# ChenDavidTimothy/mujoco-template

Hardware: AMD Instinct MI355X
Metric: env-steps/sec (whole node), humanoid batch=4096 random-ctrl rollout (higher is better)
Workload: dtype f32

## Files before the change

### mujoco_template_amd/csrc/mjb_api.hip

```cpp
#include <hip/hip_runtime.h>

#include <dlfcn.h>

#include <cmath>
#include <cstdio>
#include <cstdlib>
#include <chrono>
#include <cstring>
#include <map>
#include <string>
#include <vector>

#include "../../include/mjbatch.h"
#include "mjb_buffer.hpp"
#include "mjb_host.hpp"
#include "mjb_kernels.hpp"
#include "mjb_lqr.hpp"
#include "mjb_dare.hpp"
#include "mjb_eig.hpp"
#include "mjb_dlyap.hpp"
#include "mjb_traj.hpp"

using namespace mjb;

namespace {
thread_local std::string g_err;
int fail(int code, const std::string& msg) { g_err = msg; return code; }
#define HIPCHK(expr)                                                                                           \
  do {                                                                                                         \
    hipError_t e_ = (expr);                                                                                    \
    if (e_ != hipSuccess) return fail(MJB_ERR_DEVICE, std::string(#expr) + ": " + hipGetErrorString(e_));      \
  } while (0)

struct DevAlloc {
  Arena& arena;
  template <typename X> const X* put(const std::vector<X>& v) {
    X* p = arena.alloc<X>(v.size());
    if (p && v.size() && hipMemcpy(p, v.data(), v.size() * sizeof(X), hipMemcpyHostToDevice) != hipSuccess) arena.ok = false;
    return p;
  }
  const float* putf(const std::vector<float>& v) { return put(v); }
  const double* putf(const std::vector<double>& v) { return put(v); }
  const int* puti(const std::vector<int>& v) { return put(v); }
  const unsigned long long* putu(const std::vector<unsigned long long>& v) { return put(v); }
};
template <typename... B> void reset_all(B&... b) { (b.reset(), ...); }
template <typename X> hipError_t reserve_zeroed(Buffer<X>& b, size_t n) {
  if (n <= b.count()) return hipSuccess;
  hipError_t e = b.reserve(n);
  if (e == hipSuccess && b.kind() != Mem::Device) std::memset(b.get(), 0, n * sizeof(X));
  else if (e == hipSuccess && (e = hipMemset(b.get(), 0, n * sizeof(X))) != hipSuccess) b.reset();
  return e;
}

struct ArrayInfo { void* ptr; long per_env; int kind; };
}

struct mjbModel {
  HostModel h;
  int disableactuator;
  int iterations;
  double tolerance;
  std::vector<char> blob;
  struct Field { std::string name; int dtype; long count; size_t off; };
  std::vector<Field> fields;
  std::map<int, std::vector<std::string>> names;
};

struct mjbObsSpec {
  ObsSpecDev dev;
  Arena arena;
};

struct Config {
  int G, G_fd, ncon_max, nefc_max;
  Lay Lf, Ld;
  Lay Lf2;
};

struct mjbData {
  mjbModel* model;
  int batch, dtype, device, env0;
  Config cfg;
  hipStream_t stream;
  Arena arena;
  DevModel<float> mf;
  DevModel<double> md;
// ... 170 lines not shown
  HIPCHK(hipMemcpy(d->md_dev, &d->md, sizeof(d->md), hipMemcpyHostToDevice));
  d->up_disable = mm->disableactuator; d->up_iter = mm->iterations; d->up_tol = mm->tolerance;
  return MJB_OK;
}


void choose_caps(const HostModel& h, int dtype, int lanes, int nconmax, int nefcmax, int& nc_out, int& ne_out) {
  int ne, nc;
  if (nconmax > 0 || nefcmax > 0) {
    nc = nconmax > 0 ? nconmax : (h.ncon_alloc < 32 ? h.ncon_alloc : 32);
    ne = nefcmax > 0 ? nefcmax : (h.nefc_alloc < 96 ? h.nefc_alloc : 96);
  } else {
    const size_t budget = (size_t)160 * 1024 / (dtype == MJB_F32 ? 8 : 4);
    ne = h.nefc_alloc < 96 ? h.nefc_alloc : 96; nc = 0;
    if (h.nefc_alloc <= 96 && h.ncon_alloc <= 32) {
      ne = h.nefc_alloc; nc = h.ncon_alloc;
    } else for (;; ne -= 8) {
      int hi = ne * 3 / 8; if (hi < 8) hi = 8; if (hi > h.ncon_alloc) hi = h.ncon_alloc;
      int lo = ne / 3; if (lo < 8) lo = 8; if (lo > hi) lo = hi;
      bool fits = false;
      for (nc = hi; nc >= lo; nc--) {
        Lay t = make_layout(h, nc > 0 ? nc : 1, ne > 0 ? ne : 1, dtype == MJB_F32 ? sizeof(float) : sizeof(double));
        if ((size_t)(64 / lanes) * (size_t)t.bytes <= budget) { fits = true; break; }
      }
      if (fits) break;
      if (ne <= 32) { nc = hi; break; }
    }
  }
  if (nc < 1) nc = 1;
  if (ne < 1) ne = 1;
  nc_out = nc; ne_out = ne;
}
int auto_lanes(const HostModel& h, int lanes) { return lanes == 0 ? (h.nv <= 4 ? 8 : (h.nv <= 16 ? 16 : 64)) : lanes; }

bool derive_config(const HostModel& h, int dtype, int lanes, int nconmax, int nefcmax, Config& c, std::string& err) {
  c.G = auto_lanes(h, lanes);
  if (c.G != 8 && c.G != 16 && c.G != 64) { err = "lanes must be 8, 16 or 64"; return false; }
  choose_caps(h, dtype, c.G, nconmax, nefcmax, c.ncon_max, c.nefc_max);
  c.Lf = make_layout(h, c.ncon_max, c.nefc_max, sizeof(float));
  c.Ld = make_layout(h, c.ncon_max, c.nefc_max, sizeof(double));
  c.G_fd = c.G;
  while (c.G_fd < 64 && (size_t)(64 / c.G_fd) * (size_t)c.Ld.bytes > 160 * 1024) c.G_fd = c.G_fd == 8 ? 16 : 64;
  const size_t lds = (size_t)(64 / c.G) * (size_t)(dtype == MJB_F32 ? c.Lf.bytes : c.Ld.bytes);
  if (lds > 160 * 1024 || (size_t)(64 / c.G_fd) * (size_t)c.Ld.bytes > 160 * 1024) {
    char buf[256];
    std::snprintf(buf, sizeof buf, "per-workgroup LDS %zu B exceeds 160 KiB (lower nconmax/nefcmax or use more lanes)", lds);
    err = buf;
    return false;
  }
  std::memset(&c.Lf2, 0, sizeof(Lay));
  if (dtype == MJB_F32 && c.G == 64 && h.nv <= 32 && h.integrator != INT_RK4) {
    c.Lf2 = make_layout(h, c.ncon_max, c.nefc_max, sizeof(float), true);
    if ((size_t)c.Lf2.bytes > 64 * 1024) std::memset(&c.Lf2, 0, sizeof(Lay));
  }
  return true;
}

struct KernelKind { const char* symbol; const char* banner; const char* not_applicable; };
const KernelKind kKinds[4] = {
    {nullptr, nullptr, nullptr},
    {"mjb_k_step_spec", "// generated by mjb_model_spec_source(): size- and layout-specialised k_step<float, float, G> of ONE compiled model\n",
     "only the float32 step kernel is specialised"},
    {"mjb_k_fd_spec", "// generated by mjb_fd_spec_source(): size- and layout-specialised k_fd<double, TS, G> of ONE compiled model\n", ""},
    {"mjb_k_step2_spec", "// generated by mjb_step2_spec_source(): size- and (flat) layout-specialised two-wave step kernel k_step2<float, float> of ONE compiled model\n",
     "the two-wave step kernel does not apply to this configuration (fp32, one wave per environment, nv <= 32, Euler)"},
};
bool valid_kind(int kind) { return kind == MJB_KERNEL_STEP || kind == MJB_KERNEL_FD || kind == MJB_KERNEL_STEP2; }

struct KernelTarget { const Lay* L; int G; const char* ts; bool applies; };
KernelTarget kernel_target(const Config& c, int dtype, int kind) {
  switch (kind) {
    case MJB_KERNEL_STEP: return {&c.Lf, c.G, "float", dtype == MJB_F32};
    case MJB_KERNEL_FD: return {&c.Ld, c.G_fd, dtype == MJB_F32 ? "float" : "double", true};
    default: return {&c.Lf2, 64, "float", c.Lf2.bytes > 0};
  }
}
int check_kind(const Config& c, int dtype, int kind) {
  if (!valid_kind(kind)) return fail(MJB_ERR_ARG, "unknown kernel kind (MJB_KERNEL_STEP, MJB_KERNEL_FD or MJB_KERNEL_STEP2)");
  if (!kernel_target(c, dtype, kind).applies) return fail(MJB_ERR_ARG, kKinds[kind].not_applicable);
  return MJB_OK;
}

struct EmitAlloc {
  std::string text;
  int n = 0;
  static constexpr unsigned long long TOKEN = 0x7E57AB1Eull << 32;
  template <typename X, typename F> const X* emit(const std::vector<X>& v, const char* ctype, F fmt) {
    std::string body;
    if (v.empty()) body = "0";
    for (size_t i = 0; i < v.size(); i++) { if (i) body += (i % 16 == 0 ? ",\n " : ","); body += fmt(v[i]); }
    text += std::string("static const __constant__ ") + ctype + " mjb_tab_" + std::to_string(n) + "[] = {" + body + "};\n";
    return (const X*)(uintptr_t)(TOKEN + (unsigned long long)(n++) * 16ull + 16ull);
  }
  const float* putf(const std::vector<float>& v) {
    return emit(v, "float", [](float x) {
      if (std::isnan(x)) return std::string("__builtin_nanf(\"\")");
      if (std::isinf(x)) return std::string(x > 0 ? "__builtin_inff()" : "-__builtin_inff()");
      char b[48]; std::snprintf(b, sizeof(b), "%af", (double)x); return std::string(b);
    });
  }
  const double* putf(const std::vector<double>& v) {
    return emit(v, "double", [](double x) {
      if (std::isnan(x)) return std::string("__builtin_nan(\"\")");
      if (std::isinf(x)) return std::string(x > 0 ? "__builtin_inf()" : "-__builtin_inf()");
      char b[48]; std::snprintf(b, sizeof(b), "%a", x); return std::string(b);
    });
  }
  const int* puti(const std::vector<int>& v) { return emit(v, "int", [](int x) { return std::to_string(x); }); }
  const unsigned long long* putu(const std::vector<unsigned long long>& v) {
    return emit(v, "unsigned long long", [](unsigned long long x) { char b[40]; std::snprintf(b, sizeof(b), "0x%llxull", x); return std::string(b); });
  }
};

template <typename T>
std::string baked_model_source(const HostModel& h, int ncon_max, int nefc_max) {
  static_assert(sizeof(DevModel<T>) % 8 == 0, "DevModel<T> is written out in 8-byte words");
  const char* tname = sizeof(T) == 4 ? "float" : "double";
  EmitAlloc ea;
  DevModel<T> m;
  fill_dev_model<T>(h, ea, ncon_max, nefc_max, m);
  const size_t nw = sizeof(m) / 8;
  std::vector<unsigned long long> wv(nw);
  std::memcpy(wv.data(), (const void*)&m, sizeof(m));
  std::string decl = "struct MjbBakedModel {", init = "static const __constant__ MjbBakedModel mjb_baked_model = {";
  for (size_t i = 0; i < nw; i++) {
    const unsigned long long v = wv[i];
    if ((v >> 32) == (EmitAlloc::TOKEN >> 32)) {
      decl += " const void MJB_CONST* p" + std::to_string(i) + ";";
      init += " (const void MJB_CONST*)mjb_tab_" + std::to_string((int)((v - EmitAlloc::TOKEN) / 16 - 1)) + ",";
    } else {
      char b[64];
      decl += " unsigned a" + std::to_string(i) + ", b" + std::to_string(i) + ";";
      std::snprintf(b, sizeof(b), " 0x%xu, 0x%xu,", (unsigned)(v & 0xffffffffull), (unsigned)(v >> 32));
      init += b;
    }
    if (i % 8 == 7) init += "\n ";
  }
  decl += " };\n"; init += " };\n";
  {
    std::vector<int> seen((size_t)ea.n, 0);
    bool ok = true;
    for (size_t i = 0; i < nw && ok; i++)
      if ((wv[i] >> 32) == (EmitAlloc::TOKEN >> 32)) {
        const unsigned long long k = (wv[i] - EmitAlloc::TOKEN) / 16 - 1;
        if (k >= (unsigned long long)ea.n || (wv[i] - EmitAlloc::TOKEN) % 16 != 0 || seen[(size_t)k]++) ok = false;
      }
    for (int k = 0; k < ea.n && ok; k++) if (seen[(size_t)k] != 1) ok = false;
    if (!ok) return std::string("// (model not baked in: the DevModel image did not map one-to-one onto the emitted tables)\n");
  }
  std::string s = "#include \"mjb_types.hpp\"\n// the model as constant data of this translation unit (tables, then the DevModel image)\n";
  s += ea.text + decl + init;
  s += std::string("static_assert(sizeof(MjbBakedModel) == sizeof(mjb::DevModel<") + tname + ">), \"baked model image\");\n";
  s += std::string("#define MJB_SPEC_BAKED (*(const mjb::DevModel<") + tname + "> MJB_CONST*)&mjb_baked_model)\n";
  return s;
}

std::string spec_source(const HostModel& h_model, const Config& c, int dtype, int kind, int prm_mask) {
  HostModel h_damped;
  if ((prm_mask >> PRM_DOF_DAMPING) & 1) { h_damped = h_model; h_damped.has_damping = 1; }
  const HostModel& h = (prm_mask >> PRM_DOF_DAMPING) & 1 ? h_damped : h_model;
  const KernelTarget t = kernel_target(c, dtype, kind);
  const Lay& L = *t.L;
  const int ncon_max = c.ncon_max, nefc_max = c.nefc_max;
  std::string s = kKinds[kind].banner;
  s += "#define MJB_SPEC_KERNEL " + std::to_string(kind) + "\n#define MJB_SPEC_TS " + t.ts + "\n#define MJB_SPEC_G " + std::to_string(t.G) + "\n#define MJB_SPEC_ASSUME(m)";
  auto A = [&](const char* obj, const char* f, long v) { s += std::string(" __builtin_assume((") + obj + ")." + f + " == " + std::to_string(v) + ");"; };
#define SM(f, v) A("m", #f, (long)(v))
  SM(nq, h.nq); SM(nv, h.nv); SM(nu, h.nu); SM(nbody, h.nbody); SM(njnt, h.njnt); SM(ngeom, h.ngeom); SM(nsite, h.nsite);
  SM(ntendon, h.ntendon); SM(nwrap, h.nwrap); SM(nsensor, h.nsensor); SM(nsensordata, h.nsensordata); SM(nkey, h.nkey); SM(npair, h.npair);
  SM(nlevel, h.nlevel); SM(integrator, h.integrator); SM(has_damping, h.has_damping); SM(has_fluid, h.has_fluid); SM(has_accel, h.has_accel);
  SM(nvp, h.nvp); SM(nvshift, h.nvshift); SM(ncon_max, ncon_max); SM(nefc_max, nefc_max); SM(nsiteact, h.siteact.size()); SM(nmpair, h.mpair.size());
  SM(nround, h.nround); SM(nround_inner, h.nround_inner); SM(max_nsub, h.max_nsub); SM(dfs_ok, h.dfs_ok);
#undef SM
  s += "\n";
  if (prm_mask) s += "#define MJB_SPEC_PARAMS " + std::to_string(prm_mask) + "   // per-environment model parameters: bit k = field MJB_PRM_k\n";
  s += "#define MJB_SPEC_ASSUME_LAY(L)";
#define SL(f) A("L", #f, (long)L.f)
  SL(qpos); SL(qvel); SL(ctrl); SL(qacc); SL(qacc_ws); SL(qacc_smooth); SL(qfrc_bias); SL(qfrc_passive); SL(qfrc_actuator); SL(qfrc_smooth);
  SL(qfrc_constraint); SL(xpos); SL(xquat); SL(xmat); SL(xipos); SL(ximat); SL(xanchor); SL(xaxis); SL(geom_xpos); SL(geom_xmat); SL(site_xpos);
  SL(site_xmat); SL(subtree_com); SL(cinert); SL(crb); SL(cdof); SL(cdof_dot); SL(cvel); SL(cacc); SL(cfrc); SL(dofbuf); SL(bfrc); SL(M); SL(W);
  SL(ten_length); SL(ten_J); SL(act_force); SL(sens); SL(con); SL(efc_J); SL(efc_pos); SL(efc_D); SL(efc_aref); SL(efc_jar); SL(efc_jv);
  SL(efc_force); SL(efc_KBI); SL(Ma); SL(grad); SL(search); SL(Mv); SL(tmp); SL(cholcol); SL(rk); SL(nT); SL(i_efc_type); SL(i_efc_id);
  SL(i_con_pair); SL(i_scal); SL(i_mail); SL(nI); SL(bytes);
#undef SL
  s += "\n";
  {
    bool le2 = true;
    for (const char* name : {"jnt_solimp", "tendon_solimp", "pair_solimp"}) {
      const auto& v = h.D(name);
      for (size_t k = 4; k < v.size(); k += 5) { const double pw = v[k] > 1.0 ? v[k] : 1.0; if (pw != 1.0 && pw != 2.0) le2 = false; }
    }
    if (le2) s += "#define MJB_SPEC_SOLIMP_POWER_1_OR_2 1\n";
  }
  s += kind != MJB_KERNEL_FD ? baked_model_source<float>(h, ncon_max, nefc_max) : baked_model_source<double>(h, ncon_max, nefc_max);
  s += "#include \"mjb_kernels.hpp\"\n";
  if (prm_mask) s += "extern \"C\" __constant__ int mjb_spec_params = " + std::to_string(prm_mask) + ";   // checked by mjb_kernel_load\n";
  return s;
}

static void choose_schedule(mjbData* d, StepArgs& a) {
  a.chunk_steps = 0; a.fair_bit = 0; a.nblk = 0; a.grid_blocks = 0; a.nuniform = 0; a.nchunk = 0;
  if (a.mode != 0) return;
  if (d->sched_chunk == -1) {
    const char* e1 = std::getenv("MJB_CHUNK_STEPS"); const char* e2 = std::getenv("MJB_FAIR_BIT");
    d->sched_chunk = e1 ? std::atoi(e1) : -2; d->fair_bit = e2 ? std::atoi(e2) : -2;
  }
  const int epb = 64 / d->cfg.G;
  const long nblk = (d->batch + epb - 1) / epb;
  if (d->step_slots < 0) {
    int nb = 0;
    if (hipFunction_t fn = d->spec[MJB_KERNEL_STEP].fn) {
      if (hipModuleOccupancyMaxActiveBlocksPerMultiprocessor(&nb, fn, 64, (size_t)epb * d->cfg.Lf.bytes) != hipSuccess) nb = 0;
    } else nb = d->dtype == MJB_F32 ? step_blocks_per_cu<float, float>(d->cfg.G, d->cfg.Lf) : step_blocks_per_cu<double, double>(d->cfg.G, d->cfg.Ld);
    d->step_slots = nb > 0 ? (long)nb * d->ncu : 0;
  }
  a.fair_bit = d->fair_bit >= 0 ? d->fair_bit : 15;
  a.nblk = (int)nblk; a.grid_blocks = d->step_slots > 0 && d->step_slots < nblk ? (int)d->step_slots : (int)nblk;
  if (d->sched_chunk >= 0) {
    a.chunk_steps = a.nstep > 1 ? d->sched_chunk : 0;
    if (std::getenv("MJB_SCHED_DEBUG")) std::fprintf(stderr, "[mjb] schedule (override): blocks %ld, resident slots %ld, steps %d -> chunk_steps %d, fair_bit %d\n", nblk, d->step_slots, a.nstep, a.chunk_steps, a.fair_bit);
    return;
  }
  if (d->step_slots > 0 && nblk > d->step_slots && a.nstep >= 4) {
    int c = (int)std::lround(std::sqrt(3.0 * (double)a.nstep));
    a.chunk_steps = c < 1 ? 1 : (c > 32 ? 32 : c);
  }
  if (std::getenv("MJB_SCHED_DEBUG")) std::fprintf(stderr, "[mjb] schedule: blocks %ld, resident slots %ld, steps %d -> chunk_steps %d, fair_bit %d\n", nblk, d->step_slots, a.nstep, a.chunk_steps, a.fair_bit);
}

int engine_check(const mjbData* d) {
  if (d->flags_pin.get() && __atomic_load_n(d->flags_pin.get() + 3, __ATOMIC_ACQUIRE) != 0)
    return fail(MJB_ERR_DEVICE, "a ticket-mode launch timed out waiting for a state hand-over (engine flag 8): the environments concerned were not "
                                "advanced; mjb_reset() clears the condition");
  return MJB_OK;
}

hipError_t launch_spec_step(mjbData* d, int kind, const Lay* lg, const DevDebug<float>& dbg, const StepArgs& a, const ObsSpecDev& obs,
                            void* obs_out, unsigned grid, unsigned block, size_t lds) {
  const DevModel<float>* mg = d->mf_dev;
  DevData<float> dv = d->df; DevDebug<float> dbgarg = dbg; StepArgs av = a; ObsSpecDev ov = obs; float* oo = (float*)obs_out;
  void* args[] = {(void*)&mg, (void*)&lg, (void*)&dv, (void*)&dbgarg, (void*)&av, (void*)&ov, (void*)&oo};
  return hipModuleLaunchKernel(d->spec[kind].fn, grid, 1, 1, block, 1, 1, (unsigned)lds, d->stream, args, nullptr);
}

int launch(mjbData* d, const StepArgs& a_in, const ObsSpecDev& obs, void* obs_out, bool debug) {
  int rc = engine_check(d);
  if (rc != MJB_OK) return rc;
  rc = refresh_options(d);
  if (rc != MJB_OK) return rc;
  hipError_t e;
  StepArgs a = a_in;
  choose_schedule(d, a);
  if (a.chunk_steps > 0) {
    if (d->dtype != MJB_F32 || a.nstep >= (1 << 20) - 2) a.chunk_steps = 0;
  }
  if (a.chunk_steps > 0 && !d->df.xfer) {
    const HostModel& hm = d->model->h;
    if (reserve_zeroed(d->xfer, (size_t)d->batch * (size_t)(hm.nq + 3 * hm.nv + 2)) != hipSuccess) a.chunk_steps = 0;
    d->df.xfer = d->xfer.get();
  }
  if (a.chunk_steps > 0) chunk_plan_counts(a.nstep, a.chunk_steps, a.nuniform, a.nchunk);
  if (a.mode == 0) {
    const int epb = 64 / d->cfg.G;
    d->last_sched[0] = a.nstep; d->last_sched[1] = (d->batch + epb - 1) / epb; d->last_sched[2] = (int)(d->step_slots > 0 ? d->step_slots : 0);
    d->last_sched[3] = a.chunk_steps; d->last_sched[4] = a.fair_bit;
  }
  unsigned seq_next = d->launch_seq;
  unsigned long long ticket_after = d->ticket_next;
  if (a.chunk_steps > 0) {
    do { seq_next++; } while ((seq_next & 0xFFFu) == 0);
    a.tagbase = (seq_next & 0xFFFu) << 20;
    const unsigned long long adv = (unsigned long long)a.nblk * (unsigned)a.nchunk + (unsigned long long)a.grid_blocks;
    if (d->ticket_next + adv > 0xF0000000ull) { HIPCHK(hipMemsetAsync(d->df.sched, 0, sizeof(unsigned), d->stream)); d->ticket_next = 0; }
    a.ticket_base = (unsigned)d->ticket_next;
    ticket_after = d->ticket_next + adv;
    if (d->xfer_timeout == 0) {
      const char* e1 = std::getenv("MJB_XFER_TIMEOUT_MS");
// ... 1668 lines not shown
```

### mujoco_template_amd/csrc/mjb_device.hpp

```cpp
#pragma once
#include "mjb_types.hpp"

#ifdef MJB_HOST_EMU
#include <cmath>
#include "mjb_hostemu.hpp"
#define MJB_DEV static inline
#define MJB_DEVM inline
#define MJB_DEV_CALL static __attribute__((noinline))
#else
#include <hip/hip_runtime.h>
#define MJB_DEV __device__ __forceinline__
#define MJB_DEVM __device__ __forceinline__
#define MJB_DEV_CALL __device__ __attribute__((noinline))
#endif

#ifdef MJB_HOST_EMU
#define MJB_MFMA(a, b, acc) emu_mfma((a), (b), (acc))
#define MJB_BALLOT(p) emu_ballot(p)
#define MJB_RSQF(x) (1.0f / sqrtf(x))
#define MJB_RCPF(x) (1.0f / (x))
#define MJB_MEMTIME() 0ull
#define MJB_OPAQUE1(a) ((void)0)
#define MJB_OPAQUE2(a, b) ((void)0)
#define MJB_OPAQUE9(a, b, c, d, e, f, g, h, i) ((void)0)
#else
#define MJB_MFMA(a, b, acc) __builtin_amdgcn_mfma_f32_32x32x2f32((a), (b), (acc), 0, 0, 0)
#define MJB_BALLOT(p) __ballot(p)
#define MJB_RSQF(x) __builtin_amdgcn_rsqf(x)
#define MJB_RCPF(x) __builtin_amdgcn_rcpf(x)
#define MJB_MEMTIME() __builtin_amdgcn_s_memtime()
#define MJB_OPAQUE1(a) asm volatile("" : "+v"(a))
#define MJB_OPAQUE2(a, b) asm volatile("" : "+v"(a), "+v"(b))
#define MJB_OPAQUE9(a, b, c, d, e, f, g, h, i) asm volatile("" : "+v"(a), "+v"(b), "+v"(c), "+v"(d), "+v"(e), "+v"(f), "+v"(g), "+v"(h), "+v"(i))
#endif

namespace mjb {

#ifndef MJB_HOST_EMU
typedef float mjb_f16v __attribute__((ext_vector_type(16)));
#endif

#ifndef MJB_HOST_EMU
template <int G> MJB_DEV void gsync() {
  __builtin_amdgcn_fence(__ATOMIC_RELEASE, "wavefront");
  __builtin_amdgcn_wave_barrier();
  __builtin_amdgcn_fence(__ATOMIC_ACQUIRE, "wavefront");
}

template <int CTRL> MJB_DEV int dpp_i(int v) { return __builtin_amdgcn_update_dpp(0, v, CTRL, 0xF, 0xF, false); }
template <int CTRL> MJB_DEV float dpp_f(float v) { return __int_as_float(dpp_i<CTRL>(__float_as_int(v))); }
template <int CTRL> MJB_DEV double dpp_f(double v) {
  return __hiloint2double(dpp_i<CTRL>(__double2hiint(v)), dpp_i<CTRL>(__double2loint(v)));
}
MJB_DEV int rdlane_i(int v, int l) { return __builtin_amdgcn_readlane(v, l); }
MJB_DEV float rdlane_f(float v, int l) { return __int_as_float(__builtin_amdgcn_readlane(__float_as_int(v), l)); }
MJB_DEV double rdlane_f(double v, int l) {
  return __hiloint2double(__builtin_amdgcn_readlane(__double2hiint(v), l), __builtin_amdgcn_readlane(__double2loint(v), l));
}
MJB_DEV float wave_rows_sum(float v) {
  asm("s_nop 1\n\tv_add_f32_dpp %0, %0, %0 row_bcast:15 row_mask:0xa bank_mask:0xf\n\ts_nop 1\n\tv_add_f32_dpp %0, %0, %0 row_bcast:31 row_mask:0xc bank_mask:0xf" : "+v"(v));
  return rdlane_f(v, 63);
}
MJB_DEV double wave_rows_sum(double v) { return (rdlane_f(v, 0) + rdlane_f(v, 16)) + (rdlane_f(v, 32) + rdlane_f(v, 48)); }
MJB_DEV int wave_rows_sum(int v) { return (rdlane_i(v, 0) + rdlane_i(v, 16)) + (rdlane_i(v, 32) + rdlane_i(v, 48)); }
template <typename T, int G> MJB_DEV T gsum(T v) {
  v += dpp_f<0xB1>(v);
  v += dpp_f<0x4E>(v);
  if (G >= 8) v += dpp_f<0x141>(v);
  if (G >= 16) v += dpp_f<0x140>(v);
  if (G == 64) v = wave_rows_sum(v);
  return v;
}
template <int G> MJB_DEV int gsumi(int v) {
  v += dpp_i<0xB1>(v);
  v += dpp_i<0x4E>(v);
  if (G >= 8) v += dpp_i<0x141>(v);
  if (G >= 16) v += dpp_i<0x140>(v);
  if (G == 64) v = wave_rows_sum(v);
  return v;
}
template <int G> MJB_DEV int gmaxi(int v) {
  int t;
  t = dpp_i<0xB1>(v); v = t > v ? t : v;
  t = dpp_i<0x4E>(v); v = t > v ? t : v;
// ... 319 lines not shown
  T e[NB][NB];
#pragma unroll
  for (int a = 0; a < NB; a++)
#pragma unroll
    for (int b = 0; b < NB; b++) {
      int r = 8 * a + lr, cc = 8 * b + lc;
      e[a][b] = (r < n && cc <= r) ? M[r * n + cc] : (T)0;
    }
  if (mode == 1) {
    for (int row = 0; row < nefc; row++) {
      T d = dw[row];
      if (d == 0) continue;
      T jr[NB], jc[NB];
#pragma unroll
      for (int a = 0; a < NB; a++) { int r = 8 * a + lr; jr[a] = r < n ? d * J[row * n + r] : (T)0; }
#pragma unroll
      for (int b = 0; b < NB; b++) { int cc = 8 * b + lc; jc[b] = cc < n ? J[row * n + cc] : (T)0; }
#pragma unroll
      for (int a = 0; a < NB; a++)
#pragma unroll
        for (int b = 0; b < NB; b++) e[a][b] += jr[a] * jc[b];
    }
  } else if (mode == 2) {
    if (lr == lc) {
#pragma unroll
      for (int a = 0; a < NB; a++) { int r = 8 * a + lr; if (r < n) e[a][a] += m.timestep * m.dof_damping[r]; }
    }
  }
  for (int j = 0; j < n; j++) {
    const int bj = j >> 3, lj = j & 7;
    if (lr == lj && lc == lj) {
#pragma unroll
      for (int b = 0; b < NB; b++) if (b == bj) col[n] = e[b][b];
    }
    gsync<64>();
    const T ljj = t_sqrt(t_max(col[n], Num<T>::minval()));
    const T inv = 1 / ljj;
    if (lc == lj) {
#pragma unroll
      for (int b = 0; b < NB; b++) {
        if (b != bj) continue;
#pragma unroll
        for (int a = 0; a < NB; a++) {
          int r = 8 * a + lr;
          if (r > j && r < n) { T v = e[a][b] * inv; e[a][b] = v; col[r] = v; }
          else if (r == j) e[a][b] = ljj;
        }
      }
    }
    if (lane == 0) dinv[j] = inv;
    gsync<64>();
    T rv[NB], cv[NB];
#pragma unroll
    for (int a = 0; a < NB; a++) { int r = 8 * a + lr; rv[a] = (r > j && r < n) ? col[r] : (T)0; }
#pragma unroll
    for (int b = 0; b < NB; b++) { int cc = 8 * b + lc; cv[b] = (cc > j && cc < n) ? col[cc] : (T)0; }
#pragma unroll
    for (int a = 0; a < NB; a++)
#pragma unroll
      for (int b = 0; b < NB; b++) e[a][b] -= rv[a] * cv[b];
  }
#pragma unroll
  for (int a = 0; a < NB; a++)
#pragma unroll
    for (int b = 0; b < NB; b++) {
      int r = 8 * a + lr, cc = 8 * b + lc;
      if (r < n && cc <= r) W[tri_at(r, cc)] = e[a][b];
    }
  gsync<64>();
}

#ifndef MJB_SPEC_ASSUME
#define MJB_SPEC_ASSUME(m)
#endif
#ifndef MJB_SPEC_ASSUME_LAY
#define MJB_SPEC_ASSUME_LAY(L)
#endif
#if defined(MJB_SPEC_BAKED) && !defined(MJB_HOST_EMU)
#define MJB_MODEL_OF(p) MJB_SPEC_BAKED
#else
#define MJB_MODEL_OF(p) (*(p))
#endif
#define MJB_OPT(c, f) ((*(c).mp).f)
#ifdef MJB_HOST_EMU
#define MJB_ENV(c) ModelRef<T> m = *(c).mp; LayRef L = *(c).lp
#else
#define MJB_ENV(c)                                     \
  auto mp_ = (c).mp; auto lp_ = (c).lp;                \
  asm volatile("" : "+s"(mp_), "+s"(lp_));             \
  ModelRef<T> m = MJB_MODEL_OF(mp_); LayRef L = *lp_;  \
  MJB_SPEC_ASSUME(m) MJB_SPEC_ASSUME_LAY(L)
#endif
template <typename T> using ModelRef = const DevModel<T> MJB_CONST&;
typedef const Lay MJB_CONST& LayRef;

template <typename T> struct Ctx {
  bool skip_dynamics = false;
  const DevModel<T> MJB_CONST* mp;
  const Lay MJB_CONST* lp;
  const PrmRows MJB_CONST* pr;
  int env;
  T* w;
  int* wi;
  int lane;
  int ncon, nefc, niter, con_dropped, efc_dropped;
#if defined(MJB_PHASE_REPEAT) && !defined(MJB_HOST_EMU)
  int rep = -1;
#endif
#if defined(MJB_PROFILE) && !defined(MJB_HOST_EMU)
  unsigned long long pacc[PH_N] = {};
  unsigned long long pt = 0;
#endif
  MJB_DEVM Ctx(const DevModel<T> MJB_CONST* m_, const Lay MJB_CONST* L_, T* w_, int* wi_, int lane_, const PrmRows MJB_CONST* pr_ = nullptr, int env_ = 0)
      : mp(m_), lp(L_), pr(pr_), env(env_), w(w_), wi(wi_), lane(lane_), ncon(0), nefc(0), niter(0), con_dropped(0), efc_dropped(0) {}
};

#if defined(MJB_SPEC_KERNEL) && !defined(MJB_HOST_EMU)
#ifndef MJB_SPEC_PARAMS
#define MJB_SPEC_PARAMS 0
#endif
#define MJB_PRM_ON(k) ((((MJB_SPEC_PARAMS) >> (k)) & 1) != 0)
#define MJB_PRM_SURE 1
#else
#define MJB_PRM_ON(k) true
#define MJB_PRM_SURE 0
#endif
template <int K> MJB_DEVM constexpr int prm_src() { return K == PRM_SUBTREEMASS ? PRM_BODY_MASS : (K == PRM_PAIR_FRICTION ? PRM_GEOM_FRICTION : K); }
template <typename T> struct PrmSel;
template <> struct PrmSel<float> { static MJB_DEVM const float MJB_CONST* get(const PrmRows MJB_CONST* r, int k) { return r->f[k]; } };
template <> struct PrmSel<double> { static MJB_DEVM const double MJB_CONST* get(const PrmRows MJB_CONST* r, int k) { return r->d[k]; } };
template <int K, typename T, typename TP>
MJB_DEV const T MJB_CONST* prm_row(const Ctx<T>& c, TP tab, int n) {
  if constexpr (MJB_PRM_ON(prm_src<K>())) {
#ifdef MJB_HOST_EMU
    if (!c.pr) return tab;
#endif
    const T MJB_CONST* row = PrmSel<T>::get(c.pr, K);
    if (MJB_PRM_SURE || row) return row + (long)c.env * n;
  }
  return tab;
}
template <int K, typename T, typename TP>
MJB_DEV T prm_get(const Ctx<T>& c, TP tab, int n, int i, int ti) {
  if constexpr (MJB_PRM_ON(prm_src<K>())) {
#ifdef MJB_HOST_EMU
    if (!c.pr) return tab[ti];
#endif
    const T MJB_CONST* row = PrmSel<T>::get(c.pr, K);
    if (MJB_PRM_SURE || row) return row[(long)c.env * n + i];
  }
  return tab[ti];
}
template <typename T> MJB_DEV bool has_damping(const Ctx<T>& c, int model_has_damping) {
  if constexpr (MJB_PRM_ON(PRM_DOF_DAMPING)) {
    if (MJB_PRM_SURE) return true;
#ifdef MJB_HOST_EMU
    if (!c.pr) return model_has_damping != 0;
#endif
    return model_has_damping != 0 || PrmSel<T>::get(c.pr, PRM_DOF_DAMPING) != nullptr;
  }
  return model_has_damping != 0;
}
template <typename T> struct DampRef { T timestep; const T MJB_CONST* dof_damping; };
template <typename T> MJB_DEV DampRef<T> damp_ref(const Ctx<T>& c, const DevModel<T> MJB_CONST& m) {
  return DampRef<T>{m.timestep, prm_row<PRM_DOF_DAMPING>(c, m.dof_damping, m.nv)};
}

#if defined(MJB_PROFILE) && !defined(MJB_HOST_EMU)
#define MJB_STAMP_START(c) ((c).pt = __builtin_amdgcn_s_memtime())
#define MJB_STAMP(c, k) do { unsigned long long t_ = __builtin_amdgcn_s_memtime(); (c).pacc[k] += t_ - (c).pt; (c).pt = t_; } while (0)
#define MJB_TIMED(c, k, call) do { unsigned long long t0_ = __builtin_amdgcn_s_memtime(); call; (c).pacc[k] += __builtin_amdgcn_s_memtime() - t0_; } while (0)
#define MJB_COUNT(c, k) ((c).pacc[k] += 1)
#define MJB_PACC(c, k) ((c).pacc + (k))
#define MJB_PROF_FLUSH(c, prof, lane) do { if ((lane) == 0 && (prof)) for (int k_ = 0; k_ < PH_N; k_++) atomicAdd((prof) + k_, (c).pacc[k_]); } while (0)
#else
#define MJB_STAMP_START(c) ((void)0)
#define MJB_STAMP(c, k) ((void)0)
#define MJB_TIMED(c, k, call) do { call; } while (0)
#define MJB_COUNT(c, k) ((void)0)
#define MJB_PACC(c, k) nullptr
#define MJB_PROF_FLUSH(c, prof, lane) ((void)0)
#endif
#if defined(MJB_PHASE_REPEAT) && !defined(MJB_HOST_EMU)
#define MJB_SET_REPEAT(c, k) ((c).rep = (k))
#define MJB_REPEATS(c, k) ((c).rep == (k))
#else
#define MJB_SET_REPEAT(c, k) ((void)0)
#define MJB_REPEATS(c, k) false
#endif
#define MJB_REP_N(c, id) (MJB_REPEATS(c, id) ? 2 : 1)
#define MJB_PHASE_CALL(c, k, call) do { call; if (MJB_REPEATS(c, k)) { gsync<G>(); call; } } while (0)
enum { REP_CHOL = 32, REP_REUSE = 33, REP_MV = 34, REP_LS = 35, REP_WARM = 36, REP_GRAD = 37, REP_CTRL = 38 };

template <typename T, typename MRef>
MJB_DEV void reg_factor32(MRef m, const T* M, T* W, T* dinv, const T* J, const T* dw, int nefc, int mode, int n, int lane, T* x) {
  T a[32];
  const bool own = lane < n;
#pragma unroll
  for (int k = 0; k < 32; k++) a[k] = (own && k < n) ? M[lane * n + k] : ((k == lane) ? (T)1 : (T)0);
  if (mode == 1) {
    for (int row = 0; row < nefc; row++) {
      T d = dw[row];
      if (d == 0) continue;
      T jrow = own ? J[row * n + lane] : (T)0;
      T s = d * jrow;
#pragma unroll
      for (int k = 0; k < 32; k++) a[k] += s * rdlane_f(jrow, k);
    }
  } else if (mode == 2) {
    T dd = own ? m.timestep * m.dof_damping[lane] : (T)0;
#pragma unroll
    for (int k = 0; k < 32; k++) if (k == lane) a[k] += dd;
  }
  T myinv = 1;
  T r = (x && own) ? x[lane] : (T)0;
#pragma unroll
  for (int j = 0; j < 32; j++) {
    T ajj = t_max(rdlane_f(a[j], j), Num<T>::minval());
    T inv = t_rsqrt(ajj);
    T ljj = ajj * inv;
    a[j] = lane == j ? ljj : a[j] * inv;
    if (lane == j) myinv = inv;
    T yj = rdlane_f(r, j) * inv;
    r = lane > j ? r - a[j] * yj : (lane == j ? yj : r);
#pragma unroll
    for (int k = j + 1; k < 32; k++) a[k] -= a[j] * rdlane_f(a[j], k);
  }
  if (own) {
#pragma unroll
    for (int k = 0; k < 32; k++) if (k <= lane) W[tri_at(lane, k)] = a[k];
    dinv[lane] = myinv;
  }
  gsync<64>();
  if (x) {
    T lrow[32];
// ... 351 lines not shown
#pragma unroll
      for (int k = 0; k < NC; k++) { pa[k] = arr[NC * p + k]; ch[k] = arr[NC * b + k]; }
#pragma unroll
      for (int k = 0; k < NC; k++) arr[NC * p + k] = pa[k] + ch[k];
    }
    gsync<G>();
  }
}

#define MJB_TREE_PASSES 4
template <typename T, int G, int NC> MJB_DEV void tree_forward_sum(Ctx<T>& c, T* arr) {
  MJB_ENV(c); const int lane = c.lane;
  const int nitem = m.nbody * NC, nl = m.nlevel;
  if (nitem > MJB_TREE_PASSES * G) { tree_forward_sum_levels<T, G, NC>(c, arr); return; }
  T s[MJB_TREE_PASSES];
#pragma unroll
  for (int ps = 0; ps < MJB_TREE_PASSES; ps++) {
    const int e = lane + ps * G;
    s[ps] = 0;
    if (e < nitem) {
      const int b = e / NC, k = e - b * NC;
      int na = b > 0 ? m.body_depth[b] - 1 : 0;
      MJB_OPAQUE1(na);
      T acc = arr[e];
      for (int u = 0; u < nl - 1; u++) {
        const int a = m.body_anc[b * nl + u];
        T v = arr[NC * a + k];
        acc += u < na ? v : (T)0;
      }
      s[ps] = acc;
    }
  }
  gsync<G>();
#pragma unroll
  for (int ps = 0; ps < MJB_TREE_PASSES; ps++) { const int e = lane + ps * G; if (e < nitem) arr[e] = s[ps]; }
  gsync<G>();
}
template <typename T, int G, int NC> MJB_DEV void tree_backward_sum(Ctx<T>& c, T* arr, int nrounds, int first_body) {
  MJB_ENV(c); const int lane = c.lane;
  const int nitem = m.nbody * NC, mx = m.max_nsub;
  if (!m.dfs_ok || nitem > MJB_TREE_PASSES * G) { tree_backward_sum_rounds<T, G, NC>(c, arr, nrounds); return; }
  T s[MJB_TREE_PASSES];
#pragma unroll
  for (int ps = 0; ps < MJB_TREE_PASSES; ps++) {
    if (ps * G >= nitem) { s[ps] = 0; continue; }
    const int e = lane + ps * G;
    const bool on = e < nitem;
    const int b = on ? e / NC : 0;
    const int n = on && b >= first_body ? m.body_nsub[b] : 0;
    const T* base = arr + (on ? e : 0);
    T acc = base[0];
    for (int d0 = 0; d0 < mx && gany<G>(d0 < n); d0 += 4) {
      T v[4];
#pragma unroll
      for (int u = 0; u < 4; u++) { const int dd = d0 + u + 1; v[u] = base[NC * (dd <= n ? dd : n)]; }
#pragma unroll
      for (int u = 0; u < 4; u++) acc += d0 + u + 1 <= n ? v[u] : (T)0;
    }
    s[ps] = acc;
  }
  gsync<G>();
#pragma unroll
  for (int ps = 0; ps < MJB_TREE_PASSES; ps++) { const int e = lane + ps * G; if (e < nitem) arr[e] = s[ps]; }
  gsync<G>();
}

template <typename T> MJB_DEV void quat_rot(T* r, const T* q, const T* v) {
  T R[9];
  quat2mat(R, q);
  mulmatvec3(r, R, v);
}

template <typename T, int G> MJB_DEV void kinematics(Ctx<T>& c) {
  MJB_ENV(c); T* w = c.w; const int lane = c.lane;
  T *xpos = w + L.xpos, *xquat = w + L.xquat, *xmat = w + L.xmat, *xipos = w + L.xipos, *ximat = w + L.ximat;
  T *qpos = w + L.qpos, *xanchor = w + L.xanchor, *xaxis = w + L.xaxis;
  if (lane == 0) {
    xpos[0] = xpos[1] = xpos[2] = 0; xquat[0] = 1; xquat[1] = xquat[2] = xquat[3] = 0;
    xipos[0] = xipos[1] = xipos[2] = 0;
#pragma unroll
    for (int k = 0; k < 9; k++) { xmat[k] = (k % 4 == 0) ? (T)1 : (T)0; ximat[k] = xmat[k]; }
  }
  for (int b = 1 + lane; b < m.nbody; b += G) {
    const int jadr = m.body_irec[4 * b], jnum = m.body_irec[4 * b + 1], jt0 = m.body_irec[4 * b + 2];
    T pos[3], quat[4], R[9];
    if (jnum == 1 && jt0 == JNT_FREE) {
      int qa = m.jnt_irec[6 * jadr + 1];
      quat[0] = qpos[qa + 3]; quat[1] = qpos[qa + 4]; quat[2] = qpos[qa + 5]; quat[3] = qpos[qa + 6];
      quat_normalize(quat);
      qpos[qa + 3] = quat[0]; qpos[qa + 4] = quat[1]; qpos[qa + 5] = quat[2]; qpos[qa + 6] = quat[3];
      pos[0] = qpos[qa]; pos[1] = qpos[qa + 1]; pos[2] = qpos[qa + 2];
      xanchor[3 * jadr] = pos[0]; xanchor[3 * jadr + 1] = pos[1]; xanchor[3 * jadr + 2] = pos[2];
      xaxis[3 * jadr] = 0; xaxis[3 * jadr + 1] = 0; xaxis[3 * jadr + 2] = 1;
    } else {
#pragma unroll
      for (int k = 0; k < 3; k++) pos[k] = m.body_pos[3 * b + k];
#pragma unroll
      for (int k = 0; k < 4; k++) quat[k] = m.body_quat[4 * b + k];
      quat2mat(R, quat);
      for (int j = jadr; j < jadr + jnum; j++) {
        T jp[3] = {m.jnt_rec[8 * j], m.jnt_rec[8 * j + 1], m.jnt_rec[8 * j + 2]};
        T ja[3] = {m.jnt_rec[8 * j + 3], m.jnt_rec[8 * j + 4], m.jnt_rec[8 * j + 5]};
        const int jtype = m.jnt_irec[6 * j], qa = m.jnt_irec[6 * j + 1];
        T val = qpos[qa] - m.jnt_rec[8 * j + 6];
        T anchor[3], axis[3];
        mulmatvec3(anchor, R, jp);
        anchor[0] += pos[0]; anchor[1] += pos[1]; anchor[2] += pos[2];
        mulmatvec3(axis, R, ja);
        xanchor[3 * j] = anchor[0]; xanchor[3 * j + 1] = anchor[1]; xanchor[3 * j + 2] = anchor[2];
        xaxis[3 * j] = axis[0]; xaxis[3 * j + 1] = axis[1]; xaxis[3 * j + 2] = axis[2];
        if (jtype == JNT_SLIDE) {
          pos[0] += axis[0] * val; pos[1] += axis[1] * val; pos[2] += axis[2] * val;
        } else {
          T ql[4], qn[4], v[3];
          axisangle2quat(ql, ja, val);
          quat_mul(qn, quat, ql);
          quat[0] = qn[0]; quat[1] = qn[1]; quat[2] = qn[2]; quat[3] = qn[3];
          quat2mat(R, quat);
          mulmatvec3(v, R, jp);
          pos[0] = anchor[0] - v[0]; pos[1] = anchor[1] - v[1]; pos[2] = anchor[2] - v[2];
        }
      }
    }
#pragma unroll
    for (int k = 0; k < 3; k++) xpos[3 * b + k] = pos[k];
#pragma unroll
    for (int k = 0; k < 4; k++) xquat[4 * b + k] = quat[k];
  }
  gsync<G>();
  if (m.nbody - 1 <= G) {
    const int b = 1 + lane, nl = m.nlevel;
    const bool own = b < m.nbody;
    const int dep = own ? m.body_depth[b] : 0;
    for (int d = 1; d < nl; d <<= 1) {
      const bool hop = own && d <= dep - 1;
      T pq[4], pp[3], lq[4], lp[3], q[4], t[3];
      if (hop) {
        const int a = m.body_anc[b * nl + d - 1];
#pragma unroll
        for (int k = 0; k < 4; k++) { pq[k] = xquat[4 * a + k]; lq[k] = xquat[4 * b + k]; }
#pragma unroll
        for (int k = 0; k < 3; k++) { pp[k] = xpos[3 * a + k]; lp[k] = xpos[3 * b + k]; }
        quat_mul(q, pq, lq);
        quat_rot(t, pq, lp);
      }
      gsync<G>();
      if (hop) {
#pragma unroll
        for (int k = 0; k < 4; k++) xquat[4 * b + k] = q[k];
#pragma unroll
        for (int k = 0; k < 3; k++) xpos[3 * b + k] = pp[k] + t[k];
      }
      gsync<G>();
    }
    if (own) {
      T q[4];
#pragma unroll
      for (int k = 0; k < 4; k++) q[k] = xquat[4 * b + k];
      quat_normalize(q);
#pragma unroll
      for (int k = 0; k < 4; k++) xquat[4 * b + k] = q[k];
    }
    gsync<G>();
  } else {
    const int b0 = 1 + lane;
    int dep0 = -1, par0 = 0;
    if (b0 < m.nbody) { dep0 = m.body_depth[b0]; par0 = m.body_parentid[b0]; }
    for (int lev = 1; lev <= m.nlevel; lev++) {
      for (int b = b0; b < m.nbody; b += G) {
        const int dep = b == b0 ? dep0 : m.body_depth[b];
        if (dep != lev) continue;
        const int p = b == b0 ? par0 : m.body_parentid[b];
        T pq[4], pp[3], lq[4], lp[3], q[4], t[3];
#pragma unroll
        for (int k = 0; k < 4; k++) { pq[k] = xquat[4 * p + k]; lq[k] = xquat[4 * b + k]; }
#pragma unroll
        for (int k = 0; k < 3; k++) { pp[k] = xpos[3 * p + k]; lp[k] = xpos[3 * b + k]; }
        quat_mul(q, pq, lq);
        quat_normalize(q);
        quat_rot(t, pq, lp);
#pragma unroll
        for (int k = 0; k < 4; k++) xquat[4 * b + k] = q[k];
#pragma unroll
        for (int k = 0; k < 3; k++) xpos[3 * b + k] = pp[k] + t[k];
      }
      gsync<G>();
    }
  }
  for (int b = 1 + lane; b < m.nbody; b += G) {
    T quat[4], R[9], t[3], q2[4], R2[9];
#pragma unroll
    for (int k = 0; k < 4; k++) quat[k] = xquat[4 * b + k];
    quat2mat(R, quat);
    T ip[3] = {m.body_ipos[3 * b], m.body_ipos[3 * b + 1], m.body_ipos[3 * b + 2]};
    T iq[4] = {m.body_iquat[4 * b], m.body_iquat[4 * b + 1], m.body_iquat[4 * b + 2], m.body_iquat[4 * b + 3]};
    mulmatvec3(t, R, ip);
    quat_mul(q2, quat, iq);
    quat2mat(R2, q2);
#pragma unroll
    for (int k = 0; k < 3; k++) xipos[3 * b + k] = xpos[3 * b + k] + t[k];
#pragma unroll
    for (int k = 0; k < 9; k++) { xmat[9 * b + k] = R[k]; ximat[9 * b + k] = R2[k]; }
  }
  for (int j = lane; j < m.njnt; j += G) {
    if (m.jnt_irec[6 * j] == JNT_FREE) continue;
    int p = m.jnt_irec[6 * j + 4];
    T pq[4], R[9], a[3], ax[3], la[3] = {xanchor[3 * j], xanchor[3 * j + 1], xanchor[3 * j + 2]}, lx[3] = {xaxis[3 * j], xaxis[3 * j + 1], xaxis[3 * j + 2]};
#pragma unroll
    for (int k = 0; k < 4; k++) pq[k] = xquat[4 * p + k];
    quat2mat(R, pq);
    mulmatvec3(a, R, la);
    mulmatvec3(ax, R, lx);
#pragma unroll
    for (int k = 0; k < 3; k++) { xanchor[3 * j + k] = xpos[3 * p + k] + a[k]; xaxis[3 * j + k] = ax[k]; }
  }
  gsync<G>();
  T *gx = w + L.geom_xpos, *gm = w + L.geom_xmat, *sx = w + L.site_xpos, *sm = w + L.site_xmat;
  for (int g = lane; g < m.ngeom + m.nsite; g += G) {
    bool is_geom = g < m.ngeom;
    int id = is_geom ? g : g - m.ngeom;
    int b = is_geom ? m.geom_bodyid[id] : m.site_bodyid[id];
    auto lp = is_geom ? m.geom_pos + 3 * id : m.site_pos + 3 * id;
    auto lq = is_geom ? m.geom_quat + 4 * id : m.site_quat + 4 * id;
    T p3[3] = {lp[0], lp[1], lp[2]}, q4[4] = {lq[0], lq[1], lq[2], lq[3]}, bm[9], bq[4], t[3], q[4], R[9];
#pragma unroll
    for (int k = 0; k < 9; k++) bm[k] = xmat[9 * b + k];
#pragma unroll
    for (int k = 0; k < 4; k++) bq[k] = xquat[4 * b + k];
    mulmatvec3(t, bm, p3);
    quat_mul(q, bq, q4);
    quat_normalize(q);
    quat2mat(R, q);
    T* op = is_geom ? gx + 3 * id : sx + 3 * id;
    T* om = is_geom ? gm + 9 * id : sm + 9 * id;
#pragma unroll
    for (int k = 0; k < 3; k++) op[k] = xpos[3 * b + k] + t[k];
#pragma unroll
    for (int k = 0; k < 9; k++) om[k] = R[k];
  }
  gsync<G>();
}

template <typename T, int G> MJB_DEV void com_pos(Ctx<T>& c) {
  MJB_ENV(c); T* w = c.w; const int lane = c.lane;
  T *sc = w + L.subtree_com, *xipos = w + L.xipos, *ximat = w + L.ximat, *xmat = w + L.xmat;
  for (int b = lane; b < m.nbody; b += G) {
    T ms = prm_row<PRM_BODY_MASS>(c, m.body_mass, m.nbody)[b];
#pragma unroll
    for (int k = 0; k < 3; k++) sc[3 * b + k] = ms * xipos[3 * b + k];
  }
  gsync<G>();
  tree_backward_sum<T, G, 3>(c, sc, m.nround, 0);
  for (int b = lane; b < m.nbody; b += G) {
    T sm = prm_row<PRM_SUBTREEMASS>(c, m.body_subtreemass, m.nbody)[b];
    if (sm < Num<T>::minval()) { sc[3 * b] = xipos[3 * b]; sc[3 * b + 1] = xipos[3 * b + 1]; sc[3 * b + 2] = xipos[3 * b + 2]; }
    else { T inv = 1 / sm; sc[3 * b] *= inv; sc[3 * b + 1] *= inv; sc[3 * b + 2] *= inv; }
  }
  gsync<G>();
  T* cin = w + L.cinert;
  for (int b = lane; b < m.nbody; b += G) {
    if (b == 0) {
#pragma unroll
      for (int k = 0; k < 10; k++) cin[k] = 0;
      continue;
    }
    int r = m.body_rootid[b];
    T off[3], im[9], res[10];
    const T MJB_CONST* inertia = prm_row<PRM_BODY_INERTIA>(c, m.body_inertia, 3 * m.nbody);
    T inr[3] = {inertia[3 * b], inertia[3 * b + 1], inertia[3 * b + 2]};
#pragma unroll
    for (int k = 0; k < 3; k++) off[k] = xipos[3 * b + k] - sc[3 * r + k];
#pragma unroll
    for (int k = 0; k < 9; k++) im[k] = ximat[9 * b + k];
    inert_com(res, inr, im, off, prm_row<PRM_BODY_MASS>(c, m.body_mass, m.nbody)[b]);
#pragma unroll
    for (int k = 0; k < 10; k++) cin[10 * b + k] = res[k];
  }
  T *cdof = w + L.cdof, *xanchor = w + L.xanchor, *xaxis = w + L.xaxis;
  for (int j = lane; j < m.njnt; j += G) {
    int b = m.jnt_irec[6 * j + 3], da = m.jnt_irec[6 * j + 2], r = m.jnt_irec[6 * j + 5], jt = m.jnt_irec[6 * j];
    T off[3];
#pragma unroll
    for (int k = 0; k < 3; k++) off[k] = sc[3 * r + k] - xanchor[3 * j + k];
    T* cd = cdof + 6 * da;
    if (jt == JNT_FREE) {
      for (int i = 0; i < 3; i++) {
#pragma unroll
        for (int k = 0; k < 6; k++) cd[6 * i + k] = (k == 3 + i) ? (T)1 : (T)0;
        T ax[3] = {xmat[9 * b + i], xmat[9 * b + 3 + i], xmat[9 * b + 6 + i]}, cr[3];
        cross3(cr, ax, off);
        T* cc = cd + 6 * (3 + i);
        cc[0] = ax[0]; cc[1] = ax[1]; cc[2] = ax[2]; cc[3] = cr[0]; cc[4] = cr[1]; cc[5] = cr[2];
      }
    } else if (jt == JNT_SLIDE) {
      cd[0] = cd[1] = cd[2] = 0; cd[3] = xaxis[3 * j]; cd[4] = xaxis[3 * j + 1]; cd[5] = xaxis[3 * j + 2];
    } else {
      T ax[3] = {xaxis[3 * j], xaxis[3 * j + 1], xaxis[3 * j + 2]}, cr[3];
      cross3(cr, ax, off);
      cd[0] = ax[0]; cd[1] = ax[1]; cd[2] = ax[2]; cd[3] = cr[0]; cd[4] = cr[1]; cd[5] = cr[2];
    }
  }
  T *tl = w + L.ten_length, *qpos = w + L.qpos;
  for (int t = lane; t < m.ntendon; t += G) {
    T len = 0;
    for (int wi = m.tendon_adr[t]; wi < m.tendon_adr[t] + m.tendon_num[t]; wi++) {
      int j = m.wrap_objid[wi];
      len += m.wrap_prm[wi] * qpos[m.jnt_qposadr[j]];
    }
    tl[t] = len;
  }
  gsync<G>();
}

template <typename T, int G> MJB_DEV void tendon_jacobian(Ctx<T>& c) {
  MJB_ENV(c); T* tj = c.w + L.ten_J;
  for (int t = c.lane; t < m.ntendon; t += G) {
    for (int i = 0; i < m.nv; i++) tj[t * m.nv + i] = 0;
    for (int wi = m.tendon_adr[t]; wi < m.tendon_adr[t] + m.tendon_num[t]; wi++) tj[t * m.nv + m.jnt_dofadr[m.wrap_objid[wi]]] = m.wrap_prm[wi];
  }
}

template <typename T> MJB_DEV void jac_col_moving(const Ctx<T>& c, int b, int i, const T* point, T* jp, T* jr);
template <typename T> MJB_DEV void jac_col(const Ctx<T>& c, int b, int i, const T* point, T* jp, T* jr) {
  ModelRef<T> m = MJB_MODEL_OF(c.mp);
  jp[0] = jp[1] = jp[2] = 0;
  if (jr) { jr[0] = jr[1] = jr[2] = 0; }
  if (!((m.body_dofmask[b] >> i) & 1ull)) return;
  jac_col_moving<T>(c, b, i, point, jp, jr);
}
template <typename T> MJB_DEV void jac_col_moving(const Ctx<T>& c, int b, int i, const T* point, T* jp, T* jr) {
  ModelRef<T> m = MJB_MODEL_OF(c.mp);
  const T* cd = c.w + c.lp->cdof + 6 * i;
  const T* sc = c.w + c.lp->subtree_com + 3 * m.body_rootid[b];
  T off[3] = {point[0] - sc[0], point[1] - sc[1], point[2] - sc[2]}, ang[3] = {cd[0], cd[1], cd[2]}, t[3];
  cross3(t, ang, off);
  jp[0] = cd[3] + t[0]; jp[1] = cd[4] + t[1]; jp[2] = cd[5] + t[2];
  if (jr) { jr[0] = ang[0]; jr[1] = ang[1]; jr[2] = ang[2]; }
}

template <typename T, int G> MJB_DEV void crb_factor(Ctx<T>& c) {
  MJB_ENV(c); T* w = c.w; const int lane = c.lane, nv = m.nv;
  T *crb = w + L.crb, *cin = w + L.cinert, *cdof = w + L.cdof, *buf = w + L.dofbuf, *M = w + L.M, *W = w + L.W;
  for (int i = lane; i < 10 * m.nbody; i += G) crb[i] = cin[i];
  gsync<G>();
  tree_backward_sum<T, G, 10>(c, crb, m.nround_inner, 1);
  for (int i = lane; i < nv; i += G) {
    T in[10], v[6], r[6];
    int b = m.dof_bodyid[i];
#pragma unroll
    for (int k = 0; k < 10; k++) in[k] = crb[10 * b + k];
#pragma unroll
    for (int k = 0; k < 6; k++) v[k] = cdof[6 * i + k];
    mul_inert_vec(r, in, v);
#pragma unroll
    for (int k = 0; k < 6; k++) buf[6 * i + k] = r[k];
  }
  gsync<G>();
  for (int idx = lane; idx < m.nmpair; idx += G) {
    int pr = m.mpair[idx], i = pr >> 8, j = pr & 0xff;
    T val = 0;
#pragma unroll
    for (int k = 0; k < 6; k++) val += cdof[6 * j + k] * buf[6 * i + k];
    if (i == j) val += prm_row<PRM_DOF_ARMATURE>(c, m.dof_armature, nv)[i];
    M[i * nv + j] = val; M[j * nv + i] = val;
  }
  gsync<G>();
}

template <typename T> struct RawCon { T dist, pos[3], n[3], yh[3]; };

template <typename T> MJB_DEV int nc_sphere_sphere(const T* p1, T r1, const T* p2, T r2, T margin, RawCon<T>& o) {
  T dif[3] = {p2[0] - p1[0], p2[1] - p1[1], p2[2] - p1[2]};
  T cd = t_sqrt(dot3(dif, dif)), dist = cd - r1 - r2;
  if (dist > margin) return 0;
  if (cd < Num<T>::minval()) { o.n[0] = 1; o.n[1] = 0; o.n[2] = 0; } else { T s = 1 / cd; o.n[0] = dif[0] * s; o.n[1] = dif[1] * s; o.n[2] = dif[2] * s; }
  o.dist = dist; o.yh[0] = o.yh[1] = o.yh[2] = 0;
  T k = r1 + (T)0.5 * dist;
  o.pos[0] = p1[0] + o.n[0] * k; o.pos[1] = p1[1] + o.n[1] * k; o.pos[2] = p1[2] + o.n[2] * k;
  return 1;
}
template <typename T> MJB_DEV int nc_plane_sphere(const T* pp, const T* n, const T* sp, T r, T margin, RawCon<T>& o) {
  T dif[3] = {sp[0] - pp[0], sp[1] - pp[1], sp[2] - pp[2]};
  T dist = dot3(dif, n) - r;
  if (dist > margin) return 0;
  o.dist = dist; o.n[0] = n[0]; o.n[1] = n[1]; o.n[2] = n[2]; o.yh[0] = o.yh[1] = o.yh[2] = 0;
  T k = -(r + (T)0.5 * dist);
  o.pos[0] = sp[0] + n[0] * k; o.pos[1] = sp[1] + n[1] * k; o.pos[2] = sp[2] + n[2] * k;
  return 1;
}

template <typename T, int G> MJB_DEV void collide_pass(Ctx<T>& c, int p, bool valid, int& ncon, int& dropped) {
  MJB_ENV(c); T* w = c.w; const int lane = c.lane;
  T *gx = w + L.geom_xpos, *gm = w + L.geom_xmat, *con = w + L.con;
  int* con_pair = c.wi + L.i_con_pair;
  {
    int n = 0;
    RawCon<T> rc[4];
    if (valid) {
      int g1 = m.pair_geom1[p], g2 = m.pair_geom2[p], t1 = m.geom_type[g1], t2 = m.geom_type[g2];
      T margin = m.pair_margin[p];
      T p1[3] = {gx[3 * g1], gx[3 * g1 + 1], gx[3 * g1 + 2]}, p2[3] = {gx[3 * g2], gx[3 * g2 + 1], gx[3 * g2 + 2]};
      T s1[3] = {m.geom_size[3 * g1], m.geom_size[3 * g1 + 1], m.geom_size[3 * g1 + 2]};
      T s2[3] = {m.geom_size[3 * g2], m.geom_size[3 * g2 + 1], m.geom_size[3 * g2 + 2]};
      T z1[3] = {gm[9 * g1 + 2], gm[9 * g1 + 5], gm[9 * g1 + 8]}, z2[3] = {gm[9 * g2 + 2], gm[9 * g2 + 5], gm[9 * g2 + 8]};
      if (t1 == G_PLANE) {
        if (t2 == G_SPHERE) n = nc_plane_sphere(p1, z1, p2, s2[0], margin, rc[0]);
        else if (t2 == G_CAPSULE) {
#pragma unroll
          for (int s = 0; s < 2; s++) {
            T sg = s == 0 ? s2[1] : -s2[1];
            T e[3] = {p2[0] + z2[0] * sg, p2[1] + z2[1] * sg, p2[2] + z2[2] * sg};
            RawCon<T> tmp;
            if (nc_plane_sphere(p1, z1, e, s2[0], margin, tmp)) {
              tmp.yh[0] = z2[0]; tmp.yh[1] = z2[1]; tmp.yh[2] = z2[2];
              if (n == 0) rc[0] = tmp; else rc[1] = tmp;
              n++;
            }
          }
        } else if (t2 == G_BOX) {
          T bm[9];
#pragma unroll
          for (int k = 0; k < 9; k++) bm[k] = gm[9 * g2 + k];
          T dif[3] = {p2[0] - p1[0], p2[1] - p1[1], p2[2] - p1[2]};
          T dist = dot3(dif, z1);
#pragma unroll
          for (int i = 0; i < 8; i++) {
            T v[3] = {(i & 1 ? s2[0] : -s2[0]), (i & 2 ? s2[1] : -s2[1]), (i & 4 ? s2[2] : -s2[2])}, corner[3];
            mulmatvec3(corner, bm, v);
            T ld = dot3(z1, corner);
            if (n < 4 && !(dist + ld > margin || ld > 0)) {
              RawCon<T> tmp;
              tmp.dist = dist + ld; tmp.n[0] = z1[0]; tmp.n[1] = z1[1]; tmp.n[2] = z1[2]; tmp.yh[0] = tmp.yh[1] = tmp.yh[2] = 0;
              T k = -(T)0.5 * tmp.dist;
#pragma unroll
              for (int a = 0; a < 3; a++) tmp.pos[a] = corner[a] + p2[a] + z1[a] * k;
              if (n == 0) rc[0] = tmp; else if (n == 1) rc[1] = tmp; else if (n == 2) rc[2] = tmp; else rc[3] = tmp;
              n++;
            }
          }
        } else if (t2 == G_ELLIPSOID) {
          T em[9], nn[3] = {-z1[0], -z1[1], -z1[2]}, dl[3], s[3], wpt[3];
#pragma unroll
          for (int k = 0; k < 9; k++) em[k] = gm[9 * g2 + k];
          mulmatTvec3(dl, em, nn);
          T den = t_sqrt(s2[0] * s2[0] * dl[0] * dl[0] + s2[1] * s2[1] * dl[1] * dl[1] + s2[2] * s2[2] * dl[2] * dl[2]);
          den = t_max(den, Num<T>::minval());
#pragma unroll
          for (int k = 0; k < 3; k++) s[k] = s2[k] * s2[k] * dl[k] / den;
          mulmatvec3(wpt, em, s);
          wpt[0] += p2[0]; wpt[1] += p2[1]; wpt[2] += p2[2];
          T dif[3] = {wpt[0] - p1[0], wpt[1] - p1[1], wpt[2] - p1[2]};
          T dist = dot3(dif, z1);
          if (!(dist > margin)) {
            rc[0].dist = dist; rc[0].n[0] = z1[0]; rc[0].n[1] = z1[1]; rc[0].n[2] = z1[2]; rc[0].yh[0] = rc[0].yh[1] = rc[0].yh[2] = 0;
            T k = -(T)0.5 * dist;
#pragma unroll
            for (int a = 0; a < 3; a++) rc[0].pos[a] = wpt[a] + z1[a] * k;
            n = 1;
          }
        }
      } else if (t1 == G_SPHERE && t2 == G_SPHERE) {
        n = nc_sphere_sphere(p1, s1[0], p2, s2[0], margin, rc[0]);
      } else if (t1 == G_SPHERE && t2 == G_CAPSULE) {
        T dif[3] = {p1[0] - p2[0], p1[1] - p2[1], p1[2] - p2[2]};
        T x = dot3(z2, dif);
        x = t_min(t_max(x, -s2[1]), s2[1]);
        T pt[3] = {p2[0] + z2[0] * x, p2[1] + z2[1] * x, p2[2] + z2[2] * x};
        n = nc_sphere_sphere(p1, s1[0], pt, s2[0], margin, rc[0]);
      } else if (t1 == G_CAPSULE && t2 == G_CAPSULE) {
        T dif[3] = {p1[0] - p2[0], p1[1] - p2[1], p1[2] - p2[2]};
        T ma = dot3(z1, z1), mb = -dot3(z1, z2), mc = dot3(z2, z2), u = -dot3(z1, dif), v = dot3(z2, dif);
        T det = ma * mc - mb * mb, x1, x2;
        if (t_abs(det) >= (sizeof(T) == 4 ? (T)1e-6 * ma * mc : Num<T>::minval())) {
          x1 = (mc * u - mb * v) / det; x2 = (ma * v - mb * u) / det;
          if (x1 > s1[1]) { x1 = s1[1]; x2 = (v - mb * s1[1]) / mc; }
          else if (x1 < -s1[1]) { x1 = -s1[1]; x2 = (v + mb * s1[1]) / mc; }
          if (x2 > s2[1]) { x2 = s2[1]; x1 = t_min(t_max((u - mb * s2[1]) / ma, -s1[1]), s1[1]); }
          else if (x2 < -s2[1]) { x2 = -s2[1]; x1 = t_min(t_max((u + mb * s2[1]) / ma, -s1[1]), s1[1]); }
          T v1[3] = {p1[0] + z1[0] * x1, p1[1] + z1[1] * x1, p1[2] + z1[2] * x1};
          T v2[3] = {p2[0] + z2[0] * x2, p2[1] + z2[1] * x2, p2[2] + z2[2] * x2};
          n = nc_sphere_sphere(v1, s1[0], v2, s2[0], margin, rc[0]);
        } else {
#pragma unroll
          for (int k = 0; k < 4; k++) {
            if (n >= 2) continue;
            bool ok;
            if (k < 2) { x1 = k == 0 ? s1[1] : -s1[1]; x2 = (v - mb * x1) / mc; ok = x2 >= -s2[1] && x2 <= s2[1]; }
            else { x2 = k == 2 ? s2[1] : -s2[1]; x1 = (u - mb * x2) / ma; ok = x1 >= -s1[1] && x1 <= s1[1]; }
            if (!ok) continue;
            T v1[3] = {p1[0] + z1[0] * x1, p1[1] + z1[1] * x1, p1[2] + z1[2] * x1};
            T v2[3] = {p2[0] + z2[0] * x2, p2[1] + z2[1] * x2, p2[2] + z2[2] * x2};
            RawCon<T> tmp;
            if (nc_sphere_sphere(v1, s1[0], v2, s2[0], margin, tmp)) { if (n == 0) rc[0] = tmp; else rc[1] = tmp; n++; }
          }
        }
      }
    }
    int total, off = gscan_small<G>(n, lane, total);
#pragma unroll
    for (int k = 0; k < 4; k++) {
      if (k < n) {
        int slot = ncon + off + k;
        if (slot < m.ncon_max) {
          const RawCon<T>& r = rc[k];
          T f[9] = {r.n[0], r.n[1], r.n[2], r.yh[0], r.yh[1], r.yh[2], 0, 0, 0};
          normalize3(f);
          if (dot3(f + 3, f + 3) < (T)0.25) {
            f[3] = f[4] = f[5] = 0;
            if (f[1] < (T)0.5 && f[1] > (T)-0.5) f[4] = 1; else f[5] = 1;
          }
          T d = dot3(f, f + 3);
          f[3] -= d * f[0]; f[4] -= d * f[1]; f[5] -= d * f[2];
          normalize3(f + 3);
          T* o = con + slot * CON_STRIDE;
          o[0] = r.dist; o[1] = r.pos[0]; o[2] = r.pos[1]; o[3] = r.pos[2];
#pragma unroll
          for (int a = 0; a < 6; a++) o[4 + a] = f[a];
          o[10] = prm_row<PRM_PAIR_FRICTION>(c, m.pair_friction, 5 * m.npair)[5 * p];
          con_pair[slot] = p;
        }
      }
    }
    int newn = ncon + total;
    if (newn > m.ncon_max) { dropped += newn - (ncon > m.ncon_max ? ncon : m.ncon_max); }
    ncon = newn;
  }
}

template <typename T, int G> MJB_DEV void collision(Ctx<T>& c) {
  MJB_ENV(c); T* w = c.w; const int lane = c.lane;
  T *gx = w + L.geom_xpos, *gm = w + L.geom_xmat;
  int ncon = 0, dropped = 0;
  if (m.nefc_max * m.nv < G) {
    for (int base = 0; base < m.npair; base += G) collide_pass<T, G>(c, base + lane, base + lane < m.npair, ncon, dropped);
  } else {
    int* cand = (int*)(w + L.efc_J);
    int nl = 0;
    for (int base = 0; base < m.npair; base += G) {
      const int p = base + lane;
      bool keep = false;
      if (p < m.npair) {
        const int g1 = m.pair_geom1[p], g2 = m.pair_geom2[p];
        const T cull = m.pair_cull[p];
        T d[3] = {gx[3 * g2] - gx[3 * g1], gx[3 * g2 + 1] - gx[3 * g1 + 1], gx[3 * g2 + 2] - gx[3 * g1 + 2]};
        if (cull < 0) {
          T nz[3] = {gm[9 * g1 + 2], gm[9 * g1 + 5], gm[9 * g1 + 8]};
          keep = dot3(d, nz) <= -cull * (T)1.00001 + (T)1e-6;
        } else {
          T r = cull * (T)1.00001 + (T)1e-6;
          keep = dot3(d, d) <= r * r;
        }
      }
      int total, off = gscan_small<G>(keep ? 1 : 0, lane, total);
      if (nl + total > G) {
        gsync<G>();
        collide_pass<T, G>(c, lane < nl ? cand[lane] : 0, lane < nl, ncon, dropped);
        gsync<G>();
        nl = 0;
      }
      if (keep) cand[nl + off] = p;
      nl += total;
    }
    gsync<G>();
    if (nl > 0) collide_pass<T, G>(c, lane < nl ? cand[lane] : 0, lane < nl, ncon, dropped);
  }
  c.con_dropped += dropped;
  c.ncon = ncon < m.ncon_max ? ncon : m.ncon_max;
  gsync<G>();
}

template <typename T> MJB_DEV void row_imp_R(T pos, T margin, const T* solimp, T diagApprox, T& imp, T& R) {
  const T dmin = solimp[0], dmax = solimp[1], width = solimp[2], mid = solimp[3], power = solimp[4];
  if (dmin == dmax || width <= Num<T>::minval()) imp = (T)0.5 * (dmin + dmax);
  else {
    T x = t_abs(pos - margin) / width;
    if (x >= 1) imp = dmax;
    else if (x <= 0) imp = dmin;
    else {
      T y;
      if (power == 1) y = x;
#ifdef MJB_SPEC_SOLIMP_POWER_1_OR_2
      else y = x <= mid ? x * x / mid : 1 - (1 - x) * (1 - x) / (1 - mid);
#else
      else if (power == 2) y = x <= mid ? x * x / mid : 1 - (1 - x) * (1 - x) / (1 - mid);
      else if (x <= mid) y = t_pow(x, power) / t_pow(mid, power - 1);
      else y = 1 - t_pow(1 - x, power) / t_pow(1 - mid, power - 1);
#endif
      imp = dmin + y * (dmax - dmin);
    }
  }
  R = t_max(Num<T>::minval(), (1 - imp) * diagApprox / imp);
}
template <typename T> MJB_DEV void row_params(ModelRef<T> m, T pos, T margin, const T* solref, const T* solimp, T diagApprox, T& K, T& B, T& imp, T& R) {
  T dmin = t_min(t_max(solimp[0], MJB_MINIMP), MJB_MAXIMP), dmax = t_min(t_max(solimp[1], MJB_MINIMP), MJB_MAXIMP);
  T width = t_max(solimp[2], (T)0), mid = t_min(t_max(solimp[3], MJB_MINIMP), MJB_MAXIMP), power = t_max(solimp[4], (T)1);
  if (dmin == dmax || width <= Num<T>::minval()) imp = (T)0.5 * (dmin + dmax);
  else {
    T x = t_abs(pos - margin) / width;
    if (x >= 1) imp = dmax;
    else if (x <= 0) imp = dmin;
    else {
      T y;
      if (power == 1) y = x;
#ifdef MJB_SPEC_SOLIMP_POWER_1_OR_2
      else y = x <= mid ? x * x / mid : 1 - (1 - x) * (1 - x) / (1 - mid);
#else
      else if (power == 2) y = x <= mid ? x * x / mid : 1 - (1 - x) * (1 - x) / (1 - mid);
      else if (x <= mid) y = t_pow(x, power) / t_pow(mid, power - 1);
      else y = 1 - t_pow(1 - x, power) / t_pow(1 - mid, power - 1);
#endif
      imp = dmin + y * (dmax - dmin);
    }
  }
  if (solref[0] > 0) {
    T tc = t_max(solref[0], 2 * m.timestep), dr = solref[1];
    K = 1 / t_max(Num<T>::minval(), dmax * dmax * tc * tc * dr * dr);
    B = 2 / t_max(Num<T>::minval(), dmax * tc);
  } else {
    K = -solref[0] / t_max(Num<T>::minval(), dmax * dmax);
    B = -solref[1] / t_max(Num<T>::minval(), dmax);
  }
  R = t_max(Num<T>::minval(), (1 - imp) * diagApprox / imp);
}

template <typename T, int G> MJB_DEV void make_constraint(Ctx<T>& c) {
  MJB_ENV(c); T* w = c.w; const int lane = c.lane, nv = m.nv, cap = m.nefc_max;
  T *qpos = w + L.qpos, *qvel = w + L.qvel, *J = w + L.efc_J, *epos = w + L.efc_pos, *eD = w + L.efc_D, *earef = w + L.efc_aref;
  T *eK = w + L.efc_jar, *eB = w + L.efc_jv, *eI = w + L.efc_force;
  T *emargin = w + L.efc_KBI;
  int *etype = c.wi + L.i_efc_type, *con_pair = c.wi + L.i_con_pair;
  T *con = w + L.con, *tl = w + L.ten_length, *tj = w + L.ten_J;
  const int nobj = m.njnt + m.ntendon, nitem = nobj + c.ncon;
  int nlim = 0, ncrow = 0;
  for (int base = 0; base < nitem; base += G) {
    const int k = base + lane;
    const bool isl = k < nobj, isj = k < m.njnt;
    const int ci = k - nobj;
    int cnt = 0, p = 0, sd = 0;
    T dist = 0, dist2 = 0, margin = 0, mu = 0;
    bool both = false;
    if (isl) {
      if (m.lim_i[2 * k]) {
        const T value = isj ? qpos[m.lim_i[2 * k + 1]] : tl[m.lim_i[2 * k + 1]];
        margin = m.lim_f[12 * k + 2];
        const T d0 = value - m.lim_f[12 * k], d1 = m.lim_f[12 * k + 1] - value;
        const bool a0 = d0 < margin, a1 = d1 < margin;
        cnt = (int)a0 + (int)a1;
        both = a0 && a1;
        dist = a0 ? d0 : d1; dist2 = d1; sd = a0 ? 0 : 1;
      }
    } else if (k < nitem) {
      p = con_pair[ci] & 0xffff;
      dist = con[ci * CON_STRIDE]; mu = con[ci * CON_STRIDE + 10];
      margin = m.pair_kb[PAIR_KB_STRIDE * p];
      if (dist < margin) cnt = m.pair_condim[p] == 1 ? 1 : 4;
    }
    int total, off = gscan_small<G>(cnt, lane, total);
    const int limtot = base < nobj ? gtotal_small<G>(isl ? cnt : 0, lane) : 0;
    const int cbase = nlim + limtot < cap ? nlim + limtot : cap;
    const int row = isl ? nlim + off : cbase + ncrow + (off - limtot);
    bool emit = false;
    int type = 0;
    T diag = 0, K = 0, B = 0, si[5];
    if (isl) {
      if (cnt > 0) {
        emit = row < cap;
        type = (isj ? EFC_LIMIT_JOINT : EFC_LIMIT_TENDON) | (((isj ? k : k - m.njnt) * 2 + sd) << 9);
      }
      if (emit || both) {
        diag = m.lim_f[12 * k + 3]; K = m.lim_f[12 * k + 4]; B = m.lim_f[12 * k + 5];
#pragma unroll
        for (int q = 0; q < 5; q++) si[q] = m.lim_f[12 * k + 6 + q];
      }
    } else if (k < nitem) {
      emit = cnt > 0 && row + cnt <= cap;
      con_pair[ci] = p | ((emit ? row + 1 : 0) << 16);
      if (emit) {
        const T tran = m.pair_kb[PAIR_KB_STRIDE * p + 1];
        K = m.pair_kb[PAIR_KB_STRIDE * p + 2]; B = m.pair_kb[PAIR_KB_STRIDE * p + 3];
#pragma unroll
        for (int q = 0; q < 5; q++) si[q] = m.pair_kb[PAIR_KB_STRIDE * p + 4 + q];
        if (cnt == 1) diag = tran; else diag = tran + mu * mu * tran;
        type = (cnt == 1 ? EFC_CONTACT_FRICTIONLESS : EFC_CONTACT_PYRAMIDAL) | (ci << 9);
      }
    }
    if (emit) {
      T imp, R;
      row_imp_R(dist, margin, si, diag, imp, R);
      int nr = 1;
      if (!isl && cnt == 4) {
        R = t_max(Num<T>::minval(), 2 * mu * mu * R);
        nr = 4;
        const T* cc = con + ci * CON_STRIDE;
        T nrm[3] = {cc[4], cc[5], cc[6]}, t1[3] = {cc[7], cc[8], cc[9]}, t2[3];
        cross3(t2, nrm, t1);
        earef[row] = t2[0]; earef[row + 1] = t2[1]; earef[row + 2] = t2[2];
      }
      for (int r = 0; r < nr; r++) {
        etype[row + r] = type;
        epos[row + r] = dist; emargin[row + r] = margin; eD[row + r] = 1 / R; eK[row + r] = K; eB[row + r] = B; eI[row + r] = imp;
      }
    }
    if (base < nobj && gany<G>(both)) {
      if (both && row + 1 < cap) {
        T imp, R;
        row_imp_R(dist2, margin, si, diag, imp, R);
        etype[row + 1] = type + (1 << 9);
        epos[row + 1] = dist2; emargin[row + 1] = margin; eD[row + 1] = 1 / R; eK[row + 1] = K; eB[row + 1] = B; eI[row + 1] = imp;
      }
    }
    nlim += limtot; ncrow += total - limtot;
  }
  const int nlimit = nlim < cap ? nlim : cap;
  int nefc = nlimit + ncrow;
  const int dropped = (nlim > cap ? nlim - cap : 0) + (nefc > cap ? nefc - cap : 0);
  if (nefc > cap) {
    int last = nlimit;
    for (int ci = lane; ci < c.ncon; ci += G) {
      int a = (con_pair[ci] >> 16) - 1;
      if (a >= 0) { int p = con_pair[ci] & 0xffff; int e = a + (m.pair_condim[p] == 1 ? 1 : 4); if (e > last) last = e; }
    }
    nefc = gmaxi<G>(last);
  }
  c.nefc = nefc; c.efc_dropped += dropped;
  gsync<G>();
  {
    int tot = nlimit << m.nvshift;
    for (int idx = lane; idx < tot; idx += G) {
      int r = idx >> m.nvshift, i = idx & (m.nvp - 1);
      if (i >= nv) continue;
      int id_ = etype[r] >> 9, o = id_ >> 1, s = id_ & 1;
      T sign = s == 0 ? (T)1 : (T)-1, v;
      if ((etype[r] & 0xff) == EFC_LIMIT_JOINT) v = (i == m.jnt_dofadr[o]) ? sign : (T)0;
      else v = sign * tj[o * nv + i];
      J[r * nv + i] = v;
    }
  }
  {
    int tot = c.ncon << m.nvshift;
    for (int idx = lane; idx < tot; idx += G) {
      int ci = idx >> m.nvshift, i = idx & (m.nvp - 1);
      if (i >= nv) continue;
      int row = (con_pair[ci] >> 16) - 1;
      if (row < 0) continue;
      int p = con_pair[ci] & 0xffff;
      int b1 = m.pair_body[2 * p], b2 = m.pair_body[2 * p + 1];
      const T* cc = con + ci * CON_STRIDE;
      const bool mv1 = (m.body_dofmask[b1] >> i) & 1ull, mv2 = (m.body_dofmask[b2] >> i) & 1ull;
      T dj[3] = {0, 0, 0};
      if (mv1 != mv2) {
        T pos[3] = {cc[1], cc[2], cc[3]}, col[3];
        jac_col_moving<T>(c, mv2 ? b2 : b1, i, pos, col, (T*)0);
        if (mv2) { dj[0] = col[0]; dj[1] = col[1]; dj[2] = col[2]; }
        else { dj[0] = (T)0 - col[0]; dj[1] = (T)0 - col[1]; dj[2] = (T)0 - col[2]; }
      }
      T jn = cc[4] * dj[0] + cc[5] * dj[1] + cc[6] * dj[2];
      if (m.pair_condim[p] == 1) J[row * nv + i] = jn;
      else {
        T mu = cc[10], t1[3] = {cc[7], cc[8], cc[9]}, t2[3] = {earef[row], earef[row + 1], earef[row + 2]};
        T jt1 = mu * dot3(t1, dj), jt2 = mu * dot3(t2, dj);
        J[row * nv + i] = jn + jt1; J[(row + 1) * nv + i] = jn - jt1;
        J[(row + 2) * nv + i] = jn + jt2; J[(row + 3) * nv + i] = jn - jt2;
      }
    }
  }
  gsync<G>();
  const VecLds<T> xv{qvel};
  for (int r = lane; r < nefc; r += G) {
    T v = dot_lds(J + r * nv, 1, xv, nv);
    earef[r] = -eB[r] * v - eK[r] * eI[r] * (epos[r] - emargin[r]);
  }
  gsync<G>();
}

template <typename T, int G> MJB_DEV void vel_bias_passive(Ctx<T>& c) {
  MJB_ENV(c); T* w = c.w; const int lane = c.lane, nv = m.nv;
  T *cvel = w + L.cvel, *cacc = w + L.cacc, *cfrc = w + L.cfrc, *cdof = w + L.cdof, *cdd = w + L.cdof_dot, *cin = w + L.cinert;
  T *qvel = w + L.qvel, *qpos = w + L.qpos;
  if (lane == 0) {
#pragma unroll
    for (int k = 0; k < 6; k++) { cvel[k] = 0; cfrc[k] = 0; }
    const T MJB_CONST* gravity = prm_row<PRM_GRAVITY>(c, m.gravity, 3);
    cacc[0] = cacc[1] = cacc[2] = 0; cacc[3] = -gravity[0]; cacc[4] = -gravity[1]; cacc[5] = -gravity[2];
  }
  gsync<G>();
  for (int b = 1 + lane; b < m.nbody; b += G) {
    int da = m.body_dofadr[b], dn = m.body_dofnum[b];
    T dv[6] = {0, 0, 0, 0, 0, 0};
    for (int j = da; j < da + dn; j++) {
      T qv = qvel[j];
#pragma unroll
      for (int q = 0; q < 6; q++) dv[q] += cdof[6 * j + q] * qv;
    }
#pragma unroll
    for (int q = 0; q < 6; q++) cvel[6 * b + q] = dv[q];
  }
  gsync<G>();
  tree_forward_sum<T, G, 6>(c, cvel);
  for (int j = lane; j < nv; j += G) {
    const int p = m.dof_irec[6 * j + 1], first = m.dof_irec[6 * j + 2], gs = m.dof_irec[6 * j + 3];
    T tmp[6] = {0, 0, 0, 0, 0, 0};
    if (gs >= 0) {
      T cv[6], cd[6];
#pragma unroll
      for (int q = 0; q < 6; q++) { cv[q] = cvel[6 * p + q]; cd[q] = cdof[6 * j + q]; }
      for (int k = first; k < gs; k++) {
        T qv = qvel[k];
#pragma unroll
        for (int q = 0; q < 6; q++) cv[q] += cdof[6 * k + q] * qv;
      }
      cross_motion(tmp, cv, cd);
    }
#pragma unroll
    for (int q = 0; q < 6; q++) cdd[6 * j + q] = tmp[q];
  }
  gsync<G>();
  for (int b = 1 + lane; b < m.nbody; b += G) {
    int da = m.body_dofadr[b], dn = m.body_dofnum[b];
    T da6[6] = {0, 0, 0, 0, 0, 0};
    for (int j = da; j < da + dn; j++) {
      T qv = qvel[j];
#pragma unroll
      for (int q = 0; q < 6; q++) da6[q] += cdd[6 * j + q] * qv;
    }
    if (m.body_depth[b] == 1) {
#pragma unroll
      for (int q = 0; q < 6; q++) da6[q] += cacc[q];
    }
#pragma unroll
    for (int q = 0; q < 6; q++) cacc[6 * b + q] = da6[q];
  }
  gsync<G>();
  tree_forward_sum<T, G, 6>(c, cacc);
  for (int b = 1 + lane; b < m.nbody; b += G) {
    T in[10], cv[6], ca[6], f[6], t1[6], t2[6];
#pragma unroll
    for (int k = 0; k < 10; k++) in[k] = cin[10 * b + k];
#pragma unroll
    for (int k = 0; k < 6; k++) { cv[k] = cvel[6 * b + k]; ca[k] = cacc[6 * b + k]; }
    mul_inert_vec(f, in, ca);
    mul_inert_vec(t1, in, cv);
    cross_force(t2, cv, t1);
#pragma unroll
    for (int k = 0; k < 6; k++) cfrc[6 * b + k] = f[k] + t2[k];
  }
  gsync<G>();
  tree_backward_sum<T, G, 6>(c, cfrc, m.nround_inner, 1);
  T* bfrc = w + L.bfrc;
  if (m.has_fluid) {
    T *xipos = w + L.xipos, *ximat = w + L.ximat, *sc = w + L.subtree_com;
    for (int b = lane; b < m.nbody; b += G) {
      T mass = prm_row<PRM_BODY_MASS>(c, m.body_mass, m.nbody)[b];
#pragma unroll
      for (int k = 0; k < 6; k++) bfrc[6 * b + k] = 0;
      if (b == 0 || mass < Num<T>::minval()) continue;
      const T MJB_CONST* inertia = prm_row<PRM_BODY_INERTIA>(c, m.body_inertia, 3 * m.nbody);
      T I0 = inertia[3 * b], I1 = inertia[3 * b + 1], I2 = inertia[3 * b + 2];
      T box[3] = {t_sqrt(t_max(Num<T>::minval(), I1 + I2 - I0) / mass * 6), t_sqrt(t_max(Num<T>::minval(), I0 + I2 - I1) / mass * 6), t_sqrt(t_max(Num<T>::minval(), I0 + I1 - I2) / mass * 6)};
      int r = m.body_rootid[b];
      T cv[6], off[3], lin[3], t[3], im[9], lvel[6], lfrc[6] = {0, 0, 0, 0, 0, 0};
#pragma unroll
      for (int k = 0; k < 6; k++) cv[k] = cvel[6 * b + k];
#pragma unroll
      for (int k = 0; k < 3; k++) off[k] = xipos[3 * b + k] - sc[3 * r + k];
#pragma unroll
      for (int k = 0; k < 9; k++) im[k] = ximat[9 * b + k];
      cross3(t, cv, off);
      lin[0] = cv[3] + t[0]; lin[1] = cv[4] + t[1]; lin[2] = cv[5] + t[2];
      mulmatTvec3(lvel, im, cv);
      mulmatTvec3(lvel + 3, im, lin);
      if (m.viscosity > 0) {
        T diam = (box[0] + box[1] + box[2]) / 3;
#pragma unroll
        for (int k = 0; k < 3; k++) { lfrc[k] = -MJB_PI * diam * diam * diam * m.viscosity * lvel[k]; lfrc[3 + k] = -3 * MJB_PI * diam * m.viscosity * lvel[3 + k]; }
      }
      if (m.density > 0) {
        lfrc[3] -= (T)0.5 * m.density * box[1] * box[2] * t_abs(lvel[3]) * lvel[3];
        lfrc[4] -= (T)0.5 * m.density * box[0] * box[2] * t_abs(lvel[4]) * lvel[4];
        lfrc[5] -= (T)0.5 * m.density * box[0] * box[1] * t_abs(lvel[5]) * lvel[5];
        T b0 = box[0] * box[0], b1 = box[1] * box[1], b2 = box[2] * box[2];
        lfrc[0] -= m.density * box[0] * (b1 * b1 + b2 * b2) * t_abs(lvel[0]) * lvel[0] / 64;
        lfrc[1] -= m.density * box[1] * (b0 * b0 + b2 * b2) * t_abs(lvel[1]) * lvel[1] / 64;
        lfrc[2] -= m.density * box[2] * (b0 * b0 + b1 * b1) * t_abs(lvel[2]) * lvel[2] / 64;
      }
      T o1[3], o2[3];
      mulmatvec3(o1, im, lfrc);
      mulmatvec3(o2, im, lfrc + 3);
#pragma unroll
      for (int k = 0; k < 3; k++) { bfrc[6 * b + k] = o1[k]; bfrc[6 * b + 3 + k] = o2[k]; }
    }
    gsync<G>();
  }
  T *qb = w + L.qfrc_bias, *qp = w + L.qfrc_passive;
  for (int i = lane; i < nv; i += G) {
    const int b = m.dof_irec[6 * i], qa = m.dof_irec[6 * i + 4];
    T v = 0;
#pragma unroll
    for (int k = 0; k < 6; k++) v += cdof[6 * i + k] * cfrc[6 * b + k];
    qb[i] = v;
    T pf = -prm_get<PRM_DOF_DAMPING>(c, m.dof_frec, nv, i, 4 * i) * qvel[i];
    if (qa >= 0) pf -= m.dof_frec[4 * i + 1] * (qpos[qa] - m.dof_frec[4 * i + 2]);
    if (m.has_fluid) {
      T* xipos = w + L.xipos;
      for (int bb = 1; bb < m.nbody; bb++) {
        if (!((m.body_dofmask[bb] >> i) & 1ull)) continue;
        T pt[3] = {xipos[3 * bb], xipos[3 * bb + 1], xipos[3 * bb + 2]}, jp[3], jr[3];
        jac_col<T>(c, bb, i, pt, jp, jr);
        pf += jp[0] * bfrc[6 * bb + 3] + jp[1] * bfrc[6 * bb + 4] + jp[2] * bfrc[6 * bb + 5] + jr[0] * bfrc[6 * bb] + jr[1] * bfrc[6 * bb + 1] + jr[2] * bfrc[6 * bb + 2];
      }
    }
    qp[i] = pf;
  }
  gsync<G>();
}

template <typename T, int G> MJB_DEV void actuation_forces(Ctx<T>& c) {
  MJB_ENV(c); T* w = c.w; const int lane = c.lane, nv = m.nv;
  T *ctrl = w + L.ctrl, *af = w + L.act_force, *qpos = w + L.qpos, *qvel = w + L.qvel;
  for (int a = lane; a < m.nu; a += G) {
    int grp = m.actuator_group[a];
    T force = 0;
    if (!(grp >= 0 && grp < 31 && ((MJB_OPT(c, disableactuator) >> grp) & 1))) {
      T u = ctrl[a];
      if (m.actuator_ctrllimited[a]) u = t_min(t_max(u, m.actuator_ctrlrange[2 * a]), m.actuator_ctrlrange[2 * a + 1]);
      force = prm_row<PRM_ACT_GAINPRM>(c, m.actuator_gainprm, 3 * m.nu)[3 * a] * u;
      if (m.actuator_biastype[a] == 1) {
        T len = 0, vel = 0;
        if (m.actuator_trntype[a] == TRN_JOINT) {
          int j = m.actuator_trnid[2 * a];
          const T MJB_CONST* gear = prm_row<PRM_ACT_GEAR>(c, m.actuator_gear, 6 * m.nu);
          len = gear[6 * a] * qpos[m.jnt_qposadr[j]];
          vel = gear[6 * a] * qvel[m.jnt_dofadr[j]];
        }
        const T MJB_CONST* bias = prm_row<PRM_ACT_BIASPRM>(c, m.actuator_biasprm, 3 * m.nu);
        force += bias[3 * a] + bias[3 * a + 1] * len + bias[3 * a + 2] * vel;
      }
      if (m.actuator_forcelimited[a]) force = t_min(t_max(force, m.actuator_forcerange[2 * a]), m.actuator_forcerange[2 * a + 1]);
    }
    af[a] = force;
  }
  gsync<G>();
  T *qa = w + L.qfrc_actuator, *qs = w + L.qfrc_smooth, *qas = w + L.qacc_smooth, *qb = w + L.qfrc_bias, *qp = w + L.qfrc_passive;
  T *sx = w + L.site_xpos, *sm = w + L.site_xmat;
  for (int i = lane; i < nv; i += G) {
    T s = 0;
    const T MJB_CONST* gear = prm_row<PRM_ACT_GEAR>(c, m.actuator_gear, 6 * m.nu);
    for (int k = m.dofact_adr[i]; k < m.dofact_adr[i + 1]; k++) { int a = m.dofact_act[k]; s += gear[6 * a] * af[a]; }
    for (int k = 0; k < m.nsiteact; k++) {
      int a = m.siteact[k], id = m.actuator_trnid[2 * a], b = m.site_bodyid[id];
      if (!((m.body_dofmask[b] >> i) & 1ull)) continue;
      T g[6], R[9], f[3], tq[3], pt[3] = {sx[3 * id], sx[3 * id + 1], sx[3 * id + 2]}, jp[3], jr[3];
#pragma unroll
      for (int q = 0; q < 6; q++) g[q] = gear[6 * a + q];
#pragma unroll
      for (int q = 0; q < 9; q++) R[q] = sm[9 * id + q];
      mulmatvec3(f, R, g);
      mulmatvec3(tq, R, g + 3);
      jac_col<T>(c, b, i, pt, jp, jr);
      s += (dot3(jp, f) + dot3(jr, tq)) * af[a];
    }
    qa[i] = s;
    T fs = qp[i] - qb[i] + s;
    qs[i] = fs; qas[i] = fs;
  }
  gsync<G>();
}
template <typename T, int G> MJB_DEV void actuation_acceleration(Ctx<T>& c) {
  actuation_forces<T, G>(c);
  factor_W<T, G>(c, 0, c.w + c.lp->qacc_smooth);
}

template <typename T, int G> MJB_DEV bool jt_split(int nv) { return G == 64 && nv <= 32; }
template <typename T, int G> MJB_DEV T jt_dot(const T* J, const T* f, int nefc, int nv, int lane) {
  const int h = lane >> 5, i = lane & 31, n2 = (nefc + 1) >> 1;
  const int r0 = h ? n2 : 0, cnt = h ? nefc - n2 : n2;
  T p = i < nv ? dot_lds(J + r0 * nv + i, nv, VecLds<T>{f + r0}, cnt) : (T)0;
  return half_sum(p);
}

template <typename T, int G> MJB_DEV T solver_cost(Ctx<T>& c, const T* qacc, bool store) {
  MJB_ENV(c); T* w = c.w; const int lane = c.lane, nv = m.nv, nefc = c.nefc;
  T *M = w + L.M, *J = w + L.efc_J, *Ma = w + L.Ma, *jar = w + L.efc_jar, *aref = w + L.efc_aref, *D = w + L.efc_D, *force = w + L.efc_force;
  T *qs = w + L.qfrc_smooth, *qas = w + L.qacc_smooth;
  T part = 0;
  const VecLds<T> xq{qacc};
  for (int rho = lane; rho < nv + nefc; rho += G) {
    const bool ism = rho < nv;
    const int r = ism ? rho : rho - nv;
    T s = dot_lds(ism ? M + r * nv : J + r * nv, 1, xq, nv);
    if (ism) {
      Ma[r] = s;
      part += (T)0.5 * (s - qs[r]) * (qacc[r] - qas[r]);
    } else {
      s -= aref[r];
      jar[r] = s;
      if (s < 0) { part += (T)0.5 * D[r] * s * s; if (store) force[r] = -D[r] * s; }
      else if (store) force[r] = 0;
    }
  }
  T cost = gsum<T, G>(part);
  gsync<G>();
  return cost;
}

template <typename T> MJB_DEV bool mark_active_row(int* etype, T* dw, int r, T sj, T d) {
  const int act = sj < 0 ? 1 : 0, t = etype[r];
  etype[r] = (t & ~0x100) | (act << 8);
  dw[r] = act ? d : (T)0;
  return ((t >> 8) & 1) != act;
}
template <typename T, int G> MJB_DEV T newton_direction(Ctx<T>& c, bool rebuild, T gtol2) {
  MJB_ENV(c); T* w = c.w; const int lane = c.lane, nv = m.nv, nefc = c.nefc;
  T *M = w + L.M, *W = w + L.W, *J = w + L.efc_J, *Ma = w + L.Ma, *force = w + L.efc_force;
  T *grad = w + L.grad, *search = w + L.search, *qs = w + L.qfrc_smooth;
  T gpart = 0;
  for (int rp_ = MJB_REP_N(c, REP_GRAD); rp_ > 0; rp_--) {
  gpart = 0;
  if (jt_split<T, G>(nv)) {
    const int i = lane & 31;
    T jf = jt_dot<T, G>(J, force, nefc, nv, lane);
    if (lane < nv) { T g = Ma[i] - qs[i] - jf; grad[i] = g; search[i] = -g; gpart = g * g; }
  } else {
    for (int i = lane; i < nv; i += G) {
      T g = Ma[i] - qs[i] - dot_lds(J + i, nv, VecLds<T>{force}, nefc);
      grad[i] = g; search[i] = -g;
      gpart += g * g;
    }
  }
  }
  T gn = gsum<T, G>(gpart);
  gsync<G>();
  if (gn < gtol2) return gn;
  MJB_COUNT(c, PH_CNT_DIR); if (rebuild) MJB_COUNT(c, PH_CNT_FACT);
  for (int rp_ = MJB_REP_N(c, rebuild ? REP_CHOL : REP_REUSE); rp_ > 1; rp_--) {
    if (rebuild) factor_W<T, G>(c, 1, search);
    else if (fused_inverse_path<T, G>(nv)) { gsync<G>(); if constexpr (sizeof(T) == 4) mfma_solve32(W, w + L.tmp, search, nv, lane); }
// ... 130 lines not shown
    T old = cost;
    cost = gsum<T, G>(part);
    rebuild_wanted = gany<G>(chg);
    gsync<G>();
    c.niter = iter + 1;
    if (scale * (old - cost) < tolerance) break;
  }
  if (jt_split<T, G>(nv)) {
    T jf = jt_dot<T, G>(J, force, nefc, nv, lane);
    if (lane < nv) { qc[lane] = jf; ws[lane] = qacc[lane]; }
  } else {
    for (int i = lane; i < nv; i += G) { qc[i] = dot_lds(J + i, nv, VecLds<T>{force}, nefc); ws[i] = qacc[i]; }
  }
  gsync<G>();
}

template <typename T, typename TS, int G> MJB_DEV void sensors(const Ctx<T>& c, TS* dst) {
  ModelRef<T> m = MJB_MODEL_OF(c.mp); LayRef L = *c.lp; const T* w = c.w; const int lane = c.lane;
  for (int s = lane; s < m.nsensor; s += G) {
    TS* out = dst + m.sensor_adr[s];
    int id = m.sensor_objid[s], st = m.sensor_type[s];
    if (st == SENS_JOINTPOS) { out[0] = (TS)w[L.qpos + m.jnt_qposadr[id]]; continue; }
    int b = m.site_bodyid[id];
    T R[9];
#pragma unroll
    for (int k = 0; k < 9; k++) R[k] = w[L.site_xmat + 9 * id + k];
    if (st == SENS_GYRO) {
      T wv[3] = {w[L.cvel + 6 * b], w[L.cvel + 6 * b + 1], w[L.cvel + 6 * b + 2]}, o3[3];
      mulmatTvec3(o3, R, wv);
      out[0] = (TS)o3[0]; out[1] = (TS)o3[1]; out[2] = (TS)o3[2];
    } else if (st == SENS_FRAMEQUAT) {
      T bq[4] = {w[L.xquat + 4 * b], w[L.xquat + 4 * b + 1], w[L.xquat + 4 * b + 2], w[L.xquat + 4 * b + 3]};
      T sq[4] = {m.site_quat[4 * id], m.site_quat[4 * id + 1], m.site_quat[4 * id + 2], m.site_quat[4 * id + 3]}, q[4];
      quat_mul(q, bq, sq);
      quat_normalize(q);
      out[0] = (TS)q[0]; out[1] = (TS)q[1]; out[2] = (TS)q[2]; out[3] = (TS)q[3];
    } else if (st == SENS_ACCEL) {
      T cv[6], ca[6];
#pragma unroll
      for (int k = 0; k < 6; k++) { cv[k] = w[L.cvel + 6 * b + k]; ca[k] = w[L.cacc + 6 * b + k]; }
      for (int i = 0; i < m.nv; i++) {
        if (!((m.body_dofmask[b] >> i) & 1ull)) continue;
        T qa = w[L.qacc + i];
#pragma unroll
        for (int k = 0; k < 6; k++) ca[k] += w[L.cdof + 6 * i + k] * qa;
      }
      int r = m.body_rootid[b];
      T dif[3] = {w[L.site_xpos + 3 * id] - w[L.subtree_com + 3 * r], w[L.site_xpos + 3 * id + 1] - w[L.subtree_com + 3 * r + 1], w[L.site_xpos + 3 * id + 2] - w[L.subtree_com + 3 * r + 2]};
      T t[3], vlin[3], alin[3], wl[3], vl[3], al[3], cr[3];
      cross3(t, cv, dif); vlin[0] = cv[3] + t[0]; vlin[1] = cv[4] + t[1]; vlin[2] = cv[5] + t[2];
      cross3(t, ca, dif); alin[0] = ca[3] + t[0]; alin[1] = ca[4] + t[1]; alin[2] = ca[5] + t[2];
      mulmatTvec3(wl, R, cv); mulmatTvec3(vl, R, vlin); mulmatTvec3(al, R, alin);
      cross3(cr, wl, vl);
      out[0] = (TS)(al[0] + cr[0]); out[1] = (TS)(al[1] + cr[1]); out[2] = (TS)(al[2] + cr[2]);
    } else { out[0] = 0; }
  }
}

template <typename T, int G> MJB_DEV void forward_position(Ctx<T>& c) {
  MJB_STAMP(c, PH_OTHER);
  MJB_PHASE_CALL(c, PH_KIN, (kinematics<T, G>(c))); MJB_STAMP(c, PH_KIN);
  MJB_PHASE_CALL(c, PH_COM, (com_pos<T, G>(c))); MJB_STAMP(c, PH_COM);
  MJB_PHASE_CALL(c, PH_COLL, (collision<T, G>(c))); MJB_STAMP(c, PH_COLL);
  MJB_PHASE_CALL(c, PH_CRB, (crb_factor<T, G>(c))); MJB_STAMP(c, PH_CRB);
}
template <typename T, int G> MJB_DEV void forward_velocity(Ctx<T>& c) {
  MJB_PHASE_CALL(c, PH_CONS, (make_constraint<T, G>(c))); MJB_STAMP(c, PH_CONS);
  MJB_PHASE_CALL(c, PH_VEL, (vel_bias_passive<T, G>(c))); MJB_STAMP(c, PH_VEL);
}
template <typename T, int G> MJB_DEV void forward_acceleration(Ctx<T>& c) {
  MJB_PHASE_CALL(c, PH_ACT, (actuation_acceleration<T, G>(c))); MJB_STAMP(c, PH_ACT);
  solve_constraints<T, G>(c); MJB_STAMP(c, PH_SOLVE);
  if (c.mp->nsensor > 0) { sensors<T, T, G>(c, c.w + c.lp->sens); gsync<G>(); }
}
template <typename T, int G> MJB_DEV void forward(Ctx<T>& c) {
  forward_position<T, G>(c);
  forward_velocity<T, G>(c);
  if (c.skip_dynamics) return;
  forward_acceleration<T, G>(c);
}

template <typename T, int G> MJB_DEV void integrate_pos(ModelRef<T> m, T* qpos, const T* qvel, T h, int lane) {
  for (int j = lane; j < m.njnt; j += G) {
    int qa = m.jnt_irec[6 * j + 1], da = m.jnt_irec[6 * j + 2];
    if (m.jnt_irec[6 * j] == JNT_FREE) {
      qpos[qa] += h * qvel[da]; qpos[qa + 1] += h * qvel[da + 1]; qpos[qa + 2] += h * qvel[da + 2];
      T q[4] = {qpos[qa + 3], qpos[qa + 4], qpos[qa + 5], qpos[qa + 6]}, wv[3] = {qvel[da + 3], qvel[da + 4], qvel[da + 5]};
      quat_integrate(q, wv, h);
      qpos[qa + 3] = q[0]; qpos[qa + 4] = q[1]; qpos[qa + 5] = q[2]; qpos[qa + 6] = q[3];
    } else qpos[qa] += h * qvel[da];
  }
}

template <typename T, int G> MJB_DEV void euler(Ctx<T>& c, const mjb_f16v* inv = nullptr) {
  MJB_ENV(c); T* w = c.w; const int lane = c.lane, nv = m.nv;
  T *qacc = w + L.qacc, *qvel = w + L.qvel, *qpos = w + L.qpos, *tmpv = w + L.Mv, *M = w + L.M, *W = w + L.W;
  T h = m.timestep;
  if (has_damping(c, m.has_damping)) {
    T *qs = w + L.qfrc_smooth, *qc = w + L.qfrc_constraint;
    if (MJB_REPEATS(c, PH_INTEG)) {
      for (int i = lane; i < nv; i += G) tmpv[i] = qs[i] + qc[i];
      gsync<G>();
      factor_W<T, G>(c, 2, tmpv);
      gsync<G>();
    }
    for (int i = lane; i < nv; i += G) tmpv[i] = qs[i] + qc[i];
    gsync<G>();
#ifndef MJB_HOST_EMU
    if constexpr (sizeof(T) == 4 && G == 64) {
      if (inv) mfma_sweep_apply32(*inv, w + L.tmp, nv, lane, tmpv);
      else factor_W<T, G>(c, 2, tmpv);
    } else
#endif
    factor_W<T, G>(c, 2, tmpv);
  } else {
    for (int i = lane; i < nv; i += G) tmpv[i] = qacc[i];
    gsync<G>();
  }
  for (int i = lane; i < nv; i += G) qvel[i] += h * tmpv[i];
  gsync<G>();
  integrate_pos<T, G>(m, qpos, qvel, h, lane);
  gsync<G>();
}

template <typename T, int G> MJB_DEV void rk4_stage(Ctx<T>& c, int st) {
  MJB_ENV(c); T* w = c.w; const int lane = c.lane, nv = m.nv, nq = m.nq;
  T *qacc = w + L.qacc, *qvel = w + L.qvel, *qpos = w + L.qpos;
  T *X0q = w + L.rk, *X0v = X0q + nq, *Fv = X0v + nv, *Fa = Fv + 4 * nv, *dv = Fa + 4 * nv;
  const T h = m.timestep;
  if (st == 0) {
    for (int i = lane; i < nq; i += G) X0q[i] = qpos[i];
    for (int i = lane; i < nv; i += G) X0v[i] = qvel[i];
  }
  for (int i = lane; i < nv; i += G) { Fv[st * nv + i] = qvel[i]; Fa[st * nv + i] = qacc[i]; }
  gsync<G>();
  for (int i = lane; i < nv; i += G) {
    T sv, sa;
    if (st < 3) { T a = st == 2 ? (T)1 : (T)0.5; sv = a * Fv[st * nv + i]; sa = a * Fa[st * nv + i]; }
    else {
      sv = (Fv[i] + 2 * Fv[nv + i] + 2 * Fv[2 * nv + i] + Fv[3 * nv + i]) * (T)(1.0 / 6);
      sa = (Fa[i] + 2 * Fa[nv + i] + 2 * Fa[2 * nv + i] + Fa[3 * nv + i]) * (T)(1.0 / 6);
    }
    dv[i] = sv; qvel[i] = X0v[i] + h * sa;
  }
  for (int i = lane; i < nq; i += G) qpos[i] = X0q[i];
  gsync<G>();
  integrate_pos<T, G>(m, qpos, dv, h, lane);
  gsync<G>();
}

MJB_DEV unsigned philox_first(unsigned c0, unsigned c1, unsigned c2, unsigned c3, unsigned k0, unsigned k1) {
  for (int r = 0; r < 10; r++) {
    unsigned long long p0 = 0xD2511F53ull * c0, p1 = 0xCD9E8D57ull * c2;
    unsigned n0 = (unsigned)(p1 >> 32) ^ c1 ^ k0, n1 = (unsigned)p1, n2 = (unsigned)(p0 >> 32) ^ c3 ^ k1, n3 = (unsigned)p0;
    c0 = n0; c1 = n1; c2 = n2; c3 = n3;
    k0 += 0x9E3779B9u; k1 += 0xBB67AE85u;
  }
  return c0;
}
template <typename T, int G> MJB_DEV void random_ctrl(ModelRef<T> m, T* ctrl, unsigned seed, unsigned env, unsigned step, T scale, int lane) {
  for (int a = lane; a < m.nu; a += G) {
    unsigned r = philox_first(env, step, (unsigned)a, 0u, seed, 0x5EEDu);
    T u = (T)(r >> 8) * (T)(1.0 / 16777216.0);
    T lo = -1, hi = 1;
    if (m.actuator_ctrllimited[a]) { lo = m.actuator_ctrlrange[2 * a]; hi = m.actuator_ctrlrange[2 * a + 1]; }
    ctrl[a] = (T)0.5 * (lo + hi) + (T)0.5 * (hi - lo) * scale * (2 * u - 1);
  }
}

template <typename T, int G> MJB_DEV void feedback_ctrl(Ctx<T>& c, ArgsRef a, unsigned env, unsigned step) {
  MJB_ENV(c); T* w = c.w; const int lane = c.lane, nv = m.nv, nu = m.nu;
  auto K = (const T MJB_CONST*)a.fb_K; auto u0 = (const T MJB_CONST*)a.fb_u0;
  auto q0 = (const T MJB_CONST*)a.fb_q0; auto v0 = (const T MJB_CONST*)a.fb_v0;
  T *dx = w + L.grad, *qpos = w + L.qpos, *qvel = w + L.qvel, *ctrl = w + L.ctrl;
  for (int j = lane; j < m.njnt; j += G) {
    int qa = m.jnt_qposadr[j], da = m.jnt_dofadr[j];
    if (m.jnt_type[j] == JNT_FREE) {
      dx[da] = qpos[qa] - q0[qa]; dx[da + 1] = qpos[qa + 1] - q0[qa + 1]; dx[da + 2] = qpos[qa + 2] - q0[qa + 2];
      T qa4[4] = {q0[qa + 3], q0[qa + 4], q0[qa + 5], q0[qa + 6]}, qb4[4] = {qpos[qa + 3], qpos[qa + 4], qpos[qa + 5], qpos[qa + 6]}, r[3];
      quat_sub(r, qa4, qb4);
      dx[da + 3] = r[0]; dx[da + 4] = r[1]; dx[da + 5] = r[2];
    } else dx[da] = qpos[qa] - q0[qa];
  }
  for (int i = lane; i < nv; i += G) dx[nv + i] = qvel[i] - v0[i];
  gsync<G>();
  for (int act = lane; act < nu; act += G) {
    T u = u0[act];
    for (int k = 0; k < 2 * nv; k++) u -= K[act * 2 * nv + k] * dx[k];
    if (a.fb_nsteps > 0) {
      const long idx = ((long)step + (long)env * a.fb_env_stride) % a.fb_nsteps;
      u += ((const T MJB_CONST*)a.fb_noise_std)[act] * ((const T MJB_CONST*)a.fb_noise_tab)[idx * nu + act];
    }
    if (m.actuator_ctrllimited[act]) u = t_min(t_max(u, m.actuator_ctrlrange[2 * act]), m.actuator_ctrlrange[2 * act + 1]);
    ctrl[act] = u;
  }
  gsync<G>();
}

template <typename T, typename TS, int G> MJB_DEV_CALL void sequence_ctrl(T* ctrl, ArgsRef a, int nu, int env, int step, int lane) {
  const TS* src = (const TS*)a.ctrl_seq + (long)step * a.ctrl_step_stride + (long)env * a.ctrl_env_stride;
  for (int i = lane; i < nu; i += G) ctrl[i] = (T)src[i];
}

template <typename T, typename TS, int G> MJB_DEV void inverse_dynamics(Ctx<T>& c, TS* inv_out, TS* moment_out) {
  MJB_ENV(c); T* w = c.w; const int lane = c.lane, nv = m.nv, nefc = c.nefc;
  T *J = w + L.efc_J, *aref = w + L.efc_aref, *D = w + L.efc_D, *force = w + L.efc_force, *qacc = w + L.qacc, *M = w + L.M;
  T *qb = w + L.qfrc_bias, *qp = w + L.qfrc_passive, *qc = w + L.qfrc_constraint;
  for (int r = lane; r < nefc; r += G) {
    T jar = dot_lds(J + r * nv, 1, VecLds<T>{qacc}, nv) - aref[r];
    force[r] = jar < 0 ? -D[r] * jar : (T)0;
  }
  gsync<G>();
  for (int i = lane; i < nv; i += G) {
    T fc = dot_lds(J + i, nv, VecLds<T>{force}, nefc);
    T ma = dot_lds(M + i * nv, 1, VecLds<T>{qacc}, nv);
    qc[i] = fc;
    inv_out[i] = (TS)(ma + qb[i] - qp[i] - fc);
  }
  T *sx = w + L.site_xpos, *sm = w + L.site_xmat;
  for (int idx = lane; idx < m.nu * nv; idx += G) {
    int a = idx / nv, i = idx - a * nv, id = m.actuator_trnid[2 * a];
    T v = 0;
    const T MJB_CONST* gear = prm_row<PRM_ACT_GEAR>(c, m.actuator_gear, 6 * m.nu);
    if (m.actuator_trntype[a] == TRN_JOINT) v = (i == m.jnt_dofadr[id]) ? gear[6 * a] : (T)0;
    else {
      int b = m.site_bodyid[id];
      if ((m.body_dofmask[b] >> i) & 1ull) {
        T g[6], R[9], f[3], tq[3], pt[3] = {sx[3 * id], sx[3 * id + 1], sx[3 * id + 2]}, jp[3], jr[3];
#pragma unroll
        for (int q = 0; q < 6; q++) g[q] = gear[6 * a + q];
#pragma unroll
        for (int q = 0; q < 9; q++) R[q] = sm[9 * id + q];
        mulmatvec3(f, R, g);
        mulmatvec3(tq, R, g + 3);
        jac_col<T>(c, b, i, pt, jp, jr);
        v = dot3(jp, f) + dot3(jr, tq);
      }
    }
    moment_out[idx] = (TS)v;
  }
  gsync<G>();
}

template <typename T, int G> MJB_DEV bool group_bad(const T* x, int n, int lane) {
  int bad = 0;
  for (int i = lane; i < n; i += G) { T v = x[i]; if (!(t_abs(v) <= (T)1e10)) bad = 1; }
  return gany<G>(bad != 0);
}
template <typename T, int G> MJB_DEV void reset_state(Ctx<T>& c) {
  MJB_ENV(c); T* w = c.w;
  for (int i = c.lane; i < m.nq; i += G) w[L.qpos + i] = m.qpos0[i];
  for (int i = c.lane; i < m.nv; i += G) { w[L.qvel + i] = 0; w[L.qacc + i] = 0; w[L.qacc_ws + i] = 0; }
  for (int i = c.lane; i < m.nu; i += G) w[L.ctrl + i] = 0;
  gsync<G>();
}

struct ResetSpec {
  int nq, nv, nu, njnt;
  const int *jnt_type, *jnt_qposadr, *jnt_dofadr;
  const double *qpos, *qvel, *ctrl;
  double time;
  unsigned seed;
  double qpos_noise, qvel_noise;
};
MJB_DEV double reset_uniform(unsigned seed, unsigned genv, unsigned episode, unsigned i, unsigned stream) {
  return (double)(philox_first(genv, episode, i, stream, seed, 0x5EEDu) >> 8) * (1.0 / 16777216.0);
}
template <typename TS>
MJB_DEV void reset_env_state(const ResetSpec& r, unsigned genv, unsigned episode, TS* qpos, TS* qvel, TS* ctrl, TS* qacc, TS* qacc_ws) {
  for (int i = 0; i < r.nq; i++) qpos[i] = (TS)r.qpos[i];
  if (r.qpos_noise != 0) {
    for (int j = 0; j < r.njnt; j++) {
      const int qa = r.jnt_qposadr[j], da = r.jnt_dofadr[j], t = r.jnt_type[j];
      double dq[6];
      const int nd = t == JNT_FREE ? 6 : (t == JNT_BALL ? 3 : 1);
      for (int k = 0; k < nd; k++) dq[k] = r.qpos_noise * (2.0 * reset_uniform(r.seed, genv, episode, (unsigned)(da + k), 1u) - 1.0);
// ... 426 lines not shown
```

### mujoco_template_amd/csrc/mjb_host.hpp

```cpp
#pragma once
#include <cstring>
#include <string>
#include <vector>

#include "mjb_types.hpp"

namespace mjb {

struct Table {
  int n;
  const char* const* names;
  const void* const* ptrs;
  const int* dtypes;
  const long* counts;
  int find(const char* name) const {
    for (int i = 0; i < n; i++) if (!std::strcmp(names[i], name)) return i;
    return -1;
  }
  bool getd(const char* name, long count, std::vector<double>& out, std::string& err) const {
    int i = find(name);
    if (i < 0 || dtypes[i] != 0 || counts[i] != count) {
      err = std::string("model field '") + name + "': missing or wrong dtype/size (want f64 x " + std::to_string(count) + ")";
      return false;
    }
// ... 90 lines not shown
      for (int b = 1; b < nbody; b++) {
        int r = 0;
        for (int o = 1; o < b; o++) if (parent[o] == parent[b]) r++;
        rank[b] = r;
        if (r + 1 > nrank[depth[b]]) nrank[depth[b]] = r + 1;
      }
      int acc = 0;
      for (int lev = maxd; lev >= 1; lev--) { if (lev == 1) nround_inner = acc; base[lev] = acc; acc += nrank[lev]; }
      nround = acc;
      body_round.assign(nbody, -1);
      for (int b = 1; b < nbody; b++) body_round[b] = base[depth[b]] + rank[b];
    }
    {
      body_nsub.assign(nbody, 0);
      for (int b = nbody - 1; b >= 1; b--) body_nsub[parent[b]] += body_nsub[b] + 1;
      dfs_ok = 1; max_nsub = 0;
      for (int b = 0; b < nbody; b++) {
        if (b >= 1 && body_nsub[b] > max_nsub) max_nsub = body_nsub[b];
        for (int d = b + 1; d <= b + body_nsub[b] && d < nbody; d++) {
          int a = d; while (a != b && a != 0) a = parent[a];
          if (a != b) dfs_ok = 0;
        }
        if (b + body_nsub[b] >= nbody) dfs_ok = 0;
      }
      if (body_nsub[0] > max_nsub) max_nsub = body_nsub[0];
      const int nl = nlevel > 0 ? nlevel : 1;
      body_anc.assign((size_t)nbody * nl, 0);
      for (int b = 0; b < nbody; b++) {
        int a = b, u = 0;
        for (; u < nl; u++) { if (a == 0 || parent[a] == 0) break; a = parent[a]; body_anc[(size_t)b * nl + u] = a; }
        for (; u < nl; u++) body_anc[(size_t)b * nl + u] = b;
      }
    }
    child_adr.assign(nbody + 1, 0);
    child_id.clear();
    for (int b = 0; b < nbody; b++) {
      child_adr[b] = (int)child_id.size();
      for (int ch = 1; ch < nbody; ch++) if (parent[ch] == b) child_id.push_back(ch);
    }
    child_adr[nbody] = (int)child_id.size();
    const auto& dofadr = I("body_dofadr"); const auto& dofnum = I("body_dofnum"); const auto& dofpar = I("dof_parentid");
    body_dofmask.assign(nbody > 0 ? nbody : 1, 0ull);
    for (int b = 1; b < nbody; b++) {
      int p = b;
      while (p > 0) {
        for (int k = 0; k < dofnum[p]; k++) body_dofmask[b] |= 1ull << (dofadr[p] + k);
        p = parent[p];
      }
    }
    dof_ancmask.assign(nv > 0 ? nv : 1, 0ull);
    for (int i = 0; i < nv; i++) for (int j = i; j >= 0; j = dofpar[j]) dof_ancmask[i] |= 1ull << j;
    tri_tab.clear();
    for (int r = 0; r < (nv > 0 ? nv : 1); r++) for (int cc = 0; cc <= r; cc++) tri_tab.push_back((r << 16) | cc);
    {
      const auto& trntype = I("actuator_trntype"); const auto& trnid = I("actuator_trnid"); const auto& jdof = I("jnt_dofadr");
      dofact_adr.assign(nv + 1, 0); dofact_act.clear(); siteact.clear();
      for (int i = 0; i < nv; i++) {
        dofact_adr[i] = (int)dofact_act.size();
        for (int a = 0; a < nu; a++) if (trntype[a] == TRN_JOINT && jdof[trnid[2 * a]] == i) dofact_act.push_back(a);
      }
      dofact_adr[nv] = (int)dofact_act.size();
      for (int a = 0; a < nu; a++) if (trntype[a] != TRN_JOINT) siteact.push_back(a);
      mpair.clear();
      for (int i = 0; i < nv; i++) for (int j = i; j >= 0; j = dofpar[j]) mpair.push_back((i << 8) | j);
    }
    has_damping = 0;
    for (double v : D("dof_damping")) if (v > 0) has_damping = 1;
    has_fluid = (density > 0 || viscosity > 0) ? 1 : 0;
    has_accel = 0;
    for (int t : I("sensor_type")) if (t == SENS_ACCEL) has_accel = 1;
    nvp = 1; nvshift = 0;
    while (nvp < nv) { nvp <<= 1; nvshift++; }
    const auto& g1 = I("pair_geom1"); const auto& g2 = I("pair_geom2"); const auto& gt = I("geom_type");
    int nc = 0;
    for (int p = 0; p < npair; p++) {
      int t1 = gt[g1[p]], t2 = gt[g2[p]];
      nc += ((t1 == G_PLANE && t2 == G_CAPSULE) || (t1 == G_CAPSULE && t2 == G_CAPSULE)) ? 2 : (t1 == G_PLANE && t2 == G_BOX) ? 4 : 1;
    }
    ncon_alloc = nc;
    nefc_alloc = 2 * njnt + 2 * ntendon + 4 * nc;
  }
};

template <typename T, typename Alloc>
void fill_dev_model(const HostModel& h, Alloc& alloc, int ncon_max, int nefc_max, DevModel<T>& m) {
  std::memset((void*)&m, 0, sizeof(m));
  m.nq = h.nq; m.nv = h.nv; m.nu = h.nu; m.nbody = h.nbody; m.njnt = h.njnt; m.ngeom = h.ngeom; m.nsite = h.nsite;
  m.ntendon = h.ntendon; m.nwrap = h.nwrap; m.nsensor = h.nsensor; m.nsensordata = h.nsensordata; m.nkey = h.nkey; m.npair = h.npair;
  m.nlevel = h.nlevel; m.integrator = h.integrator; m.disableactuator = h.disableactuator; m.iterations = h.iterations;
  m.has_damping = h.has_damping; m.has_fluid = h.has_fluid; m.has_accel = h.has_accel; m.nvp = h.nvp; m.nvshift = h.nvshift;
  m.ncon_max = ncon_max; m.nefc_max = nefc_max; m.nsiteact = (int)h.siteact.size(); m.nmpair = (int)h.mpair.size();
  m.timestep = (T)h.timestep; m.gravity[0] = (T)h.gravity[0]; m.gravity[1] = (T)h.gravity[1]; m.gravity[2] = (T)h.gravity[2];
  m.density = (T)h.density; m.viscosity = (T)h.viscosity; m.meaninertia = (T)h.meaninertia;
  m.tolerance = (T)h.tolerance;
  if (sizeof(T) == 4 && m.tolerance < (T)1e-6) m.tolerance = (T)1e-6;
  typedef typename DevModel<T>::FP FP;
  typedef typename DevModel<T>::IP IP;
  typedef typename DevModel<T>::UP UP;
  auto F = [&](const char* k) -> FP {
    const auto& v = h.D(k);
    std::vector<T> tv(v.begin(), v.end());
    return (FP)alloc.putf(tv);
  };
  auto Iq = [&](const char* k) -> IP { return (IP)alloc.puti(h.I(k)); };
  m.body_parentid = Iq("body_parentid"); m.body_depth = Iq("body_depth"); m.body_round = (IP)alloc.puti(h.body_round); m.nround = h.nround; m.nround_inner = h.nround_inner;
  m.body_nsub = (IP)alloc.puti(h.body_nsub); m.body_anc = (IP)alloc.puti(h.body_anc); m.max_nsub = h.max_nsub; m.dfs_ok = h.dfs_ok; m.body_rootid = Iq("body_rootid"); m.body_jntadr = Iq("body_jntadr"); m.body_jntnum = Iq("body_jntnum");
  m.body_dofadr = Iq("body_dofadr"); m.body_dofnum = Iq("body_dofnum");
  m.level_adr = (IP)alloc.puti(h.level_adr); m.level_body = (IP)alloc.puti(h.level_body); m.child_adr = (IP)alloc.puti(h.child_adr); m.child_id = (IP)alloc.puti(h.child_id); m.tri_tab = (IP)alloc.puti(h.tri_tab);
  m.dofact_adr = (IP)alloc.puti(h.dofact_adr); m.dofact_act = (IP)alloc.puti(h.dofact_act); m.siteact = (IP)alloc.puti(h.siteact); m.mpair = (IP)alloc.puti(h.mpair);
  m.body_pos = F("body_pos"); m.body_quat = F("body_quat"); m.body_ipos = F("body_ipos"); m.body_iquat = F("body_iquat"); m.body_mass = F("body_mass");
  m.body_inertia = F("body_inertia"); m.body_subtreemass = F("body_subtreemass"); m.body_invweight0 = F("body_invweight0");
  m.body_dofmask = (UP)alloc.putu(h.body_dofmask); m.dof_ancmask = (UP)alloc.putu(h.dof_ancmask);
  m.jnt_type = Iq("jnt_type"); m.jnt_qposadr = Iq("jnt_qposadr"); m.jnt_dofadr = Iq("jnt_dofadr"); m.jnt_bodyid = Iq("jnt_bodyid"); m.jnt_limited = Iq("jnt_limited");
  m.jnt_pos = F("jnt_pos"); m.jnt_axis = F("jnt_axis"); m.jnt_range = F("jnt_range"); m.jnt_stiffness = F("jnt_stiffness"); m.jnt_margin = F("jnt_margin");
  m.jnt_solref = F("jnt_solref"); m.jnt_solimp = F("jnt_solimp"); m.qpos0 = F("qpos0"); m.qpos_spring = F("qpos_spring");
  m.dof_bodyid = Iq("dof_bodyid"); m.dof_jntid = Iq("dof_jntid"); m.dof_parentid = Iq("dof_parentid");
  m.dof_armature = F("dof_armature"); m.dof_damping = F("dof_damping"); m.dof_invweight0 = F("dof_invweight0");
  m.geom_type = Iq("geom_type"); m.geom_bodyid = Iq("geom_bodyid"); m.geom_pos = F("geom_pos"); m.geom_quat = F("geom_quat"); m.geom_size = F("geom_size");
  m.site_bodyid = Iq("site_bodyid"); m.site_pos = F("site_pos"); m.site_quat = F("site_quat");
  m.tendon_adr = Iq("tendon_adr"); m.tendon_num = Iq("tendon_num"); m.tendon_limited = Iq("tendon_limited"); m.wrap_objid = Iq("wrap_objid");
  m.tendon_range = F("tendon_range"); m.tendon_margin = F("tendon_margin"); m.tendon_solref = F("tendon_solref"); m.tendon_solimp = F("tendon_solimp");
  m.tendon_invweight0 = F("tendon_invweight0"); m.wrap_prm = F("wrap_prm");
  m.actuator_trntype = Iq("actuator_trntype"); m.actuator_trnid = Iq("actuator_trnid"); m.actuator_biastype = Iq("actuator_biastype");
  m.actuator_ctrllimited = Iq("actuator_ctrllimited"); m.actuator_forcelimited = Iq("actuator_forcelimited"); m.actuator_group = Iq("actuator_group");
  m.actuator_gear = F("actuator_gear"); m.actuator_gainprm = F("actuator_gainprm"); m.actuator_biasprm = F("actuator_biasprm");
  m.actuator_ctrlrange = F("actuator_ctrlrange"); m.actuator_forcerange = F("actuator_forcerange");
  m.sensor_type = Iq("sensor_type"); m.sensor_objid = Iq("sensor_objid"); m.sensor_adr = Iq("sensor_adr");
  m.pair_geom1 = Iq("pair_geom1"); m.pair_geom2 = Iq("pair_geom2"); m.pair_condim = Iq("pair_condim");
  m.pair_friction = F("pair_friction"); m.pair_solref = F("pair_solref"); m.pair_solimp = F("pair_solimp"); m.pair_margin = F("pair_margin"); m.pair_gap = F("pair_gap");
  {
    const double MINIMP = 0.0001, MAXIMP = 0.9999, MINVAL = 1e-15;
    auto KB = [&](const double* solref, double dmax_raw, double& K, double& B) {
      const double dmax = std::min(std::max(dmax_raw, MINIMP), MAXIMP);
      if (solref[0] > 0) {
        const double tc = std::max(solref[0], 2 * h.timestep), dr = solref[1];
        K = 1 / std::max(MINVAL, dmax * dmax * tc * tc * dr * dr);
        B = 2 / std::max(MINVAL, dmax * tc);
      } else {
        K = -solref[0] / std::max(MINVAL, dmax * dmax);
        B = -solref[1] / std::max(MINVAL, dmax);
      }
    };
    const auto& g1 = h.I("pair_geom1"); const auto& g2 = h.I("pair_geom2"); const auto& gb = h.I("geom_bodyid");
    const auto& pm = h.D("pair_margin"); const auto& pg = h.D("pair_gap"); const auto& psr = h.D("pair_solref"); const auto& psi = h.D("pair_solimp");
    const auto& biw = h.D("body_invweight0");
    auto clamp_solimp = [](const double* raw, T* out) {
      const T lo = (T)0.0001, hi = (T)0.9999;
      auto tmax = [](T a, T b) { return a > b ? a : b; };
      auto tmin = [](T a, T b) { return a < b ? a : b; };
      out[0] = tmin(tmax((T)raw[0], lo), hi); out[1] = tmin(tmax((T)raw[1], lo), hi);
      out[2] = tmax((T)raw[2], (T)0); out[3] = tmin(tmax((T)raw[3], lo), hi); out[4] = tmax((T)raw[4], (T)1);
    };
    std::vector<T> kb((size_t)h.npair * PAIR_KB_STRIDE, (T)0);
    for (int p = 0; p < h.npair; p++) {
      double K, B;
      KB(&psr[2 * p], psi[5 * p + 1], K, B);
      T* r = &kb[(size_t)p * PAIR_KB_STRIDE];
      r[0] = (T)(pm[p] - pg[p]);
      r[1] = (T)(biw[2 * gb[g1[p]]] + biw[2 * gb[g2[p]]]);
      r[2] = (T)K; r[3] = (T)B;
      clamp_solimp(&psi[5 * p], r + 4);
    }
    m.pair_kb = (FP)alloc.putf(kb);
    std::vector<int> pb((size_t)h.npair * 2);
    for (int p = 0; p < h.npair; p++) { pb[2 * p] = gb[g1[p]]; pb[2 * p + 1] = gb[g2[p]]; }
    m.pair_body = (IP)alloc.puti(pb);
    const int nobj = h.njnt + h.ntendon;
    std::vector<T> lf((size_t)nobj * 12, (T)0);
    std::vector<int> li((size_t)nobj * 2, 0);
    const auto& jl = h.I("jnt_limited"); const auto& jt = h.I("jnt_type"); const auto& jq = h.I("jnt_qposadr"); const auto& jd = h.I("jnt_dofadr");
    const auto& jr = h.D("jnt_range"); const auto& jm = h.D("jnt_margin"); const auto& jsr = h.D("jnt_solref"); const auto& jsi = h.D("jnt_solimp");
    const auto& diw = h.D("dof_invweight0");
    for (int o = 0; o < h.njnt; o++) {
      double K, B;
      KB(&jsr[2 * o], jsi[5 * o + 1], K, B);
      T* r = &lf[(size_t)o * 12];
      r[0] = (T)jr[2 * o]; r[1] = (T)jr[2 * o + 1]; r[2] = (T)jm[o]; r[3] = (T)diw[jd[o]]; r[4] = (T)K; r[5] = (T)B;
      clamp_solimp(&jsi[5 * o], r + 6);
      li[2 * o] = (jl[o] && (jt[o] == JNT_HINGE || jt[o] == JNT_SLIDE)) ? 1 : 0; li[2 * o + 1] = jq[o];
    }
    if (h.ntendon > 0) {
      const auto& tl = h.I("tendon_limited"); const auto& tr = h.D("tendon_range"); const auto& tm = h.D("tendon_margin");
      const auto& tsr = h.D("tendon_solref"); const auto& tsi = h.D("tendon_solimp"); const auto& tiw = h.D("tendon_invweight0");
      for (int t = 0; t < h.ntendon; t++) {
        double K, B;
        KB(&tsr[2 * t], tsi[5 * t + 1], K, B);
        T* r = &lf[(size_t)(h.njnt + t) * 12];
        r[0] = (T)tr[2 * t]; r[1] = (T)tr[2 * t + 1]; r[2] = (T)tm[t]; r[3] = (T)tiw[t]; r[4] = (T)K; r[5] = (T)B;
        clamp_solimp(&tsi[5 * t], r + 6);
        li[2 * (h.njnt + t)] = tl[t] != 0 ? 1 : 0; li[2 * (h.njnt + t) + 1] = t;
      }
    }
    m.lim_f = (FP)alloc.putf(lf);
    m.lim_i = (IP)alloc.puti(li);
    const auto& jp = h.D("jnt_pos"); const auto& ja = h.D("jnt_axis"); const auto& q0 = h.D("qpos0");
    std::vector<T> jrec((size_t)h.njnt * 8, (T)0);
    std::vector<int> jirec((size_t)h.njnt * 6, 0);
    const auto& jb = h.I("jnt_bodyid"); const auto& bpar = h.I("body_parentid"); const auto& broot = h.I("body_rootid");
    for (int j = 0; j < h.njnt; j++) {
      for (int k = 0; k < 3; k++) { jrec[8 * j + k] = (T)jp[3 * j + k]; jrec[8 * j + 3 + k] = (T)ja[3 * j + k]; }
      jrec[8 * j + 6] = (T)q0[jq[j]];
      int* r = &jirec[6 * j];
      r[0] = jt[j]; r[1] = jq[j]; r[2] = jd[j]; r[3] = jb[j]; r[4] = bpar[jb[j]]; r[5] = broot[jb[j]];
    }
    {
      const auto& db = h.I("dof_bodyid"); const auto& dj = h.I("dof_jntid"); const auto& bda = h.I("body_dofadr");
      const auto& dd = h.D("dof_damping"); const auto& js = h.D("jnt_stiffness"); const auto& qs = h.D("qpos_spring");
      std::vector<int> dir((size_t)h.nv * 6, 0);
      std::vector<T> dfr((size_t)h.nv * 4, (T)0);
      for (int i = 0; i < h.nv; i++) {
        const int b = db[i], j = dj[i], type = jt[j], first = jd[j];
        int* r = &dir[6 * i];
        r[0] = b; r[1] = bpar[b]; r[2] = bda[b];
        r[3] = type == JNT_FREE ? (i < first + 3 ? -1 : first + 3) : i;
        const bool spring = (type == JNT_HINGE || type == JNT_SLIDE) && js[j] != 0;
        r[4] = spring ? jq[j] : -1;
        dfr[4 * i] = (T)dd[i]; dfr[4 * i + 1] = (T)(spring ? js[j] : 0.0); dfr[4 * i + 2] = (T)(spring ? qs[jq[j]] : 0.0);
      }
      m.dof_irec = (IP)alloc.puti(dir); m.dof_frec = (FP)alloc.putf(dfr);
    }
    const auto& bja = h.I("body_jntadr"); const auto& bjn = h.I("body_jntnum");
    std::vector<int> birec((size_t)h.nbody * 4, 0);
    for (int b = 0; b < h.nbody; b++) { birec[4 * b] = bja[b]; birec[4 * b + 1] = bjn[b]; birec[4 * b + 2] = bjn[b] > 0 ? jt[bja[b]] : -1; }
    m.jnt_rec = (FP)alloc.putf(jrec); m.jnt_irec = (IP)alloc.puti(jirec); m.body_irec = (IP)alloc.puti(birec);
  }
  {
    const auto& gt = h.I("geom_type"); const auto& gs = h.D("geom_size");
    const auto& g1 = h.I("pair_geom1"); const auto& g2 = h.I("pair_geom2"); const auto& pm = h.D("pair_margin");
    auto rb = [&](int g) -> double {
      const double a = gs[3 * g], b = gs[3 * g + 1], c = gs[3 * g + 2];
      switch (gt[g]) {
        case G_SPHERE: return a;
        case G_CAPSULE: return a + b;
        case G_ELLIPSOID: return std::max(a, std::max(b, c));
        case G_BOX: return std::sqrt(a * a + b * b + c * c);
        default: return 0.0;
      }
    };
    std::vector<T> cull((size_t)h.npair);
    for (int p = 0; p < h.npair; p++) {
      const bool plane = gt[g1[p]] == G_PLANE;
      const double r = (plane ? 0.0 : rb(g1[p])) + rb(g2[p]) + pm[p];
      cull[p] = (T)(plane ? -std::max(r, 1e-30) : r);
    }
    m.pair_cull = (FP)alloc.putf(cull);
  }
  m.key_qpos = F("key_qpos"); m.key_qvel = F("key_qvel"); m.key_ctrl = F("key_ctrl"); m.key_time = F("key_time");
}

inline Lay make_layout(const HostModel& h, int ncon_max, int nefc_max, size_t sizeofT, bool flat = false) {
  Lay L;
  std::memset(&L, 0, sizeof(L));
  int o = 0;
  auto A = [&](int n) { int r = o; o += n > 0 ? n : 0; return r; };
  int nq = h.nq, nv = h.nv, nu = h.nu, nb = h.nbody, nj = h.njnt, ng = h.ngeom, ns = h.nsite, nt = h.ntendon;
  L.qpos = A(nq); L.qvel = A(nv); L.ctrl = A(nu); L.qacc = A(nv); L.qacc_ws = A(nv); L.qacc_smooth = A(nv);
  L.qfrc_bias = A(nv); L.qfrc_passive = A(nv); L.qfrc_actuator = A(nv); L.qfrc_smooth = A(nv); L.qfrc_constraint = A(nv);
  L.xpos = A(3 * nb); L.xquat = A(4 * nb); L.xipos = A(3 * nb); L.ximat = A(9 * nb);
  L.geom_xpos = A(3 * ng); L.site_xpos = A(3 * ns); L.site_xmat = A(9 * ns);
  L.subtree_com = A(3 * nb); L.cinert = A(10 * nb); L.cdof = A(6 * nv); L.cvel = A(6 * nb); L.bfrc = A(h.has_fluid ? 6 * nb : 0);
  L.M = A(nv * nv); L.W = A(nv * (nv + 1) / 2); L.ten_length = A(nt); L.ten_J = A(nt * nv); L.act_force = A(nu); L.sens = A(h.nsensordata);
  L.con = A(ncon_max * CON_STRIDE);
  L.efc_J = A(nefc_max * nv); L.efc_pos = A(nefc_max); L.efc_D = A(nefc_max); L.efc_aref = A(nefc_max);
  L.tmp = A(nv > 32 ? nv + 1 : 33);
  if (h.has_accel) L.cacc = A(6 * nb);
  int r0 = o, rend = o;
  L.xmat = A(9 * nb); L.xanchor = A(3 * nj); L.xaxis = A(3 * nj); L.geom_xmat = A(9 * ng);
  if (o > rend) rend = o; if (!flat) o = r0;
  L.crb = A(10 * nb); L.dofbuf = A(6 * nv);
  if (o > rend) rend = o; if (!flat) o = r0;
  L.cdof_dot = A(6 * nv); if (!h.has_accel) L.cacc = A(6 * nb); L.cfrc = A(6 * nb);
  if (o > rend) rend = o; if (!flat) o = r0;
  L.Ma = A(nv); L.grad = A(nv); L.search = A(nv); L.Mv = A(nv); L.cholcol = A(nv + 1);
  L.efc_jar = A(nefc_max); L.efc_jv = A(nefc_max); L.efc_force = A(nefc_max); L.efc_KBI = A(nefc_max);
  if (o > rend) rend = o;
  o = rend;
  L.rk = A(h.integrator == INT_RK4 ? nq + nv + 8 * nv + nv : 0);
  L.nT = o;
  int oi = 0;
  auto AI = [&](int n) { int r = oi; oi += n > 0 ? n : 0; return r; };
  L.i_efc_type = AI(nefc_max); L.i_efc_id = L.i_efc_type; L.i_con_pair = AI(ncon_max); L.i_scal = L.i_con_pair;
  L.i_mail = AI(8);
  L.nI = oi;
  size_t bytes = (size_t)L.nT * sizeofT + (size_t)L.nI * sizeof(int);
  L.bytes = (int)((bytes + 15) / 16 * 16);
  return L;
}

inline bool fd_highest_element(long T, long B, long n, long step_stride, long env_stride, __int128& hi) {
  hi = -1;
  if (T < 1 || B < 1 || n < 0 || step_stride < 0 || env_stride < 0) return false;
  if (n == 0) return true;
  hi = (__int128)(T - 1) * step_stride + (__int128)(B - 1) * env_stride + (n - 1);
  return true;
}
inline bool fd_extent_inside(unsigned long long ptr, __int128 hi, unsigned long long esize, unsigned long long base, unsigned long long size) {
  if (hi < 0) return true;
  const __int128 end = (__int128)ptr + (hi + 1) * (__int128)esize, limit = (__int128)base + (__int128)size;
  return ptr >= base && end <= limit;
}
inline unsigned long long fd_point_scratch_bytes(int nq, int nv, int nu) {
  return (unsigned long long)(1 + 2 * (2 * nv + nu)) * (unsigned long long)(nq + nv) * 8ull;
}
inline long fd_slab_points(unsigned long long bytes_per_point, unsigned long long budget) {
  if (bytes_per_point == 0) bytes_per_point = 1;
  const unsigned long long n = budget / bytes_per_point;
  return n < 1 ? 1 : (n > 0x7fffffffull ? 0x7fffffffL : (long)n);
// ... 16 lines not shown
```

### mujoco_template_amd/csrc/mjb_kernels.hpp

```cpp
#pragma once
#include <hip/hip_runtime.h>

#include <cstddef>

#include "mjb_device.hpp"

namespace mjb {

#ifndef MJB_WPS
#define MJB_WPS 2
#endif
template <typename T, typename TS, int G>
MJB_DEV void k_step_body() {
  extern __shared__ __align__(16) char smem[];
  typedef StepKernArgs<T, TS> KA;
  const KA MJB_CONST* kp = (const KA MJB_CONST*)__builtin_amdgcn_kernarg_segment_ptr();
#if defined(MJB_TIMELINE)
  const unsigned long long tl0 = __builtin_amdgcn_s_memrealtime();
  unsigned long long tlacc = 0, tlt = 0;
#define MJB_TLACC &tlacc
#else
#define MJB_TLACC nullptr
#endif
  if (kp->a.mode == 1 && kp->a.env_mask) {
// ... 88 lines not shown
}
namespace mjb {
#endif

template <typename T, typename TS> struct ModelDataKernArgs { const DevModel<T>* mg; const Lay* lg; DevData<TS> d; };
typedef ModelDataKernArgs<double, double> MdkaDD;
typedef StepKernArgs<double, double> SkaDD;
static_assert(offsetof(MdkaDD, d) == offsetof(SkaDD, d) && offsetof(MdkaDD, d) == 2 * sizeof(void*), "the kernels' argument lists start (mg, lg, d)");
template <typename T, typename TS> MJB_DEV const PrmRows MJB_CONST* kernarg_prm() {
  return &((const ModelDataKernArgs<T, TS> MJB_CONST*)__builtin_amdgcn_kernarg_segment_ptr())->d.prm;
}

template <typename T, typename TS> struct FdKernArgs { const DevModel<T>* mg; const Lay* lg; DevData<TS> d; int ncol; T eps; T* y_out; int* valid; int cv, cc; FdPoints pt; };
typedef FdKernArgs<double, float> FkaDF;
typedef FdKernArgs<double, double> FkaDD;
static_assert(offsetof(FkaDF, mg) == 0 && offsetof(FkaDF, lg) == sizeof(void*) && offsetof(FkaDF, d) == offsetof(MdkaDD, d), "k_fd starts (mg, lg, d)");
static_assert(offsetof(FkaDF, ncol) == offsetof(FkaDF, d) + sizeof(DevData<float>) && offsetof(FkaDF, eps) == offsetof(FkaDF, ncol) + 8 &&
              offsetof(FkaDF, y_out) == offsetof(FkaDF, eps) + 8 && offsetof(FkaDF, valid) == offsetof(FkaDF, y_out) + 8 &&
              offsetof(FkaDF, cv) == offsetof(FkaDF, valid) + 8 && offsetof(FkaDF, cc) == offsetof(FkaDF, cv) + 4 &&
              offsetof(FkaDF, pt) == offsetof(FkaDF, cc) + 4, "(ncol, eps, y_out, valid, cv, cc, pt) follow d without padding beyond ncol's");
static_assert(sizeof(DevData<float>) == sizeof(DevData<double>) && offsetof(FkaDD, pt) == offsetof(FkaDF, pt) && alignof(FdPoints) == 8 &&
              sizeof(FkaDF) == offsetof(FkaDF, pt) + sizeof(FdPoints) && sizeof(FdPoints) == 12 * 8 + 2 * 4, "the point table is the last kernel argument");

template <typename T, typename TS, int G>
MJB_DEV void k_fd_body(const DevModel<T>* mg, const Lay* lg, const DevData<TS>& d, int ncol, T eps, T* y_out, int* valid, int cv, int cc) {
  const FdPoints MJB_CONST& pt = ((const FdKernArgs<T, TS> MJB_CONST*)__builtin_amdgcn_kernarg_segment_ptr())->pt;
  extern __shared__ __align__(16) char smem[];
  const int lane = threadIdx.x & (G - 1), sub = threadIdx.x / G;
  const long gid = (long)blockIdx.x * (64 / G) + sub;
  const DevModel<T> MJB_CONST* mp = (const DevModel<T> MJB_CONST*)mg;
  const Lay MJB_CONST* lp = (const Lay MJB_CONST*)lg;
  ModelRef<T> m = MJB_MODEL_OF(mp); LayRef L = *lp;
  MJB_SPEC_ASSUME(m) MJB_SPEC_ASSUME_LAY(L)
  const int nq = m.nq, nv = m.nv, nu = m.nu;
  const int nCj = (1 + 2 * nu + cc - 1) / cc, nVj = (2 * nv + cv - 1) / cv, nQj = 2 * nv, njob = nCj + nVj + nQj;
  if (gid >= (long)pt.npoint * njob) return;
  const int job = (int)(gid / pt.npoint), pl = (int)(gid % pt.npoint);
  const int env = (pt.p0 + pl) % d.batch;
  const long tp = (pt.p0 + pl) / d.batch;
  const bool rk4 = m.integrator == INT_RK4;
  int share, first, cnt, colbase;
  if (job < nCj) { share = 2; first = job * cc; cnt = 1 + 2 * nu - first; if (cnt > cc) cnt = cc; colbase = 4 * nv; }
  else if (job < nCj + nVj) { share = 1; first = (job - nCj) * cv; cnt = 2 * nv - first; if (cnt > cv) cnt = cv; colbase = 1 + 2 * nv; }
  else { share = 0; first = job - nCj - nVj; cnt = 1; colbase = 1; }
  if (rk4) share = 0;
  T* w = (T*)(smem + (size_t)sub * L.bytes);
  int* wi = (int*)(w + L.nT);
  Ctx<T> c(mp, lp, w, wi, lane, kernarg_prm<T, TS>(), env);
  for (int i = lane; i < nv * nv; i += G) w[L.M + i] = 0;
  tendon_jacobian<T, G>(c);
  const int nstage = rk4 ? 4 : 1;
  for (int it = share > 0 ? -1 : 0; it < cnt; it++) {
    {
      const TS* pq = (const TS*)pt.qpos + tp * pt.qpos_ss + (long)env * pt.qpos_es;
      const TS* pv = (const TS*)pt.qvel + tp * pt.qvel_ss + (long)env * pt.qvel_es;
      const TS* pc = (const TS*)pt.ctrl + tp * pt.ctrl_ss + (long)env * pt.ctrl_es;
      const TS* pw = pt.warmstart ? (const TS*)pt.warmstart + tp * pt.ws_ss + (long)env * pt.ws_es : nullptr;
      for (int i = lane; i < nq; i += G) w[L.qpos + i] = (T)pq[i];
      for (int i = lane; i < nv; i += G) {
        w[L.qvel + i] = (T)pv[i];
        w[L.qacc_ws + i] = pw ? (T)pw[i] : (T)0;
        w[L.qacc + i] = 0;
        w[L.Mv + i] = 0;
      }
      for (int i = lane; i < nu; i += G) w[L.ctrl + i] = (T)pc[i];
    }
    gsync<G>();
    int ok = 1, col = 0;
    if (it >= 0) {
      const int item = first + it;
      col = (share == 2 || (rk4 && job < nCj)) ? (item == 0 ? 0 : colbase + item) : colbase + item;
      if (col > 0) {
        const int k = (col - 1) >> 1;
        const T sgn = ((col - 1) & 1) ? (T)-1 : (T)1;
        if (k < nv) {
          if (lane == 0) w[L.Mv + k] = 1;
          gsync<G>();
          integrate_pos<T, G>(m, w + L.qpos, w + L.Mv, sgn * eps, lane);
        } else if (k < 2 * nv) {
          if (lane == 0) w[L.qvel + (k - nv)] += sgn * eps;
        } else {
          const int a = k - 2 * nv;
          const T v = w[L.ctrl + a] + sgn * eps;
          if (m.actuator_ctrllimited[a] && (v < m.actuator_ctrlrange[2 * a] || v > m.actuator_ctrlrange[2 * a + 1])) ok = 0;
          gsync<G>();
          if (lane == 0 && ok) w[L.ctrl + a] = v;
        }
        gsync<G>();
      }
    }
    const bool do_pos = share == 0 || it < 0;
    const bool do_vel = share == 0 || (share == 1 && it >= 0) || (share == 2 && it < 0);
    const bool do_acc = it >= 0;
    for (int st = 0; st < nstage; st++) {
      if (do_pos) forward_position<T, G>(c);
      if (do_vel) forward_velocity<T, G>(c);
      if (do_acc) forward_acceleration<T, G>(c);
      if (do_acc && nstage == 4) rk4_stage<T, G>(c, st);
    }
    if (!do_acc) continue;
    if (nstage == 1) euler<T, G>(c);
    const size_t slot = (size_t)pl * ncol + col;
    T* y = y_out + slot * (nq + nv);
    for (int i = lane; i < nq; i += G) y[i] = w[L.qpos + i];
    for (int i = lane; i < nv; i += G) y[nq + i] = w[L.qvel + i];
    if (lane == 0) valid[slot] = ok;
    gsync<G>();
  }
}
template <typename T, typename TS, int G>
__global__ __launch_bounds__(64) void k_fd(const DevModel<T>* mg, const Lay* lg, DevData<TS> d, int ncol, T eps, T* y_out, int* valid, int cv, int cc, FdPoints pt) {
  k_fd_body<T, TS, G>(mg, lg, d, ncol, eps, y_out, valid, cv, cc);
}
#if defined(MJB_SPEC_KERNEL) && MJB_SPEC_KERNEL == 2
}
extern "C" __global__ __launch_bounds__(64) void mjb_k_fd_spec(const mjb::DevModel<double>* mg, const mjb::Lay* lg, mjb::DevData<MJB_SPEC_TS> d, int ncol, double eps,
                                                               double* y_out, int* valid, int cv, int cc, mjb::FdPoints pt) {
  mjb::k_fd_body<double, MJB_SPEC_TS, MJB_SPEC_G>(mg, lg, d, ncol, eps, y_out, valid, cv, cc);
}
namespace mjb {
#endif

template <typename T>
__global__ void k_fd_combine(const DevModel<T>* mg, int batch, int ncol, int centered, T eps, const T* y, const int* valid, T* A, T* B) {
  ModelRef<T> m = *(const DevModel<T> MJB_CONST*)mg;
  const int nq = m.nq, nv = m.nv, nu = m.nu, nin = 2 * nv + nu, nx = 2 * nv;
  long tid = (long)blockIdx.x * blockDim.x + threadIdx.x;
  if (tid >= (long)batch * nin) return;
  int env = (int)(tid / nin), k = (int)(tid % nin);
  const T* y0 = y + ((size_t)env * ncol) * (nq + nv);
  const T* yp = y + ((size_t)env * ncol + 1 + 2 * k) * (nq + nv);
  const T* ym = y + ((size_t)env * ncol + 2 + 2 * k) * (nq + nv);
  bool hp = valid[(size_t)env * ncol + 1 + 2 * k] != 0, hm = centered && valid[(size_t)env * ncol + 2 + 2 * k] != 0;
  const T *a, *b; T den;
  if (hp && hm) { a = ym; b = yp; den = 2 * eps; }
  else if (hp) { a = y0; b = yp; den = eps; }
  else if (hm) { a = ym; b = y0; den = eps; }
  else { a = y0; b = y0; den = 1; }
  T* Ae = A + (size_t)env * nx * nx;
  T* Be = B + (size_t)env * nx * (nu > 0 ? nu : 1);
  for (int j = 0; j < m.njnt; j++) {
    int qa = m.jnt_qposadr[j], da = m.jnt_dofadr[j];
    T dq[6]; int nd;
    if (m.jnt_type[j] == JNT_FREE) {
      nd = 6;
      for (int q = 0; q < 3; q++) dq[q] = (b[qa + q] - a[qa + q]) / den;
      T qa4[4] = {a[qa + 3], a[qa + 4], a[qa + 5], a[qa + 6]}, qb4[4] = {b[qa + 3], b[qa + 4], b[qa + 5], b[qa + 6]}, r[3];
      quat_sub(r, qa4, qb4);
      dq[3] = r[0] / den; dq[4] = r[1] / den; dq[5] = r[2] / den;
    } else { nd = 1; dq[0] = (b[qa] - a[qa]) / den; }
    for (int q = 0; q < nd; q++) {
      if (k < 2 * nv) Ae[(size_t)(da + q) * nx + k] = dq[q]; else Be[(size_t)(da + q) * nu + (k - 2 * nv)] = dq[q];
    }
  }
  for (int r = 0; r < nv; r++) {
    T dv = (b[nq + r] - a[nq + r]) / den;
    if (k < 2 * nv) Ae[(size_t)(nv + r) * nx + k] = dv; else Be[(size_t)(nv + r) * nu + (k - 2 * nv)] = dv;
  }
}

template <typename T, typename TS, int G>
__global__ __launch_bounds__(64) void k_jac(const DevModel<T>* mg, const Lay* lg, DevData<TS> d, int nreq, const int* kinds, const int* ids, T* out_p, T* out_r) {
  extern __shared__ __align__(16) char smem[];
  const int lane = threadIdx.x & (G - 1), sub = threadIdx.x / G;
  const int env = blockIdx.x * (64 / G) + sub;
  if (env >= d.batch) return;
  const DevModel<T> MJB_CONST* mp = (const DevModel<T> MJB_CONST*)mg;
// ... 273 lines not shown
```

### mujoco_template_amd/csrc/mjb_types.hpp

```cpp
#pragma once
#include <cstdint>

#if defined(MJB_HOST_EMU) || !defined(__HIP_DEVICE_COMPILE__)
#define MJB_CONST
#else
#define MJB_CONST __attribute__((address_space(4)))
#endif

namespace mjb {

enum { JNT_FREE = 0, JNT_BALL = 1, JNT_SLIDE = 2, JNT_HINGE = 3 };
enum { G_PLANE = 0, G_HFIELD, G_SPHERE, G_CAPSULE, G_ELLIPSOID, G_CYLINDER, G_BOX, G_MESH };
enum { TRN_JOINT = 0, TRN_SITE = 4 };
enum { INT_EULER = 0, INT_RK4 = 1 };
enum { SENS_JOINTPOS = 0, SENS_GYRO, SENS_ACCEL, SENS_FRAMEQUAT };
enum { EFC_LIMIT_JOINT = 0, EFC_LIMIT_TENDON = 1, EFC_CONTACT_FRICTIONLESS = 2, EFC_CONTACT_PYRAMIDAL = 3 };
enum { CTRL_KEEP = 0, CTRL_ZERO = 1, CTRL_RANDOM = 2, CTRL_FEEDBACK = 3, CTRL_SEQUENCE = 4 };

enum { CNT_NCON = 0, CNT_NEFC, CNT_NITER, CNT_CON_DROPPED, CNT_EFC_DROPPED, CNT_BADQPOS, CNT_BADQVEL, CNT_BADQACC, CNT_N };

template <typename T>
struct DevModel {
  typedef const T MJB_CONST* FP;
  typedef const int MJB_CONST* IP;
  typedef const unsigned long long MJB_CONST* UP;
  int nq, nv, nu, nbody, njnt, ngeom, nsite, ntendon, nwrap, nsensor, nsensordata, nkey, npair;
  int nlevel, integrator, disableactuator, iterations, has_damping, has_fluid, has_accel, nvp, nvshift;
  int ncon_max, nefc_max, nsiteact, nmpair, nround, nround_inner, max_nsub, dfs_ok;
  T timestep, gravity[3], density, viscosity, tolerance, meaninertia;
  IP body_parentid, body_rootid, body_jntadr, body_jntnum, body_dofadr, body_dofnum, body_depth, body_round, body_nsub, body_anc;
  IP level_adr, level_body, child_adr, child_id, tri_tab;
  IP dofact_adr, dofact_act, siteact, mpair;
  FP body_pos, body_quat, body_ipos, body_iquat, body_mass, body_inertia, body_subtreemass, body_invweight0;
  UP body_dofmask, dof_ancmask;
  IP jnt_type, jnt_qposadr, jnt_dofadr, jnt_bodyid, jnt_limited;
  FP jnt_pos, jnt_axis, jnt_range, jnt_stiffness, jnt_margin, jnt_solref, jnt_solimp, qpos0, qpos_spring;
  IP dof_bodyid, dof_jntid, dof_parentid;
  FP dof_armature, dof_damping, dof_invweight0;
  IP geom_type, geom_bodyid;
  FP geom_pos, geom_quat, geom_size;
  IP site_bodyid;
  FP site_pos, site_quat;
  IP tendon_adr, tendon_num, tendon_limited, wrap_objid;
  FP tendon_range, tendon_margin, tendon_solref, tendon_solimp, tendon_invweight0, wrap_prm;
  IP actuator_trntype, actuator_trnid, actuator_biastype, actuator_ctrllimited, actuator_forcelimited, actuator_group;
  FP actuator_gear, actuator_gainprm, actuator_biasprm, actuator_ctrlrange, actuator_forcerange;
  IP sensor_type, sensor_objid, sensor_adr;
  IP pair_geom1, pair_geom2, pair_condim;
  FP pair_friction, pair_solref, pair_solimp, pair_margin, pair_gap;
  FP pair_kb;
  FP lim_f;
  FP jnt_rec;
  IP jnt_irec;
  IP dof_irec;
  FP dof_frec;
  IP body_irec;
  IP pair_body;
  IP lim_i;
  FP pair_cull;
  FP key_qpos, key_qvel, key_ctrl, key_time;
};

struct Lay {
  int qpos, qvel, ctrl, qacc, qacc_ws, qacc_smooth;
  int qfrc_bias, qfrc_passive, qfrc_actuator, qfrc_smooth, qfrc_constraint;
  int xpos, xquat, xmat, xipos, ximat, xanchor, xaxis, geom_xpos, geom_xmat, site_xpos, site_xmat;
  int subtree_com, cinert, crb, cdof, cdof_dot, cvel, cacc, cfrc, dofbuf, bfrc;
  int M, W, ten_length, ten_J, act_force, sens;
  int con;
  int efc_J, efc_pos, efc_D, efc_aref, efc_jar, efc_jv, efc_force, efc_KBI;
  int Ma, grad, search, Mv, tmp, cholcol;
  int rk;
  int nT;
  int i_efc_type, i_efc_id, i_con_pair, i_scal;
  int i_mail;
  int nI;
  int bytes;
};

constexpr int PAIR_KB_STRIDE = 12;
constexpr int CON_STRIDE = 11;

enum { PRM_BODY_MASS = 0, PRM_BODY_INERTIA, PRM_DOF_DAMPING, PRM_DOF_ARMATURE, PRM_ACT_GEAR, PRM_ACT_GAINPRM, PRM_ACT_BIASPRM,
       PRM_GEOM_FRICTION, PRM_GRAVITY, PRM_NFIELD, PRM_SUBTREEMASS = PRM_NFIELD, PRM_PAIR_FRICTION, PRM_NSLOT };
struct PrmRows {
  const float MJB_CONST* f[PRM_NSLOT];
  const double MJB_CONST* d[PRM_NSLOT];
};

template <typename TS>
struct DevData {
  int batch;
  TS *qpos, *qvel, *ctrl, *qacc, *qacc_warmstart;
  double* time;
  TS *xpos, *xquat, *xipos, *site_xpos, *geom_xpos, *subtree_com, *sensordata;
  TS *qfrc_inverse, *actuator_moment;
  int* counters;
  int* flags;
  int* flags_pin;
  unsigned long long* prof;
  unsigned* sched;
  unsigned long long* xfer;
  PrmRows prm;
};
enum { PH_KIN = 0, PH_COM, PH_CRB, PH_COLL, PH_CONS, PH_VEL, PH_ACT, PH_SOLVE, PH_INTEG, PH_OTHER, PH_SOL_DIR, PH_SOL_LS, PH_CNT_LS = 12, PH_CNT_DIR, PH_CNT_FACT, PH_SOL_MV, PH_FAC_LOAD = 16, PH_FAC_PANEL, PH_FAC_BACK, PH_FAC_ALL, PH_N = 24 };

template <typename TS>
struct DevDebug {
  TS *qM, *qfrc_bias, *qfrc_passive, *qfrc_actuator, *qacc_smooth, *qfrc_constraint;
  TS *efc_J, *efc_aref, *efc_D, *efc_pos, *efc_force, *con;
  TS *cdof, *cinert, *cvel;
  int *efc_type;
};

struct ObsSpecDev {
  int flags;
  int nsite, nbody, ngeom, nsubtree, dim;
  const int *site_ids, *body_ids, *geom_ids, *subtree_ids;
};

struct FdPoints {
  const void *qpos, *qvel, *ctrl, *warmstart;
  long qpos_ss, qpos_es, qvel_ss, qvel_es, ctrl_ss, ctrl_es, ws_ss, ws_es;
  int p0, npoint;
};

struct StepArgs {
  int nstep;
  int ctrl_mode;
  unsigned seed, step0, env0;
  double ctrl_scale;
  double dt;
  int mode;
  int write_kin;
  int obs_every;
  const void *fb_K, *fb_u0, *fb_q0, *fb_v0;
  const void *fb_noise_std, *fb_noise_tab;
  int fb_nsteps, fb_env_stride;
  double* mirror;
  int mirror_mask;
  unsigned long long mirror_seq;
  int fair_bit;
  unsigned ticket_base;
  unsigned tagbase;
  int nblk, grid_blocks;
  int chunk_steps;
  int repeat_phase;
  unsigned xfer_timeout;
  int xfer_poison_env;
  int nuniform, nchunk;
  const unsigned char* env_mask;
  const void* ctrl_seq;
  long ctrl_step_stride, ctrl_env_stride;
};

#if defined(__HIPCC__)
__host__ __device__
#endif
inline void chunk_plan(int nstep, int chunk_steps, int nuniform, int k, int& s0, int& s1) {
  if (k < nuniform) { s0 = k * chunk_steps; s1 = s0 + chunk_steps; return; }
  int at = nuniform * chunk_steps;
// ... 23 lines not shown
```

Baseline: 55.06 million.

## Constant-fold uniform columns of baked model record tables at compile time

```diff
diff --git a/mujoco_template_amd/csrc/mjb_api.hip b/mujoco_template_amd/csrc/mjb_api.hip
--- a/mujoco_template_amd/csrc/mjb_api.hip
+++ b/mujoco_template_amd/csrc/mjb_api.hip
@@ -3,6 +3,7 @@
 #include <dlfcn.h>
 
 #include <cmath>
+#include <cstddef>
 #include <cstdio>
 #include <cstdlib>
 #include <chrono>
@@ -339,38 +340,53 @@
 }
 
 struct EmitAlloc {
+  struct Cols { int stride = 1; unsigned long long mask = 0; const char* ctype = ""; std::vector<std::string> val; };
   std::string text;
+  std::vector<Cols> cols;
   int n = 0;
   static constexpr unsigned long long TOKEN = 0x7E57AB1Eull << 32;
-  template <typename X, typename F> const X* emit(const std::vector<X>& v, const char* ctype, F fmt) {
+  template <typename X, typename F> const X* emit(const std::vector<X>& v, const char* ctype, int stride, F fmt) {
     std::string body;
     if (v.empty()) body = "0";
     for (size_t i = 0; i < v.size(); i++) { if (i) body += (i % 16 == 0 ? ",\n " : ","); body += fmt(v[i]); }
     text += std::string("static const __constant__ ") + ctype + " mjb_tab_" + std::to_string(n) + "[] = {" + body + "};\n";
+    Cols c;
+    c.ctype = ctype;
+    const size_t S = stride > 1 ? (size_t)stride : 1;
+    if (S > 1 && S <= 64 && v.size() % S == 0 && v.size() >= 2 * S) {
+      c.stride = (int)S;
+      c.val.assign(S, "0");
+      for (size_t k = 0; k < S; k++) {
+        bool same = v[k] == v[k];
+        for (size_t r = 1; r * S < v.size() && same; r++) same = std::memcmp(&v[r * S + k], &v[k], sizeof(X)) == 0;
+        if (same) { c.mask |= 1ull << k; c.val[k] = fmt(v[k]); }
+      }
+    }
+    cols.push_back(c);
     return (const X*)(uintptr_t)(TOKEN + (unsigned long long)(n++) * 16ull + 16ull);
   }
-  const float* putf(const std::vector<float>& v) {
-    return emit(v, "float", [](float x) {
+  const float* putf(const std::vector<float>& v, int stride = 1) {
+    return emit(v, "float", stride, [](float x) {
       if (std::isnan(x)) return std::string("__builtin_nanf(\"\")");
       if (std::isinf(x)) return std::string(x > 0 ? "__builtin_inff()" : "-__builtin_inff()");
       char b[48]; std::snprintf(b, sizeof(b), "%af", (double)x); return std::string(b);
     });
   }
-  const double* putf(const std::vector<double>& v) {
-    return emit(v, "double", [](double x) {
+  const double* putf(const std::vector<double>& v, int stride = 1) {
+    return emit(v, "double", stride, [](double x) {
       if (std::isnan(x)) return std::string("__builtin_nan(\"\")");
       if (std::isinf(x)) return std::string(x > 0 ? "__builtin_inf()" : "-__builtin_inf()");
       char b[48]; std::snprintf(b, sizeof(b), "%a", x); return std::string(b);
     });
   }
-  const int* puti(const std::vector<int>& v) { return emit(v, "int", [](int x) { return std::to_string(x); }); }
-  const unsigned long long* putu(const std::vector<unsigned long long>& v) {
-    return emit(v, "unsigned long long", [](unsigned long long x) { char b[40]; std::snprintf(b, sizeof(b), "0x%llxull", x); return std::string(b); });
+  const int* puti(const std::vector<int>& v, int stride = 1) { return emit(v, "int", stride, [](int x) { return std::to_string(x); }); }
+  const unsigned long long* putu(const std::vector<unsigned long long>& v, int stride = 1) {
+    return emit(v, "unsigned long long", stride, [](unsigned long long x) { char b[40]; std::snprintf(b, sizeof(b), "0x%llxull", x); return std::string(b); });
   }
 };
 
 template <typename T>
-std::string baked_model_source(const HostModel& h, int ncon_max, int nefc_max) {
+std::string baked_model_source(const HostModel& h, int ncon_max, int nefc_max, int prm_mask) {
   static_assert(sizeof(DevModel<T>) % 8 == 0, "DevModel<T> is written out in 8-byte words");
   const char* tname = sizeof(T) == 4 ? "float" : "double";
   EmitAlloc ea;
@@ -407,6 +423,34 @@
   }
   std::string s = "#include \"mjb_types.hpp\"\n// the model as constant data of this translation unit (tables, then the DevModel image)\n";
   s += ea.text + decl + init;
+  {
+    struct Named { size_t off; const char* name; int prm; unsigned long long drop; };
+#define NM(f, prm, drop) {offsetof(DevModel<T>, f), #f, prm, drop}
+    const Named named[] = {
+        NM(body_pos, -1, 0), NM(body_quat, -1, 0), NM(body_ipos, -1, 0), NM(body_iquat, -1, 0), NM(geom_size, -1, 0), NM(actuator_trnid, -1, 0),
+        NM(actuator_gear, PRM_ACT_GEAR, ~0ull), NM(actuator_gainprm, PRM_ACT_GAINPRM, ~0ull), NM(actuator_biasprm, PRM_ACT_BIASPRM, ~0ull),
+        NM(actuator_ctrlrange, -1, 0), NM(actuator_forcerange, -1, 0), NM(pair_friction, PRM_GEOM_FRICTION, ~0ull),
+        NM(pair_kb, -1, 0), NM(lim_f, -1, 0), NM(jnt_rec, -1, 0), NM(jnt_irec, -1, 0), NM(dof_irec, -1, 0),
+        NM(dof_frec, PRM_DOF_DAMPING, 1ull), NM(body_irec, -1, 0), NM(pair_body, -1, 0), NM(lim_i, -1, 0)};
+#undef NM
+    for (size_t i = 0; i < nw; i++) {
+      if ((wv[i] >> 32) != (EmitAlloc::TOKEN >> 32)) continue;
+      const EmitAlloc::Cols& c = ea.cols[(size_t)((wv[i] - EmitAlloc::TOKEN) / 16 - 1)];
+      const Named* nm = nullptr;
+      for (const Named& x : named) if (x.off == 8 * i) nm = &x;
+      if (!nm) continue;
+      unsigned long long mask = c.mask;
+      if (nm->prm >= 0 && ((prm_mask >> nm->prm) & 1)) mask &= ~nm->drop;
+      if (!mask) continue;
+      char hex[24];
+      std::snprintf(hex, sizeof(hex), "0x%llxull", mask);
+      s += std::string("// uniform columns of ") + nm->name + " (stride " + std::to_string(c.stride) + ")\ntemplate <> struct mjb::UniformCols<" + std::to_string(i) +
+           "> { static constexpr unsigned long long mask = " + hex + ";";
+      s += std::string(" static constexpr ") + c.ctype + " val[" + std::to_string(c.stride) + "] = {";
+      for (int k = 0; k < c.stride; k++) s += (k ? ", " : "") + ((mask >> k) & 1 ? c.val[(size_t)k] : std::string("0"));
+      s += "}; };\n";
+    }
+  }
   s += std::string("static_assert(sizeof(MjbBakedModel) == sizeof(mjb::DevModel<") + tname + ">), \"baked model image\");\n";
   s += std::string("#define MJB_SPEC_BAKED (*(const mjb::DevModel<") + tname + "> MJB_CONST*)&mjb_baked_model)\n";
   return s;
@@ -449,7 +493,7 @@
     }
     if (le2) s += "#define MJB_SPEC_SOLIMP_POWER_1_OR_2 1\n";
   }
-  s += kind != MJB_KERNEL_FD ? baked_model_source<float>(h, ncon_max, nefc_max) : baked_model_source<double>(h, ncon_max, nefc_max);
+  s += kind != MJB_KERNEL_FD ? baked_model_source<float>(h, ncon_max, nefc_max, prm_mask) : baked_model_source<double>(h, ncon_max, nefc_max, prm_mask);
   s += "#include \"mjb_kernels.hpp\"\n";
   if (prm_mask) s += "extern \"C\" __constant__ int mjb_spec_params = " + std::to_string(prm_mask) + ";   // checked by mjb_kernel_load\n";
   return s;
diff --git a/mujoco_template_amd/csrc/mjb_device.hpp b/mujoco_template_amd/csrc/mjb_device.hpp
--- a/mujoco_template_amd/csrc/mjb_device.hpp
+++ b/mujoco_template_amd/csrc/mjb_device.hpp
@@ -1,5 +1,6 @@
 #pragma once
 #include "mjb_types.hpp"
+#include <cstddef>
 
 #ifdef MJB_HOST_EMU
 #include <cmath>
@@ -485,6 +486,42 @@
 #define MJB_MODEL_OF(p) (*(p))
 #endif
 #define MJB_OPT(c, f) ((*(c).mp).f)
+#if defined(MJB_SPEC_BAKED) && !defined(MJB_HOST_EMU)
+template <typename TP> struct RecElem;
+template <typename E> struct RecElem<const E MJB_CONST*> { typedef E type; };
+template <int W, int S, typename TP> MJB_DEV typename RecElem<TP>::type rec_get(TP tab, int i, int k) {
+  if constexpr (UniformCols<W>::mask != 0) {
+    if ((UniformCols<W>::mask >> k) & 1) return UniformCols<W>::val[k];
+  }
+  return tab[S * i + k];
+}
+template <typename M> struct RecModel;
+template <typename E> struct RecModel<const DevModel<E> MJB_CONST&> { typedef DevModel<E> type; };
+#define MJB_REC_W(m, f) ((int)(offsetof(typename mjb::RecModel<decltype(m)>::type, f) / 8))
+#define MJB_REC(m, f, S, i, k) (mjb::rec_get<MJB_REC_W(m, f), (S)>((m).f, (i), (k)))
+MJB_DEV bool rec_same_bits(float a, float b) { return __builtin_bit_cast(unsigned, a) == __builtin_bit_cast(unsigned, b); }
+MJB_DEV bool rec_same_bits(double a, double b) { return __builtin_bit_cast(unsigned long long, a) == __builtin_bit_cast(unsigned long long, b); }
+MJB_DEV bool rec_same_bits(int a, int b) { return a == b; }
+template <int W, typename E> MJB_DEV E rec_pin(E v, int k) {
+  if constexpr (UniformCols<W>::mask != 0) {
+    if ((UniformCols<W>::mask >> k) & 1) return UniformCols<W>::val[k];
+  }
+  return v;
+}
+template <int W1, int W2, typename E> MJB_DEV E rec_pin2(E v, int k1, int k2) {
+  if constexpr (UniformCols<W1>::mask != 0 && UniformCols<W2>::mask != 0) {
+    if (((UniformCols<W1>::mask >> k1) & 1) && ((UniformCols<W2>::mask >> k2) & 1) && rec_same_bits(UniformCols<W1>::val[k1], UniformCols<W2>::val[k2]))
+      return UniformCols<W1>::val[k1];
+  }
+  return v;
+}
+#define MJB_REC_PIN(m, f, k, v) (mjb::rec_pin<MJB_REC_W(m, f)>((v), (k)))
+#define MJB_REC_PIN2(m, f1, k1, f2, k2, v) (mjb::rec_pin2<MJB_REC_W(m, f1), MJB_REC_W(m, f2)>((v), (k1), (k2)))
+#else
+#define MJB_REC(m, f, S, i, k) ((m).f[(S) * (i) + (k)])
+#define MJB_REC_PIN(m, f, k, v) (v)
+#define MJB_REC_PIN2(m, f1, k1, f2, k2, v) (v)
+#endif
 #ifdef MJB_HOST_EMU
 #define MJB_ENV(c) ModelRef<T> m = *(c).mp; LayRef L = *(c).lp
 #else
@@ -554,6 +591,13 @@
   }
   return tab[ti];
 }
+#if defined(MJB_SPEC_BAKED) && !defined(MJB_HOST_EMU)
+#define MJB_PRM_REC(K, c, m, f, S, n, i, k) (MJB_PRM_ON(mjb::prm_src<K>()) ? mjb::prm_row<K>(c, (m).f, n)[(S) * (i) + (k)] : MJB_REC(m, f, S, i, k))
+#define MJB_PRM_GET_REC(K, c, m, f, S, n, i, k) (MJB_PRM_ON(mjb::prm_src<K>()) ? mjb::prm_get<K>(c, (m).f, n, i, (S) * (i) + (k)) : MJB_REC(m, f, S, i, k))
+#else
+#define MJB_PRM_REC(K, c, m, f, S, n, i, k) (mjb::prm_row<K>(c, (m).f, n)[(S) * (i) + (k)])
+#define MJB_PRM_GET_REC(K, c, m, f, S, n, i, k) (mjb::prm_get<K>(c, (m).f, n, i, (S) * (i) + (k)))
+#endif
 template <typename T> MJB_DEV bool has_damping(const Ctx<T>& c, int model_has_damping) {
   if constexpr (MJB_PRM_ON(PRM_DOF_DAMPING)) {
     if (MJB_PRM_SURE) return true;
@@ -1071,10 +1115,10 @@
     for (int k = 0; k < 9; k++) { xmat[k] = (k % 4 == 0) ? (T)1 : (T)0; ximat[k] = xmat[k]; }
   }
   for (int b = 1 + lane; b < m.nbody; b += G) {
-    const int jadr = m.body_irec[4 * b], jnum = m.body_irec[4 * b + 1], jt0 = m.body_irec[4 * b + 2];
+    const int jadr = MJB_REC(m, body_irec, 4, b, 0), jnum = MJB_REC(m, body_irec, 4, b, 1), jt0 = MJB_REC(m, body_irec, 4, b, 2);
     T pos[3], quat[4], R[9];
     if (jnum == 1 && jt0 == JNT_FREE) {
-      int qa = m.jnt_irec[6 * jadr + 1];
+      int qa = MJB_REC(m, jnt_irec, 6, jadr, 1);
       quat[0] = qpos[qa + 3]; quat[1] = qpos[qa + 4]; quat[2] = qpos[qa + 5]; quat[3] = qpos[qa + 6];
       quat_normalize(quat);
       qpos[qa + 3] = quat[0]; qpos[qa + 4] = quat[1]; qpos[qa + 5] = quat[2]; qpos[qa + 6] = quat[3];
@@ -1083,15 +1127,15 @@
       xaxis[3 * jadr] = 0; xaxis[3 * jadr + 1] = 0; xaxis[3 * jadr + 2] = 1;
     } else {
 #pragma unroll
-      for (int k = 0; k < 3; k++) pos[k] = m.body_pos[3 * b + k];
-#pragma unroll
-      for (int k = 0; k < 4; k++) quat[k] = m.body_quat[4 * b + k];
+      for (int k = 0; k < 3; k++) pos[k] = MJB_REC(m, body_pos, 3, b, k);
+#pragma unroll
+      for (int k = 0; k < 4; k++) quat[k] = MJB_REC(m, body_quat, 4, b, k);
       quat2mat(R, quat);
       for (int j = jadr; j < jadr + jnum; j++) {
-        T jp[3] = {m.jnt_rec[8 * j], m.jnt_rec[8 * j + 1], m.jnt_rec[8 * j + 2]};
-        T ja[3] = {m.jnt_rec[8 * j + 3], m.jnt_rec[8 * j + 4], m.jnt_rec[8 * j + 5]};
-        const int jtype = m.jnt_irec[6 * j], qa = m.jnt_irec[6 * j + 1];
-        T val = qpos[qa] - m.jnt_rec[8 * j + 6];
+        T jp[3] = {MJB_REC(m, jnt_rec, 8, j, 0), MJB_REC(m, jnt_rec, 8, j, 1), MJB_REC(m, jnt_rec, 8, j, 2)};
+        T ja[3] = {MJB_REC(m, jnt_rec, 8, j, 3), MJB_REC(m, jnt_rec, 8, j, 4), MJB_REC(m, jnt_rec, 8, j, 5)};
+        const int jtype = MJB_REC(m, jnt_irec, 6, j, 0), qa = MJB_REC(m, jnt_irec, 6, j, 1);
+        T val = qpos[qa] - MJB_REC(m, jnt_rec, 8, j, 6);
         T anchor[3], axis[3];
         mulmatvec3(anchor, R, jp);
         anchor[0] += pos[0]; anchor[1] += pos[1]; anchor[2] += pos[2];
@@ -1181,8 +1225,8 @@
 #pragma unroll
     for (int k = 0; k < 4; k++) quat[k] = xquat[4 * b + k];
     quat2mat(R, quat);
-    T ip[3] = {m.body_ipos[3 * b], m.body_ipos[3 * b + 1], m.body_ipos[3 * b + 2]};
-    T iq[4] = {m.body_iquat[4 * b], m.body_iquat[4 * b + 1], m.body_iquat[4 * b + 2], m.body_iquat[4 * b + 3]};
+    T ip[3] = {MJB_REC(m, body_ipos, 3, b, 0), MJB_REC(m, body_ipos, 3, b, 1), MJB_REC(m, body_ipos, 3, b, 2)};
+    T iq[4] = {MJB_REC(m, body_iquat, 4, b, 0), MJB_REC(m, body_iquat, 4, b, 1), MJB_REC(m, body_iquat, 4, b, 2), MJB_REC(m, body_iquat, 4, b, 3)};
     mulmatvec3(t, R, ip);
     quat_mul(q2, quat, iq);
     quat2mat(R2, q2);
@@ -1192,8 +1236,8 @@
     for (int k = 0; k < 9; k++) { xmat[9 * b + k] = R[k]; ximat[9 * b + k] = R2[k]; }
   }
   for (int j = lane; j < m.njnt; j += G) {
-    if (m.jnt_irec[6 * j] == JNT_FREE) continue;
-    int p = m.jnt_irec[6 * j + 4];
+    if (MJB_REC(m, jnt_irec, 6, j, 0) == JNT_FREE) continue;
+    int p = MJB_REC(m, jnt_irec, 6, j, 4);
     T pq[4], R[9], a[3], ax[3], la[3] = {xanchor[3 * j], xanchor[3 * j + 1], xanchor[3 * j + 2]}, lx[3] = {xaxis[3 * j], xaxis[3 * j + 1], xaxis[3 * j + 2]};
 #pragma unroll
     for (int k = 0; k < 4; k++) pq[k] = xquat[4 * p + k];
@@ -1267,7 +1311,7 @@
   }
   T *cdof = w + L.cdof, *xanchor = w + L.xanchor, *xaxis = w + L.xaxis;
   for (int j = lane; j < m.njnt; j += G) {
-    int b = m.jnt_irec[6 * j + 3], da = m.jnt_irec[6 * j + 2], r = m.jnt_irec[6 * j + 5], jt = m.jnt_irec[6 * j];
+    int b = MJB_REC(m, jnt_irec, 6, j, 3), da = MJB_REC(m, jnt_irec, 6, j, 2), r = MJB_REC(m, jnt_irec, 6, j, 5), jt = MJB_REC(m, jnt_irec, 6, j, 0);
     T off[3];
 #pragma unroll
     for (int k = 0; k < 3; k++) off[k] = sc[3 * r + k] - xanchor[3 * j + k];
@@ -1389,8 +1433,8 @@
       int g1 = m.pair_geom1[p], g2 = m.pair_geom2[p], t1 = m.geom_type[g1], t2 = m.geom_type[g2];
       T margin = m.pair_margin[p];
       T p1[3] = {gx[3 * g1], gx[3 * g1 + 1], gx[3 * g1 + 2]}, p2[3] = {gx[3 * g2], gx[3 * g2 + 1], gx[3 * g2 + 2]};
-      T s1[3] = {m.geom_size[3 * g1], m.geom_size[3 * g1 + 1], m.geom_size[3 * g1 + 2]};
-      T s2[3] = {m.geom_size[3 * g2], m.geom_size[3 * g2 + 1], m.geom_size[3 * g2 + 2]};
+      T s1[3] = {MJB_REC(m, geom_size, 3, g1, 0), MJB_REC(m, geom_size, 3, g1, 1), MJB_REC(m, geom_size, 3, g1, 2)};
+      T s2[3] = {MJB_REC(m, geom_size, 3, g2, 0), MJB_REC(m, geom_size, 3, g2, 1), MJB_REC(m, geom_size, 3, g2, 2)};
       T z1[3] = {gm[9 * g1 + 2], gm[9 * g1 + 5], gm[9 * g1 + 8]}, z2[3] = {gm[9 * g2 + 2], gm[9 * g2 + 5], gm[9 * g2 + 8]};
       if (t1 == G_PLANE) {
         if (t2 == G_SPHERE) n = nc_plane_sphere(p1, z1, p2, s2[0], margin, rc[0]);
@@ -1505,7 +1549,7 @@
           o[0] = r.dist; o[1] = r.pos[0]; o[2] = r.pos[1]; o[3] = r.pos[2];
 #pragma unroll
           for (int a = 0; a < 6; a++) o[4 + a] = f[a];
-          o[10] = prm_row<PRM_PAIR_FRICTION>(c, m.pair_friction, 5 * m.npair)[5 * p];
+          o[10] = MJB_PRM_REC(PRM_PAIR_FRICTION, c, m, pair_friction, 5, 5 * m.npair, p, 0);
           con_pair[slot] = p;
         }
       }
@@ -1629,10 +1673,10 @@
     T dist = 0, dist2 = 0, margin = 0, mu = 0;
     bool both = false;
     if (isl) {
-      if (m.lim_i[2 * k]) {
-        const T value = isj ? qpos[m.lim_i[2 * k + 1]] : tl[m.lim_i[2 * k + 1]];
-        margin = m.lim_f[12 * k + 2];
-        const T d0 = value - m.lim_f[12 * k], d1 = m.lim_f[12 * k + 1] - value;
+      if (MJB_REC(m, lim_i, 2, k, 0)) {
+        const T value = isj ? qpos[MJB_REC(m, lim_i, 2, k, 1)] : tl[MJB_REC(m, lim_i, 2, k, 1)];
+        margin = MJB_REC(m, lim_f, 12, k, 2);
+        const T d0 = value - MJB_REC(m, lim_f, 12, k, 0), d1 = MJB_REC(m, lim_f, 12, k, 1) - value;
         const bool a0 = d0 < margin, a1 = d1 < margin;
         cnt = (int)a0 + (int)a1;
         both = a0 && a1;
@@ -1641,7 +1685,7 @@
     } else if (k < nitem) {
       p = con_pair[ci] & 0xffff;
       dist = con[ci * CON_STRIDE]; mu = con[ci * CON_STRIDE + 10];
-      margin = m.pair_kb[PAIR_KB_STRIDE * p];
+      margin = MJB_REC(m, pair_kb, PAIR_KB_STRIDE, p, 0);
       if (dist < margin) cnt = m.pair_condim[p] == 1 ? 1 : 4;
     }
     int total, off = gscan_small<G>(cnt, lane, total);
@@ -1657,24 +1701,26 @@
         type = (isj ? EFC_LIMIT_JOINT : EFC_LIMIT_TENDON) | (((isj ? k : k - m.njnt) * 2 + sd) << 9);
       }
       if (emit || both) {
-        diag = m.lim_f[12 * k + 3]; K = m.lim_f[12 * k + 4]; B = m.lim_f[12 * k + 5];
-#pragma unroll
-        for (int q = 0; q < 5; q++) si[q] = m.lim_f[12 * k + 6 + q];
+        diag = MJB_REC(m, lim_f, 12, k, 3); K = MJB_REC(m, lim_f, 12, k, 4); B = MJB_REC(m, lim_f, 12, k, 5);
+#pragma unroll
+        for (int q = 0; q < 5; q++) si[q] = MJB_REC(m, lim_f, 12, k, 6 + q);
       }
     } else if (k < nitem) {
       emit = cnt > 0 && row + cnt <= cap;
       con_pair[ci] = p | ((emit ? row + 1 : 0) << 16);
       if (emit) {
-        const T tran = m.pair_kb[PAIR_KB_STRIDE * p + 1];
-        K = m.pair_kb[PAIR_KB_STRIDE * p + 2]; B = m.pair_kb[PAIR_KB_STRIDE * p + 3];
-#pragma unroll
-        for (int q = 0; q < 5; q++) si[q] = m.pair_kb[PAIR_KB_STRIDE * p + 4 + q];
+        const T tran = MJB_REC(m, pair_kb, PAIR_KB_STRIDE, p, 1);
+        K = MJB_REC(m, pair_kb, PAIR_KB_STRIDE, p, 2); B = MJB_REC(m, pair_kb, PAIR_KB_STRIDE, p, 3);
+#pragma unroll
+        for (int q = 0; q < 5; q++) si[q] = MJB_REC(m, pair_kb, PAIR_KB_STRIDE, p, 4 + q);
         if (cnt == 1) diag = tran; else diag = tran + mu * mu * tran;
         type = (cnt == 1 ? EFC_CONTACT_FRICTIONLESS : EFC_CONTACT_PYRAMIDAL) | (ci << 9);
       }
     }
     if (emit) {
       T imp, R;
+#pragma unroll
+      for (int q = 0; q < 5; q++) si[q] = MJB_REC_PIN2(m, lim_f, 6 + q, pair_kb, 4 + q, si[q]);
       row_imp_R(dist, margin, si, diag, imp, R);
       int nr = 1;
       if (!isl && cnt == 4) {
@@ -1693,6 +1739,8 @@
     if (base < nobj && gany<G>(both)) {
       if (both && row + 1 < cap) {
         T imp, R;
+#pragma unroll
+        for (int q = 0; q < 5; q++) si[q] = MJB_REC_PIN(m, lim_f, 6 + q, si[q]);
         row_imp_R(dist2, margin, si, diag, imp, R);
         etype[row + 1] = type + (1 << 9);
         epos[row + 1] = dist2; emargin[row + 1] = margin; eD[row + 1] = 1 / R; eK[row + 1] = K; eB[row + 1] = B; eI[row + 1] = imp;
@@ -1733,7 +1781,7 @@
       int row = (con_pair[ci] >> 16) - 1;
       if (row < 0) continue;
       int p = con_pair[ci] & 0xffff;
-      int b1 = m.pair_body[2 * p], b2 = m.pair_body[2 * p + 1];
+      int b1 = MJB_REC(m, pair_body, 2, p, 0), b2 = MJB_REC(m, pair_body, 2, p, 1);
       const T* cc = con + ci * CON_STRIDE;
       const bool mv1 = (m.body_dofmask[b1] >> i) & 1ull, mv2 = (m.body_dofmask[b2] >> i) & 1ull;
       T dj[3] = {0, 0, 0};
@@ -1787,7 +1835,7 @@
   gsync<G>();
   tree_forward_sum<T, G, 6>(c, cvel);
   for (int j = lane; j < nv; j += G) {
-    const int p = m.dof_irec[6 * j + 1], first = m.dof_irec[6 * j + 2], gs = m.dof_irec[6 * j + 3];
+    const int p = MJB_REC(m, dof_irec, 6, j, 1), first = MJB_REC(m, dof_irec, 6, j, 2), gs = MJB_REC(m, dof_irec, 6, j, 3);
     T tmp[6] = {0, 0, 0, 0, 0, 0};
     if (gs >= 0) {
       T cv[6], cd[6];
@@ -1882,13 +1930,13 @@
   }
   T *qb = w + L.qfrc_bias, *qp = w + L.qfrc_passive;
   for (int i = lane; i < nv; i += G) {
-    const int b = m.dof_irec[6 * i], qa = m.dof_irec[6 * i + 4];
+    const int b = MJB_REC(m, dof_irec, 6, i, 0), qa = MJB_REC(m, dof_irec, 6, i, 4);
     T v = 0;
 #pragma unroll
     for (int k = 0; k < 6; k++) v += cdof[6 * i + k] * cfrc[6 * b + k];
     qb[i] = v;
-    T pf = -prm_get<PRM_DOF_DAMPING>(c, m.dof_frec, nv, i, 4 * i) * qvel[i];
-    if (qa >= 0) pf -= m.dof_frec[4 * i + 1] * (qpos[qa] - m.dof_frec[4 * i + 2]);
+    T pf = -MJB_PRM_GET_REC(PRM_DOF_DAMPING, c, m, dof_frec, 4, nv, i, 0) * qvel[i];
+    if (qa >= 0) pf -= MJB_REC(m, dof_frec, 4, i, 1) * (qpos[qa] - MJB_REC(m, dof_frec, 4, i, 2));
     if (m.has_fluid) {
       T* xipos = w + L.xipos;
       for (int bb = 1; bb < m.nbody; bb++) {
@@ -1911,20 +1959,20 @@
     T force = 0;
     if (!(grp >= 0 && grp < 31 && ((MJB_OPT(c, disableactuator) >> grp) & 1))) {
       T u = ctrl[a];
-      if (m.actuator_ctrllimited[a]) u = t_min(t_max(u, m.actuator_ctrlrange[2 * a]), m.actuator_ctrlrange[2 * a + 1]);
-      force = prm_row<PRM_ACT_GAINPRM>(c, m.actuator_gainprm, 3 * m.nu)[3 * a] * u;
+      if (m.actuator_ctrllimited[a]) u = t_min(t_max(u, MJB_REC(m, actuator_ctrlrange, 2, a, 0)), MJB_REC(m, actuator_ctrlrange, 2, a, 1));
+      force = MJB_PRM_REC(PRM_ACT_GAINPRM, c, m, actuator_gainprm, 3, 3 * m.nu, a, 0) * u;
       if (m.actuator_biastype[a] == 1) {
         T len = 0, vel = 0;
         if (m.actuator_trntype[a] == TRN_JOINT) {
-          int j = m.actuator_trnid[2 * a];
-          const T MJB_CONST* gear = prm_row<PRM_ACT_GEAR>(c, m.actuator_gear, 6 * m.nu);
-          len = gear[6 * a] * qpos[m.jnt_qposadr[j]];
-          vel = gear[6 * a] * qvel[m.jnt_dofadr[j]];
+          int j = MJB_REC(m, actuator_trnid, 2, a, 0);
+          const T gear0 = MJB_PRM_REC(PRM_ACT_GEAR, c, m, actuator_gear, 6, 6 * m.nu, a, 0);
+          len = gear0 * qpos[m.jnt_qposadr[j]];
+          vel = gear0 * qvel[m.jnt_dofadr[j]];
         }
-        const T MJB_CONST* bias = prm_row<PRM_ACT_BIASPRM>(c, m.actuator_biasprm, 3 * m.nu);
-        force += bias[3 * a] + bias[3 * a + 1] * len + bias[3 * a + 2] * vel;
-      }
-      if (m.actuator_forcelimited[a]) force = t_min(t_max(force, m.actuator_forcerange[2 * a]), m.actuator_forcerange[2 * a + 1]);
+        force += MJB_PRM_REC(PRM_ACT_BIASPRM, c, m, actuator_biasprm, 3, 3 * m.nu, a, 0) + MJB_PRM_REC(PRM_ACT_BIASPRM, c, m, actuator_biasprm, 3, 3 * m.nu, a, 1) * len +
+                 MJB_PRM_REC(PRM_ACT_BIASPRM, c, m, actuator_biasprm, 3, 3 * m.nu, a, 2) * vel;
+      }
+      if (m.actuator_forcelimited[a]) force = t_min(t_max(force, MJB_REC(m, actuator_forcerange, 2, a, 0)), MJB_REC(m, actuator_forcerange, 2, a, 1));
     }
     af[a] = force;
   }
@@ -1933,14 +1981,13 @@
   T *sx = w + L.site_xpos, *sm = w + L.site_xmat;
   for (int i = lane; i < nv; i += G) {
     T s = 0;
-    const T MJB_CONST* gear = prm_row<PRM_ACT_GEAR>(c, m.actuator_gear, 6 * m.nu);
-    for (int k = m.dofact_adr[i]; k < m.dofact_adr[i + 1]; k++) { int a = m.dofact_act[k]; s += gear[6 * a] * af[a]; }
+    for (int k = m.dofact_adr[i]; k < m.dofact_adr[i + 1]; k++) { int a = m.dofact_act[k]; s += MJB_PRM_REC(PRM_ACT_GEAR, c, m, actuator_gear, 6, 6 * m.nu, a, 0) * af[a]; }
     for (int k = 0; k < m.nsiteact; k++) {
-      int a = m.siteact[k], id = m.actuator_trnid[2 * a], b = m.site_bodyid[id];
+      int a = m.siteact[k], id = MJB_REC(m, actuator_trnid, 2, a, 0), b = m.site_bodyid[id];
       if (!((m.body_dofmask[b] >> i) & 1ull)) continue;
       T g[6], R[9], f[3], tq[3], pt[3] = {sx[3 * id], sx[3 * id + 1], sx[3 * id + 2]}, jp[3], jr[3];
 #pragma unroll
-      for (int q = 0; q < 6; q++) g[q] = gear[6 * a + q];
+      for (int q = 0; q < 6; q++) g[q] = MJB_PRM_REC(PRM_ACT_GEAR, c, m, actuator_gear, 6, 6 * m.nu, a, q);
 #pragma unroll
       for (int q = 0; q < 9; q++) R[q] = sm[9 * id + q];
       mulmatvec3(f, R, g);
@@ -2237,8 +2284,8 @@
 
 template <typename T, int G> MJB_DEV void integrate_pos(ModelRef<T> m, T* qpos, const T* qvel, T h, int lane) {
   for (int j = lane; j < m.njnt; j += G) {
-    int qa = m.jnt_irec[6 * j + 1], da = m.jnt_irec[6 * j + 2];
-    if (m.jnt_irec[6 * j] == JNT_FREE) {
+    int qa = MJB_REC(m, jnt_irec, 6, j, 1), da = MJB_REC(m, jnt_irec, 6, j, 2);
+    if (MJB_REC(m, jnt_irec, 6, j, 0) == JNT_FREE) {
       qpos[qa] += h * qvel[da]; qpos[qa + 1] += h * qvel[da + 1]; qpos[qa + 2] += h * qvel[da + 2];
       T q[4] = {qpos[qa + 3], qpos[qa + 4], qpos[qa + 5], qpos[qa + 6]}, wv[3] = {qvel[da + 3], qvel[da + 4], qvel[da + 5]};
       quat_integrate(q, wv, h);
@@ -2318,7 +2365,7 @@
     unsigned r = philox_first(env, step, (unsigned)a, 0u, seed, 0x5EEDu);
     T u = (T)(r >> 8) * (T)(1.0 / 16777216.0);
     T lo = -1, hi = 1;
-    if (m.actuator_ctrllimited[a]) { lo = m.actuator_ctrlrange[2 * a]; hi = m.actuator_ctrlrange[2 * a + 1]; }
+    if (m.actuator_ctrllimited[a]) { lo = MJB_REC(m, actuator_ctrlrange, 2, a, 0); hi = MJB_REC(m, actuator_ctrlrange, 2, a, 1); }
     ctrl[a] = (T)0.5 * (lo + hi) + (T)0.5 * (hi - lo) * scale * (2 * u - 1);
   }
 }
@@ -2346,7 +2393,7 @@
       const long idx = ((long)step + (long)env * a.fb_env_stride) % a.fb_nsteps;
       u += ((const T MJB_CONST*)a.fb_noise_std)[act] * ((const T MJB_CONST*)a.fb_noise_tab)[idx * nu + act];
     }
-    if (m.actuator_ctrllimited[act]) u = t_min(t_max(u, m.actuator_ctrlrange[2 * act]), m.actuator_ctrlrange[2 * act + 1]);
+    if (m.actuator_ctrllimited[act]) u = t_min(t_max(u, MJB_REC(m, actuator_ctrlrange, 2, act, 0)), MJB_REC(m, actuator_ctrlrange, 2, act, 1));
     ctrl[act] = u;
   }
   gsync<G>();
diff --git a/mujoco_template_amd/csrc/mjb_host.hpp b/mujoco_template_amd/csrc/mjb_host.hpp
--- a/mujoco_template_amd/csrc/mjb_host.hpp
+++ b/mujoco_template_amd/csrc/mjb_host.hpp
@@ -196,6 +196,12 @@
   }
 };
 
+namespace put_detail {
+template <typename A, typename V> auto f(A& a, const V& v, int stride, int) -> decltype(a.putf(v, stride)) { return a.putf(v, stride); }
+template <typename A, typename V> auto f(A& a, const V& v, int, long) -> decltype(a.putf(v)) { return a.putf(v); }
+template <typename A, typename V> auto i(A& a, const V& v, int stride, int) -> decltype(a.puti(v, stride)) { return a.puti(v, stride); }
+template <typename A, typename V> auto i(A& a, const V& v, int, long) -> decltype(a.puti(v)) { return a.puti(v); }
+}
 template <typename T, typename Alloc>
 void fill_dev_model(const HostModel& h, Alloc& alloc, int ncon_max, int nefc_max, DevModel<T>& m) {
   std::memset((void*)&m, 0, sizeof(m));
@@ -211,37 +217,37 @@
   typedef typename DevModel<T>::FP FP;
   typedef typename DevModel<T>::IP IP;
   typedef typename DevModel<T>::UP UP;
-  auto F = [&](const char* k) -> FP {
+  auto F = [&](const char* k, int stride = 1) -> FP {
     const auto& v = h.D(k);
     std::vector<T> tv(v.begin(), v.end());
-    return (FP)alloc.putf(tv);
+    return (FP)put_detail::f(alloc, tv, stride, 0);
   };
-  auto Iq = [&](const char* k) -> IP { return (IP)alloc.puti(h.I(k)); };
+  auto Iq = [&](const char* k, int stride = 1) -> IP { return (IP)put_detail::i(alloc, h.I(k), stride, 0); };
   m.body_parentid = Iq("body_parentid"); m.body_depth = Iq("body_depth"); m.body_round = (IP)alloc.puti(h.body_round); m.nround = h.nround; m.nround_inner = h.nround_inner;
   m.body_nsub = (IP)alloc.puti(h.body_nsub); m.body_anc = (IP)alloc.puti(h.body_anc); m.max_nsub = h.max_nsub; m.dfs_ok = h.dfs_ok; m.body_rootid = Iq("body_rootid"); m.body_jntadr = Iq("body_jntadr"); m.body_jntnum = Iq("body_jntnum");
   m.body_dofadr = Iq("body_dofadr"); m.body_dofnum = Iq("body_dofnum");
   m.level_adr = (IP)alloc.puti(h.level_adr); m.level_body = (IP)alloc.puti(h.level_body); m.child_adr = (IP)alloc.puti(h.child_adr); m.child_id = (IP)alloc.puti(h.child_id); m.tri_tab = (IP)alloc.puti(h.tri_tab);
   m.dofact_adr = (IP)alloc.puti(h.dofact_adr); m.dofact_act = (IP)alloc.puti(h.dofact_act); m.siteact = (IP)alloc.puti(h.siteact); m.mpair = (IP)alloc.puti(h.mpair);
-  m.body_pos = F("body_pos"); m.body_quat = F("body_quat"); m.body_ipos = F("body_ipos"); m.body_iquat = F("body_iquat"); m.body_mass = F("body_mass");
-  m.body_inertia = F("body_inertia"); m.body_subtreemass = F("body_subtreemass"); m.body_invweight0 = F("body_invweight0");
+  m.body_pos = F("body_pos", 3); m.body_quat = F("body_quat", 4); m.body_ipos = F("body_ipos", 3); m.body_iquat = F("body_iquat", 4); m.body_mass = F("body_mass");
+  m.body_inertia = F("body_inertia", 3); m.body_subtreemass = F("body_subtreemass"); m.body_invweight0 = F("body_invweight0", 2);
   m.body_dofmask = (UP)alloc.putu(h.body_dofmask); m.dof_ancmask = (UP)alloc.putu(h.dof_ancmask);
   m.jnt_type = Iq("jnt_type"); m.jnt_qposadr = Iq("jnt_qposadr"); m.jnt_dofadr = Iq("jnt_dofadr"); m.jnt_bodyid = Iq("jnt_bodyid"); m.jnt_limited = Iq("jnt_limited");
-  m.jnt_pos = F("jnt_pos"); m.jnt_axis = F("jnt_axis"); m.jnt_range = F("jnt_range"); m.jnt_stiffness = F("jnt_stiffness"); m.jnt_margin = F("jnt_margin");
-  m.jnt_solref = F("jnt_solref"); m.jnt_solimp = F("jnt_solimp"); m.qpos0 = F("qpos0"); m.qpos_spring = F("qpos_spring");
+  m.jnt_pos = F("jnt_pos", 3); m.jnt_axis = F("jnt_axis", 3); m.jnt_range = F("jnt_range", 2); m.jnt_stiffness = F("jnt_stiffness"); m.jnt_margin = F("jnt_margin");
+  m.jnt_solref = F("jnt_solref", 2); m.jnt_solimp = F("jnt_solimp", 5); m.qpos0 = F("qpos0"); m.qpos_spring = F("qpos_spring");
   m.dof_bodyid = Iq("dof_bodyid"); m.dof_jntid = Iq("dof_jntid"); m.dof_parentid = Iq("dof_parentid");
   m.dof_armature = F("dof_armature"); m.dof_damping = F("dof_damping"); m.dof_invweight0 = F("dof_invweight0");
-  m.geom_type = Iq("geom_type"); m.geom_bodyid = Iq("geom_bodyid"); m.geom_pos = F("geom_pos"); m.geom_quat = F("geom_quat"); m.geom_size = F("geom_size");
-  m.site_bodyid = Iq("site_bodyid"); m.site_pos = F("site_pos"); m.site_quat = F("site_quat");
+  m.geom_type = Iq("geom_type"); m.geom_bodyid = Iq("geom_bodyid"); m.geom_pos = F("geom_pos", 3); m.geom_quat = F("geom_quat", 4); m.geom_size = F("geom_size", 3);
+  m.site_bodyid = Iq("site_bodyid"); m.site_pos = F("site_pos", 3); m.site_quat = F("site_quat", 4);
   m.tendon_adr = Iq("tendon_adr"); m.tendon_num = Iq("tendon_num"); m.tendon_limited = Iq("tendon_limited"); m.wrap_objid = Iq("wrap_objid");
-  m.tendon_range = F("tendon_range"); m.tendon_margin = F("tendon_margin"); m.tendon_solref = F("tendon_solref"); m.tendon_solimp = F("tendon_solimp");
+  m.tendon_range = F("tendon_range", 2); m.tendon_margin = F("tendon_margin"); m.tendon_solref = F("tendon_solref", 2); m.tendon_solimp = F("tendon_solimp", 5);
   m.tendon_invweight0 = F("tendon_invweight0"); m.wrap_prm = F("wrap_prm");
-  m.actuator_trntype = Iq("actuator_trntype"); m.actuator_trnid = Iq("actuator_trnid"); m.actuator_biastype = Iq("actuator_biastype");
+  m.actuator_trntype = Iq("actuator_trntype"); m.actuator_trnid = Iq("actuator_trnid", 2); m.actuator_biastype = Iq("actuator_biastype");
   m.actuator_ctrllimited = Iq("actuator_ctrllimited"); m.actuator_forcelimited = Iq("actuator_forcelimited"); m.actuator_group = Iq("actuator_group");
-  m.actuator_gear = F("actuator_gear"); m.actuator_gainprm = F("actuator_gainprm"); m.actuator_biasprm = F("actuator_biasprm");
-  m.actuator_ctrlrange = F("actuator_ctrlrange"); m.actuator_forcerange = F("actuator_forcerange");
+  m.actuator_gear = F("actuator_gear", 6); m.actuator_gainprm = F("actuator_gainprm", 3); m.actuator_biasprm = F("actuator_biasprm", 3);
+  m.actuator_ctrlrange = F("actuator_ctrlrange", 2); m.actuator_forcerange = F("actuator_forcerange", 2);
   m.sensor_type = Iq("sensor_type"); m.sensor_objid = Iq("sensor_objid"); m.sensor_adr = Iq("sensor_adr");
   m.pair_geom1 = Iq("pair_geom1"); m.pair_geom2 = Iq("pair_geom2"); m.pair_condim = Iq("pair_condim");
-  m.pair_friction = F("pair_friction"); m.pair_solref = F("pair_solref"); m.pair_solimp = F("pair_solimp"); m.pair_margin = F("pair_margin"); m.pair_gap = F("pair_gap");
+  m.pair_friction = F("pair_friction", 5); m.pair_solref = F("pair_solref", 2); m.pair_solimp = F("pair_solimp", 5); m.pair_margin = F("pair_margin"); m.pair_gap = F("pair_gap");
   {
     const double MINIMP = 0.0001, MAXIMP = 0.9999, MINVAL = 1e-15;
     auto KB = [&](const double* solref, double dmax_raw, double& K, double& B) {
@@ -275,10 +281,10 @@
       r[2] = (T)K; r[3] = (T)B;
       clamp_solimp(&psi[5 * p], r + 4);
     }
-    m.pair_kb = (FP)alloc.putf(kb);
+    m.pair_kb = (FP)put_detail::f(alloc, kb, PAIR_KB_STRIDE, 0);
     std::vector<int> pb((size_t)h.npair * 2);
     for (int p = 0; p < h.npair; p++) { pb[2 * p] = gb[g1[p]]; pb[2 * p + 1] = gb[g2[p]]; }
-    m.pair_body = (IP)alloc.puti(pb);
+    m.pair_body = (IP)put_detail::i(alloc, pb, 2, 0);
     const int nobj = h.njnt + h.ntendon;
     std::vector<T> lf((size_t)nobj * 12, (T)0);
     std::vector<int> li((size_t)nobj * 2, 0);
@@ -305,8 +311,8 @@
         li[2 * (h.njnt + t)] = tl[t] != 0 ? 1 : 0; li[2 * (h.njnt + t) + 1] = t;
       }
     }
-    m.lim_f = (FP)alloc.putf(lf);
-    m.lim_i = (IP)alloc.puti(li);
+    m.lim_f = (FP)put_detail::f(alloc, lf, 12, 0);
+    m.lim_i = (IP)put_detail::i(alloc, li, 2, 0);
     const auto& jp = h.D("jnt_pos"); const auto& ja = h.D("jnt_axis"); const auto& q0 = h.D("qpos0");
     std::vector<T> jrec((size_t)h.njnt * 8, (T)0);
     std::vector<int> jirec((size_t)h.njnt * 6, 0);
@@ -331,12 +337,12 @@
         r[4] = spring ? jq[j] : -1;
         dfr[4 * i] = (T)dd[i]; dfr[4 * i + 1] = (T)(spring ? js[j] : 0.0); dfr[4 * i + 2] = (T)(spring ? qs[jq[j]] : 0.0);
       }
-      m.dof_irec = (IP)alloc.puti(dir); m.dof_frec = (FP)alloc.putf(dfr);
+      m.dof_irec = (IP)put_detail::i(alloc, dir, 6, 0); m.dof_frec = (FP)put_detail::f(alloc, dfr, 4, 0);
     }
     const auto& bja = h.I("body_jntadr"); const auto& bjn = h.I("body_jntnum");
     std::vector<int> birec((size_t)h.nbody * 4, 0);
     for (int b = 0; b < h.nbody; b++) { birec[4 * b] = bja[b]; birec[4 * b + 1] = bjn[b]; birec[4 * b + 2] = bjn[b] > 0 ? jt[bja[b]] : -1; }
-    m.jnt_rec = (FP)alloc.putf(jrec); m.jnt_irec = (IP)alloc.puti(jirec); m.body_irec = (IP)alloc.puti(birec);
+    m.jnt_rec = (FP)put_detail::f(alloc, jrec, 8, 0); m.jnt_irec = (IP)put_detail::i(alloc, jirec, 6, 0); m.body_irec = (IP)put_detail::i(alloc, birec, 4, 0);
   }
   {
     const auto& gt = h.I("geom_type"); const auto& gs = h.D("geom_size");
diff --git a/mujoco_template_amd/csrc/mjb_kernels.hpp b/mujoco_template_amd/csrc/mjb_kernels.hpp
--- a/mujoco_template_amd/csrc/mjb_kernels.hpp
+++ b/mujoco_template_amd/csrc/mjb_kernels.hpp
@@ -194,7 +194,7 @@
         } else {
           const int a = k - 2 * nv;
           const T v = w[L.ctrl + a] + sgn * eps;
-          if (m.actuator_ctrllimited[a] && (v < m.actuator_ctrlrange[2 * a] || v > m.actuator_ctrlrange[2 * a + 1])) ok = 0;
+          if (m.actuator_ctrllimited[a] && (v < MJB_REC(m, actuator_ctrlrange, 2, a, 0) || v > MJB_REC(m, actuator_ctrlrange, 2, a, 1))) ok = 0;
           gsync<G>();
           if (lane == 0 && ok) w[L.ctrl + a] = v;
         }
diff --git a/mujoco_template_amd/csrc/mjb_types.hpp b/mujoco_template_amd/csrc/mjb_types.hpp
--- a/mujoco_template_amd/csrc/mjb_types.hpp
+++ b/mujoco_template_amd/csrc/mjb_types.hpp
@@ -77,6 +77,8 @@
   int nI;
   int bytes;
 };
+
+template <int W> struct UniformCols { static constexpr unsigned long long mask = 0; };
 
 constexpr int PAIR_KB_STRIDE = 12;
 constexpr int CON_STRIDE = 11;
```

Measured after the change: 55.80 million (median of 6 runs). 1.4% higher.
